# facebookresearch/ReAgent

Hardware: AMD Instinct MI355X
Metric: transitions/sec at batch=65536 state_dim=128; 1/2/4/8 MI355X scaling (higher is better)
Workload: dtype bf16; 1 GPU; Discrete DQN state_dim=128 |A|=16 3x512 MLP (BASELINE.json configs[1]; replay gather + normalize + 3 fwd + TD/Huber + bwd + Adam + soft update); batch=65536/GPU, 3x512 hidden; global_batch=65536, parallelism=dp1, launch=eager stream launches

## Files before the change

### include/reagent_hip.h

```cpp
#ifndef REAGENT_HIP_H_
#define REAGENT_HIP_H_

#include <stddef.h>
#include <stdint.h>

#ifdef __cplusplus
extern "C" {
#endif

typedef void* rg_stream_t;

enum { RG_OK = 0, RG_EINVAL = -1, RG_EALIGN = -2, RG_EUNSUPPORTED = -3, RG_EWORKSPACE = -4 };
enum { RG_PREC_F32 = 0, RG_PREC_BF16 = 1, RG_PREC_BF16X3 = 2  };
enum { RG_DT_F32 = 0, RG_DT_BF16 = 1 };
enum {
  RG_ACT_LINEAR = 0, RG_ACT_RELU = 1, RG_ACT_LEAKY_RELU = 2, RG_ACT_TANH = 3, RG_ACT_SIGMOID = 4,
  RG_ACT_SOFTPLUS = 5
};
enum { RG_LOSS_MSE = 0, RG_LOSS_HUBER = 1 };

const char* rg_strerror(int code);
int rg_abi_version(void);


// ... 24 lines not shown
                           rg_stream_t stream);

size_t rg_batch_norm_workspace_bytes(int batch, int n);
int rg_batch_norm_forward(const float* x, int64_t ldx, const float* gamma, const float* beta, float* running_mean,
                          float* running_var, int training, int stat_updates, double momentum, double eps, int batch, int n, float* y,
                          int64_t ldy, float* save_mean, float* save_rstd, void* workspace, size_t workspace_bytes,
                          rg_stream_t stream);
int rg_batch_norm_backward(const float* g, int64_t ldg, const float* x, int64_t ldx, const float* gamma,
                           const float* mean, const float* rstd, const float* running_var, int training, double eps,
                           int batch, int n, float* dx, int64_t lddx, float* dgamma, float* dbeta, void* workspace,
                           size_t workspace_bytes, rg_stream_t stream);

int rg_dropout(const float* x, int64_t ldx, int batch, int n, double p, int generate, uint64_t seed, uint64_t offset,
               uint8_t* keep, float* y, int64_t ldy, rg_stream_t stream);

int rg_act_backward(const float* dy, int64_t ld_dy, const float* y, int64_t ld_y, int act, float* dz,
                    int64_t ld_dz, int rows, int cols, rg_stream_t stream);


#define RG_MLP_MAX_LAYERS 6
typedef struct {
  int32_t n_layers;
  int32_t dims[RG_MLP_MAX_LAYERS + 1];
  int32_t acts[RG_MLP_MAX_LAYERS];
  const void* wfrag_fwd[RG_MLP_MAX_LAYERS];
  const void* wfrag_bwd[RG_MLP_MAX_LAYERS];
  const float* bias[RG_MLP_MAX_LAYERS];
  void* act_frag[RG_MLP_MAX_LAYERS];
  void* dz_frag[RG_MLP_MAX_LAYERS];
  void* act_sign[RG_MLP_MAX_LAYERS];
  float* db[RG_MLP_MAX_LAYERS];
  const float* w[RG_MLP_MAX_LAYERS];
  float* dw[RG_MLP_MAX_LAYERS];
  int32_t x3;
  int32_t dx_only;
  const void* x2;
  int64_t ldx2;
  int32_t x_split;
  int32_t dx_col0;
  int32_t x2_dtype;
  int32_t wgrad_flags;
  const int32_t* rowmap;
  const int32_t* tile_key;
  const int32_t* row_begin;
  int32_t n_groups;
  int32_t out_scatter;
  int64_t group_stride_fwd, group_stride_bwd;
  int32_t defer_db;
  int32_t sum_n;
  const float* db_partials;
  const float* sum_in;
  float* sum_out;
  double sum_scale;
} rg_mlp_desc;

int rg_mlp_fused_supported(const rg_mlp_desc* d);
size_t rg_frag_elems(int rows, int cols);
size_t rg_sign_bytes(int rows, int cols);
size_t rg_wfrag_elems(int out_features, int in_features);
int rg_stage_weights_frag(const float* w, int out_features, int in_features, void* wfrag_fwd,
                          void* wfrag_bwd, rg_stream_t stream);
int rg_mlp_forward_fused(const rg_mlp_desc* d, const void* x, int x_dtype, int64_t ldx, int batch,
                         float* out32, int64_t ldo, int save, rg_stream_t stream);
size_t rg_mlp_backward_fused_workspace_bytes(const rg_mlp_desc* d, int batch);
int rg_mlp_backward_fused(const rg_mlp_desc* d, const float* dout32, int64_t lddo, int batch,
                          float* dx32, int64_t lddx, void* workspace, size_t workspace_bytes,
                          rg_stream_t stream);
size_t rg_fc_wgrad_frag_workspace_bytes(int out_features, int in_features, int batch);
int rg_fc_wgrad_frag(const void* dz_frag, const void* x_frag, int out_features, int in_features,
                     int batch, float* dw, void* workspace, size_t workspace_bytes,
                     rg_stream_t stream);

int rg_mlp_stage_weights_fused(const rg_mlp_desc* d, int need_bwd, rg_stream_t stream);
size_t rg_mlp_wgrad_fused_workspace_bytes(const rg_mlp_desc* d, int batch);
int rg_mlp_wgrad_fused(const rg_mlp_desc* d, int batch, void* workspace, size_t workspace_bytes,
                       rg_stream_t stream);

typedef struct {
  float* param;
  const float* grad;
  float* exp_avg;
  float* exp_avg_sq;
  float* target;
  int32_t n_layers;
  int32_t dims[RG_MLP_MAX_LAYERS + 1];
  int64_t w_off[RG_MLP_MAX_LAYERS];
  int64_t b_off[RG_MLP_MAX_LAYERS];
  void* wfrag_fwd[RG_MLP_MAX_LAYERS];
  void* wfrag_bwd[RG_MLP_MAX_LAYERS];
  void* target_wfrag_fwd[RG_MLP_MAX_LAYERS];
  int32_t x3;
  int32_t group_rows[RG_MLP_MAX_LAYERS];
  int32_t sched_pre_ticked;
  int32_t post_tick_mod;
  int64_t* post_tick;
} rg_mlp_update_desc;
int rg_mlp_update_fused(const rg_mlp_update_desc* d, double lr, double beta1, double beta2, double eps,
                        double weight_decay, double bias_correction1, double bias_correction2_sqrt,
                        double grad_scale, double tau, rg_stream_t stream);


int rg_replay_nstep(const int64_t* indices, const uint8_t* terminal, const float* reward,
                    const float* decays, int64_t capacity, int update_horizon, int batch,
                    int64_t* steps, int64_t* next_indices, uint8_t* out_terminal,
                    float* out_reward, rg_stream_t stream);

// ... 98 lines not shown
  const int64_t* mdp_id;
  const int64_t* sequence_number;
  const float* decays;
  int64_t capacity;
  int32_t n_features;
  int32_t n_actions;
  int32_t update_horizon;
  int32_t reserved;
} rg_replay_view;
int rg_replay_dqn_batch(const rg_replay_view* view, const int64_t* indices, int batch, const rg_norm_col* cols,
                        const float* quantiles, const rg_dqn_batch_out* out, rg_stream_t stream);
int rg_replay_dqn_batch_pooled(const rg_replay_view* view, const int64_t* index_pool, const int64_t* cursor,
                               double* pre_tick_sched, int batch, const rg_norm_col* cols, const float* quantiles,
                               const rg_dqn_batch_out* out, rg_stream_t stream);

typedef struct {
  const float* observation;
  const float* action;
  const float* reward;
  const uint8_t* terminal;
  const float* log_prob;
  const float* decays;
  const float* ranges;
  int64_t capacity;
  int32_t n_features;
  int32_t action_dim;
  int32_t update_horizon;
  int32_t reserved;
} rg_policy_replay_view;
typedef struct {
  void* state;
  void* next_state;
  float* action;
  float* next_action;
  float* reward;
  float* not_terminal;
  float* action_probability;
  int32_t state_dtype;
  int32_t reserved;
} rg_policy_batch_out;
int rg_replay_policy_batch(const rg_policy_replay_view* view, const int64_t* indices, int batch, const rg_norm_col* cols,
                           const float* quantiles, const rg_policy_batch_out* out, rg_stream_t stream);

int rg_table_check_actions(const rg_dqn_table* table, const int64_t* indices, int batch, int* bad_flag,
                           rg_stream_t stream);


int rg_dqn_head_partials(int batch);
int rg_dqn_head(const float* q, const float* qn_online, const float* qn_target, const float* action,
                const float* next_mask, const float* reward, const float* reward_boosts,
                const float* not_terminal, double gamma, const float* gamma_exponent, int batch,
                int num_actions, int double_q, int loss_type, float* dq, float* loss_partials,
                float* next_q, int64_t* next_idx, float* q_sel, rg_stream_t stream);

int rg_bcq_filter(const float* imitator_logits, int batch, int num_actions, double drop_threshold, float* mask,
                  rg_stream_t stream);

int rg_cpe_head(const float* reward_est, const float* q_cpe, const float* q_cpe_tgt_next,
                const float* next_scores, const float* next_mask, const float* action,
                const float* reward, const float* extra_metrics, const float* not_terminal, double gamma,
                const float* gamma_exponent, double temperature, int batch, int num_actions,
                int num_metrics, int loss_type, float* d_reward_est, float* d_q_cpe,
                float* reward_partials, float* cpe_partials, float* propensities_out,
                rg_stream_t stream);

int rg_c51_head(const float* q, const float* qn_online, const float* qn_target, const float* action,
                const float* next_mask, const float* reward, const float* reward_boosts,
                const float* not_terminal, double gamma, const float* gamma_exponent, const float* support,
                double qmin, double qmax, int batch, int num_actions, int num_atoms, int maxq, float* dq,
                float* loss_partials, float* all_q, rg_stream_t stream);

int rg_dueling_combine(const float* value, int64_t ldv, const float* advantage, int64_t lda, int batch,
                       int num_actions, int num_atoms, float* q, int64_t ldq, rg_stream_t stream);
int rg_dueling_split(const float* dq, int64_t lddq, int batch, int num_actions, int num_atoms, float* dadvantage,
                     int64_t ldda, float* dvalue, int64_t lddv, rg_stream_t stream);

size_t rg_group_rows_workspace_bytes(int batch, int n_groups);
int rg_group_rows(const int32_t* key, int batch, int n_groups, int n_tiles, int dense, int32_t* rowmap, int32_t* tile_key,
                  int32_t* row_begin, void* workspace, size_t workspace_bytes, rg_stream_t stream);
size_t rg_group_wfrag_elems(int group_rows, int in_features, int transposed);
int rg_group_weights_stage(const float* w, int n_groups, int group_rows, int in_features, int x3, void* wfrag_fwd,
                           void* wfrag_bwd, rg_stream_t stream);
int rg_wide_head_mean(const float* w, const float* b, int n_groups, int group_rows, int in_features, float* wbar,
                      float* bbar, rg_stream_t stream);
int rg_wide_head_mean_staged(const float* w, const float* b, int n_groups, int group_rows, int in_features, float* wbar,
                             float* bbar, void* wfrag_fwd, int x3, rg_stream_t stream);
int rg_qr_select_action(const float* q, int64_t ldq, const float* mask, int batch, int num_actions, int maxq,
                        int32_t* key, rg_stream_t stream);
int rg_qr_select_group_rows(const float* q, int64_t ldq, const float* mask, int batch, int num_actions, int maxq,
                            int32_t* key, int n_tiles, int dense, int32_t* rowmap, int32_t* tile_key, int32_t* row_begin,
                            void* workspace, size_t workspace_bytes, rg_stream_t stream);
int rg_qr_compact_head(const float* z, int64_t ldz, const float* zt, int64_t ldzt, const int32_t* rowmap,
                       const int32_t* row_key, int padded_rows, const float* reward, const float* reward_boosts,
                       const float* not_terminal, double gamma, const float* gamma_exponent,
                       const float* quantiles, int batch, int num_atoms, float* dz, int64_t lddz,
                       float* loss_partials, float* tile_losses, rg_stream_t stream);
size_t rg_group_head_wgrad_workspace_bytes(int n_groups, int group_rows, int in_features, int splits);
int rg_group_head_wgrad(const void* dz_frag, const void* h_frag, const int32_t* row_begin, int n_groups,
                        int group_rows, int in_features, int splits, int x3, int rows, float* dw, void* workspace,
                        size_t workspace_bytes, rg_stream_t stream);

int rg_crr_partials(int batch);
int rg_crr_critic_head(const float* q1, const float* q2, const float* q1_next_target, const float* q2_next_target,
                       const float* next_logits, const float* action, const float* reward,
                       const float* reward_boosts, const float* not_terminal, double gamma, int batch,
                       int num_actions, float* target_out, float* dq1, float* dq2, float* partials1,
                       float* partials2, rg_stream_t stream);
int rg_crr_actor_head(const float* q, const float* logits, const float* action, const float* logged_prob,
                      double beta, double max_weight, double entropy_coeff, double clip_limit, int batch,
                      int num_actions, float* dlogits, float* plain_partials, float* entropy_partials,
                      rg_stream_t stream);

int rg_qr_head(const float* q, const float* qn_online, const float* qn_target, const float* action,
               const float* next_mask, const float* reward, const float* reward_boosts,
               const float* not_terminal, double gamma, const float* gamma_exponent,
               const float* quantiles, int batch, int num_actions, int num_atoms, int maxq, float* dq,
               float* loss_partials, float* all_q, rg_stream_t stream);


int rg_gaussian_head_forward(const float* loc_scale, int64_t ldls, const float* noise, int batch,
                             int action_dim, float* action, int64_t lda, float* log_prob,
                             float* squashed_mean, rg_stream_t stream);
int rg_gaussian_log_prob(const float* loc_scale, int64_t ldls, const float* action, int64_t lda,
                         int batch, int action_dim, float* log_prob, rg_stream_t stream);
int rg_gaussian_head_backward(const float* loc_scale, int64_t ldls, const float* noise,
                              const float* g_action, int64_t ldga, const float* g_log_prob, int batch,
                              int action_dim, float* d_loc_scale, int64_t lddls, rg_stream_t stream);
int rg_gaussian_head_backward_kld(const float* loc_scale, int64_t ldls, const float* noise, const float* g_action,
                                  int64_t ldga, const float* g_log_prob, int batch, int action_dim,
                                  float* d_loc_scale, int64_t lddls, const float* kld_coef, int kld_on_mean,
                                  rg_stream_t stream);
int rg_sac_kld(const float* x, int64_t ldx, int squash, int batch, int action_dim, const float* emb_mean,
               const float* emb_var, double weight, float* coef, float* kld_terms, float* kld, float* loss_inout,
               rg_stream_t stream);

int rg_sac_partials(int batch);
int rg_sac_critic_head(const float* q1, const float* q2, const float* q1_target, const float* q2_target,
                       const float* log_prob_next, const float* reward, const float* not_terminal,
                       double gamma, const double* alpha, int batch, float* target, float* dq1,
                       float* dq2, float* loss1_partials, float* loss2_partials, rg_stream_t stream);
int rg_sac_actor_head(const float* log_prob, const float* q1_actor, const float* q2_actor, const double* alpha,
                      double target_entropy, int batch, const float* v_cur, int crr_mode, double crr_p0,
                      double crr_clamp, int backprop_log_prob, float* g_log_prob, float* dq1_actor,
                      float* dq2_actor, float* loss_partials, float* entropy_partials, rg_stream_t stream);
int rg_sac_alpha_grad(const float* entropy_partials, int batch, const double* log_alpha, double* grad,
                      double* alpha_loss, rg_stream_t stream);
int rg_td3_target_action(const float* next_actor, int64_t ld_a, const float* noise, double noise_variance,
                         double noise_clip_lo, double noise_clip_hi, double lo, double hi, float* out,
                         int64_t ld_out, int batch, int action_dim, rg_stream_t stream);

int rg_adam_step_f64(double* param, const double* grad, double* exp_avg, double* exp_avg_sq, int64_t n,
                     double lr, double beta1, double beta2, double eps, double bias_correction1,
                     double bias_correction2_sqrt, double* exp_param_out, rg_stream_t stream);
int rg_add_cols(const float* a, int64_t lda, const float* b, int64_t ldb, int batch, int cols,
                float* out, int64_t ldo, rg_stream_t stream);

int rg_reduce_sum(const float* in, int n, float scale, float* out, rg_stream_t stream);


int rg_adam_step(float* param, const float* grad, float* exp_avg, float* exp_avg_sq, int64_t n,
                 double lr, double beta1, double beta2, double eps, double weight_decay,
                 double bias_correction1, double bias_correction2_sqrt, double grad_scale,
                 rg_stream_t stream);

int rg_adam_step_sched(float* param, const float* grad, float* exp_avg, float* exp_avg_sq, int64_t n,
                       double beta1, double beta2, double eps, double weight_decay, double grad_scale,
                       const double* sched, rg_stream_t stream);
int rg_mlp_update_fused_sched(const rg_mlp_update_desc* d, double beta1, double beta2, double eps,
                              double weight_decay, double grad_scale, double tau, const double* sched,
                              rg_stream_t stream);
int rg_adam_step_f64_sched(double* param, const double* grad, double* exp_avg, double* exp_avg_sq, int64_t n,
                           double beta1, double beta2, double eps, const double* sched,
                           double* exp_param_out, rg_stream_t stream);
int rg_sched_tick(double* sched, rg_stream_t stream);
#define RG_MAX_TICKS 8
int rg_sched_tick_many(double* const* scheds, int n, rg_stream_t stream);

int rg_soft_update(float* target, const float* source, int64_t n, double tau, rg_stream_t stream);

#ifdef __cplusplus
}
#endif
#endif
```

### profiles/microbench/fwd_phases.hip

```cpp
#include <hip/hip_runtime.h>
__device__ unsigned long long* g_stamps;
#define RG_STAMP(slot)                                                                                   \
  do {                                                                                                   \
    if ((threadIdx.x & 63) == 0)                                                                         \
      g_stamps[((long)blockIdx.x * (blockDim.x >> 6) + (threadIdx.x >> 6)) * 20 + (slot)] = __builtin_amdgcn_s_memtime(); \
  } while (0)
#include "../../reagent_amd/csrc/mlp_fused.hip"
namespace rg {
int x3_forward_launch(const rg_mlp_desc*, MlpArgs&, hipStream_t) { return RG_EINVAL; }
int x3_backward_launch(const rg_mlp_desc*, MlpArgs&, hipStream_t) { return RG_EINVAL; }
void grouped_bias_reduce_launch(const float*, const int*, int, int, float*, int, hipStream_t) {}
}
#include <cstdio>
#include <vector>

int main(int argc, char** argv) {
  using namespace rg;
  const int save = argc > 1 ? atoi(argv[1]) : 0;
  const int B = 65536, dims[5] = {128, 512, 512, 512, 16};
  MlpArgs a{};
  a.n_layers = 4; a.batch = B;
  for (int i = 0; i < 5; ++i) a.dims[i] = dims[i];
  for (int l = 0; l < 4; ++l) {
    a.acts[l] = l < 3 ? ACT_RELU : ACT_LINEAR;
    void* w; const size_t n = rg_wfrag_elems(dims[l + 1], dims[l]);
    hipMalloc(&w, n * 2); hipMemset(w, 0x3c, n * 2);
    a.wfrag[l] = (const bf16_t*)w;
    float* b; hipMalloc((void**)&b, dims[l + 1] * 4); hipMemset(b, 0, dims[l + 1] * 4);
    a.bias[l] = b;
    if (save) {
      void* f; hipMalloc(&f, rg_frag_elems(B, dims[l]) * 2); a.act_frag[l] = (bf16_t*)f;
      if (l >= 1) { void* sg; hipMalloc(&sg, rg_sign_bytes(B, dims[l])); a.act_sign[l] = (unsigned*)sg; }
    }
  }
  float *x, *out;
  hipMalloc((void**)&x, (size_t)B * 128 * 4); hipMemset(x, 0x3c, (size_t)B * 128 * 4);
  hipMalloc((void**)&out, (size_t)B * 16 * 4);
  a.x = x; a.ldx = 128; a.x_is_f32 = 1; a.out32 = out; a.ldo = 16; a.pitch = 520; a.save = save;
  const int n_wg = argc > 2 ? atoi(argv[2]) : B / 128, NPH = 20, NWV = FB_NW;
  unsigned long long* stamps;
  hipMalloc((void**)&stamps, (size_t)n_wg * NWV * NPH * 8);
  hipMemcpyToSymbol(HIP_SYMBOL(g_stamps), &stamps, sizeof(stamps));
  a.out_lds = argc > 3 ? atoi(argv[3]) : 0;
  const size_t lds = (size_t)128 * 520 * 2 + (a.out_lds ? 32 * 512 : 0);
  hipFuncSetAttribute((const void*)mlp_fwd_fused_kernel<512 / (32 * FB_NW), FB_NW, 520>, hipFuncAttributeMaxDynamicSharedMemorySize, (int)lds);
  hipEvent_t e0, e1; hipEventCreate(&e0); hipEventCreate(&e1);
  for (int w = 0; w < 3; ++w) mlp_fwd_fused_kernel<512 / (32 * FB_NW), FB_NW, 520><<<n_wg, FB_NW * 64, lds>>>(a);
  hipDeviceSynchronize();
  hipEventRecord(e0);
  for (int r = 0; r < 20; ++r) mlp_fwd_fused_kernel<512 / (32 * FB_NW), FB_NW, 520><<<n_wg, FB_NW * 64, lds>>>(a);
  hipEventRecord(e1); hipEventSynchronize(e1);
  float ms; hipEventElapsedTime(&ms, e0, e1);
  printf("forward NW=%d RING=%d save=%d: %.2f us/launch (stamps on), err=%d\n", FB_NW, MlpCfg<FB_NW>::RING, save, ms * 1e3 / 20, (int)hipGetLastError());
  std::vector<unsigned long long> h((size_t)n_wg * NWV * NPH);
  hipMemcpy(h.data(), stamps, h.size() * 8, hipMemcpyDeviceToHost);
  const char* names[NPH] = {"", "x tile load+barrier", "L0 mainloop(K=128)", "L0 pack", "L0 barrier wait", "L0 LDS store+barrier",
                            "L1 mainloop(K=512)", "L1 pack", "L1 barrier wait", "L1 LDS store+barrier",
                            "L2 mainloop(K=512)", "L2 pack", "L2 barrier wait", "L2 LDS store+barrier", "output layer", ""};
  double tot[NPH] = {0}, span = 0;
  for (int g = 0; g < n_wg; ++g)
    for (int w = 0; w < NWV; ++w) {
      const unsigned long long* s = &h[((size_t)g * NWV + w) * NPH];
      for (int p = 1; p <= 14; ++p) tot[p] += (double)(s[p] - s[p - 1]);
      span += (double)(s[14] - s[0]);
    }
  const double nw = (double)n_wg * NWV;
  printf("workgroups %d, shader clock %.3f GHz (ticks of one round / launch time)\n", n_wg, (span / nw) * ((n_wg + 255) / 256) / (ms * 1e6 / 20));
  printf("avg s_memtime ticks per wave: %.0f\n", span / nw);
  for (int p = 1; p <= 14; ++p) printf("  %-22s %9.0f ticks  %5.1f %%\n", names[p], tot[p] / nw, 100.0 * tot[p] / span);
  {
    double t[4] = {0, 0, 0, 0}, t19 = 0, n19 = 0;
    for (int g = 0; g < n_wg; ++g)
      for (int w = 0; w < NWV; ++w) {
        const unsigned long long* s = &h[((size_t)g * NWV + w) * NPH];
        if (!s[16]) continue;
        if (s[19]) { t19 += (double)(s[19] - s[18]); n19 += 1; }
        t[0] += (double)(s[16] - s[13]); t[1] += (double)(s[17] - s[16]); t[2] += (double)(s[18] - s[17]); t[3] += (double)(s[14] - s[18]);
      }
    printf("  storing waves: LDS sum %.0f ticks (of their sum + stores)\n", t19 / (n19 > 0 ? n19 : 1));
    printf("  output layer split: K loop %.0f | barrier wait %.0f | hand-off + barrier %.0f | sum + stores %.0f ticks\n", t[0] / nw, t[1] / nw, t[2] / nw, t[3] / nw);
  }
  printf("per-wave L1 main loop / barrier wait (ticks), averaged over workgroups:\n");
  for (int w = 0; w < NWV; ++w) {
    double ml = 0, bw = 0, ep = 0;
    for (int g = 0; g < n_wg; ++g) {
      const unsigned long long* s = &h[((size_t)g * NWV + w) * NPH];
      ml += (double)(s[6] - s[5]); bw += (double)(s[7] - s[6]); ep += (double)(s[8] - s[7]);
    }
    printf("  wave %d: mainloop %8.0f  pack %8.0f  wait %8.0f\n", w, ml / n_wg, bw / n_wg, ep / n_wg);
  }
  return 0;
}
```

### reagent_amd/_lib.py

```python
import ctypes
import os
import threading

import torch

_HERE = os.path.dirname(os.path.abspath(__file__))
LIB_PATH = os.environ.get("RG_LIB") or os.path.join(_HERE, "lib", "libreagent_hip.so")

ABI_VERSION = 11
PREC_F32, PREC_BF16, PREC_BF16X3 = 0, 1, 2
DT_F32, DT_BF16 = 0, 1
ACT = {"linear": 0, "relu": 1, "leaky_relu": 2, "tanh": 3, "sigmoid": 4, "softplus": 5}
LOSS = {"mse": 0, "huber": 1}
MAX_GATHER_COLS = 16

c_void_p, c_int, c_i64, c_f, c_d, c_sz = (
    ctypes.c_void_p,
    ctypes.c_int,
    ctypes.c_int64,
    ctypes.c_float,
    ctypes.c_double,
    ctypes.c_size_t,
)


class GatherCol(ctypes.Structure):
    _fields_ = [
        ("src", c_void_p),
        ("dst", c_void_p),
        ("indices", c_void_p),
        ("row_elems", ctypes.c_int32),
        ("elem_bytes", ctypes.c_int32),
        ("norm", c_void_p),
        ("norm_quantiles", c_void_p),
        ("out_dtype", ctypes.c_int32),
        ("reserved", ctypes.c_int32),
    ]


class NormCol(ctypes.Structure):
    _fields_ = [
        ("op", ctypes.c_int32),
        ("in_col", ctypes.c_int32),
        ("p0", c_f),
        ("p1", c_f),
        ("p2", c_f),
        ("p3", c_f),
    ]


MLP_MAX_LAYERS = 6


class MlpDesc(ctypes.Structure):
    _fields_ = [
        ("n_layers", ctypes.c_int32),
        ("dims", ctypes.c_int32 * (MLP_MAX_LAYERS + 1)),
        ("acts", ctypes.c_int32 * MLP_MAX_LAYERS),
        ("wfrag_fwd", c_void_p * MLP_MAX_LAYERS),
        ("wfrag_bwd", c_void_p * MLP_MAX_LAYERS),
        ("bias", c_void_p * MLP_MAX_LAYERS),
        ("act_frag", c_void_p * MLP_MAX_LAYERS),
        ("dz_frag", c_void_p * MLP_MAX_LAYERS),
        ("act_sign", c_void_p * MLP_MAX_LAYERS),
        ("db", c_void_p * MLP_MAX_LAYERS),
        ("w", c_void_p * MLP_MAX_LAYERS),
        ("dw", c_void_p * MLP_MAX_LAYERS),
        ("x3", ctypes.c_int32),
        ("dx_only", ctypes.c_int32),
        ("x2", c_void_p),
        ("ldx2", ctypes.c_int64),
        ("x_split", ctypes.c_int32),
        ("dx_col0", ctypes.c_int32),
        ("x2_dtype", ctypes.c_int32),
        ("wgrad_flags", ctypes.c_int32),
        ("rowmap", c_void_p),
        ("tile_key", c_void_p),
        ("row_begin", c_void_p),
        ("n_groups", ctypes.c_int32),
        ("out_scatter", ctypes.c_int32),
        ("group_stride_fwd", ctypes.c_int64),
        ("group_stride_bwd", ctypes.c_int64),
        ("defer_db", ctypes.c_int32),
        ("sum_n", ctypes.c_int32),
        ("db_partials", c_void_p),
        ("sum_in", c_void_p),
        ("sum_out", c_void_p),
        ("sum_scale", ctypes.c_double),
    ]


class MlpUpdateDesc(ctypes.Structure):
    _fields_ = [
        ("param", c_void_p), ("grad", c_void_p), ("exp_avg", c_void_p), ("exp_avg_sq", c_void_p), ("target", c_void_p),
        ("n_layers", ctypes.c_int32),
        ("dims", ctypes.c_int32 * (MLP_MAX_LAYERS + 1)),
        ("w_off", ctypes.c_int64 * MLP_MAX_LAYERS),
        ("b_off", ctypes.c_int64 * MLP_MAX_LAYERS),
        ("wfrag_fwd", c_void_p * MLP_MAX_LAYERS),
        ("wfrag_bwd", c_void_p * MLP_MAX_LAYERS),
        ("target_wfrag_fwd", c_void_p * MLP_MAX_LAYERS),
        ("x3", ctypes.c_int32),
        ("group_rows", ctypes.c_int32 * MLP_MAX_LAYERS),
        ("sched_pre_ticked", ctypes.c_int32),
        ("post_tick_mod", ctypes.c_int32),
        ("post_tick", c_void_p),
    ]


TABLE_COLUMNS = ("state_features", "state_features_presence", "next_state_features", "next_state_features_presence",
                 "action", "next_action", "reward", "action_probability", "time_diff", "step", "mdp_id",
                 "sequence_number", "possible_actions_mask", "possible_next_actions_mask")


class DqnTable(ctypes.Structure):
    _fields_ = [(n, c_void_p) for n in TABLE_COLUMNS] + [
        ("n_rows", ctypes.c_int64), ("n_features", ctypes.c_int32), ("n_actions", ctypes.c_int32)]


BATCH_OUT_FIELDS = ("state", "next_state", "action", "next_action", "reward", "time_diff", "step", "not_terminal",
                    "possible_actions_mask", "possible_next_actions_mask", "action_probability", "mdp_id",
                    "sequence_number")


class DqnBatchOut(ctypes.Structure):
    _fields_ = [(n, c_void_p) for n in BATCH_OUT_FIELDS] + [
        ("state_dtype", ctypes.c_int32), ("reserved", ctypes.c_int32)]


REPLAY_VIEW_COLUMNS = ("observation", "action", "reward", "terminal", "log_prob", "possible_actions_mask", "mdp_id",
                       "sequence_number", "decays")


class ReplayView(ctypes.Structure):
    _fields_ = [(n, c_void_p) for n in REPLAY_VIEW_COLUMNS] + [
        ("capacity", ctypes.c_int64), ("n_features", ctypes.c_int32), ("n_actions", ctypes.c_int32),
        ("update_horizon", ctypes.c_int32), ("reserved", ctypes.c_int32)]


POLICY_VIEW_COLUMNS = ("observation", "action", "reward", "terminal", "log_prob", "decays", "ranges")

# ... 31 lines not shown
    "rg_sign_bytes": (c_sz, [c_int, c_int]),
    "rg_wfrag_elems": (c_sz, [c_int, c_int]),
    "rg_stage_weights_frag": (c_int, [c_void_p, c_int, c_int, c_void_p, c_void_p, c_void_p]),
    "rg_mlp_forward_fused": (c_int, [ctypes.POINTER(MlpDesc), c_void_p, c_int, c_i64, c_int, c_void_p, c_i64,
                                      c_int, c_void_p]),
    "rg_mlp_backward_fused_workspace_bytes": (c_sz, [ctypes.POINTER(MlpDesc), c_int]),
    "rg_mlp_backward_fused": (c_int, [ctypes.POINTER(MlpDesc), c_void_p, c_i64, c_int, c_void_p, c_i64,
                                       c_void_p, c_sz, c_void_p]),
    "rg_fc_wgrad_frag_workspace_bytes": (c_sz, [c_int, c_int, c_int]),
    "rg_fc_wgrad_frag": (c_int, [c_void_p, c_void_p, c_int, c_int, c_int, c_void_p, c_void_p, c_sz, c_void_p]),
    "rg_mlp_stage_weights_fused": (c_int, [ctypes.POINTER(MlpDesc), c_int, c_void_p]),
    "rg_mlp_wgrad_fused_workspace_bytes": (c_sz, [ctypes.POINTER(MlpDesc), c_int]),
    "rg_mlp_wgrad_fused": (c_int, [ctypes.POINTER(MlpDesc), c_int, c_void_p, c_sz, c_void_p]),
    "rg_replay_nstep": (c_int, [c_void_p, c_void_p, c_void_p, c_void_p, c_i64, c_int, c_int,
                                 c_void_p, c_void_p, c_void_p, c_void_p, c_void_p]),
    "rg_replay_gather": (c_int, [ctypes.POINTER(GatherCol), c_int, c_i64, c_int, c_int, c_void_p]),
    "rg_mlp_update_fused": (c_int, [ctypes.POINTER(MlpUpdateDesc)] + [ctypes.c_double] * 9 + [c_void_p]),
    "rg_sumtree_depth": (c_int, [c_i64]),
    "rg_sumtree_nodes": (c_sz, [c_i64]),
    "rg_sumtree_set": (c_int, [c_void_p, c_int, c_i64, c_void_p, c_void_p, c_int, c_void_p, c_void_p]),
    "rg_sumtree_sample": (c_int, [c_void_p, c_int, c_void_p, c_int, c_void_p, c_void_p]),
    "rg_sumtree_get": (c_int, [c_void_p, c_int, c_i64, c_void_p, c_int, c_void_p, c_void_p, c_void_p]),
    "rg_make_dqn_input": (c_int, [c_void_p, c_void_p, c_void_p, c_void_p, c_int, c_int, c_void_p,
                                   c_void_p, c_void_p, c_void_p, c_void_p]),
    "rg_layer_norm_forward": (c_int, [c_void_p, c_i64, c_void_p, c_void_p, c_d, c_int, c_int, c_int, c_void_p, c_int, c_i64,
                                       c_void_p, c_i64, c_void_p, c_void_p, c_void_p]),
    "rg_layer_norm_backward_workspace_bytes": (c_sz, [c_int, c_int]),
    "rg_layer_norm_backward": (c_int, [c_void_p, c_i64, c_void_p, c_i64, c_void_p, c_void_p, c_void_p, c_int, c_int,
                                        c_void_p, c_int, c_i64, c_void_p, c_i64, c_void_p, c_void_p, c_void_p, c_sz, c_void_p]),
    "rg_batch_norm_workspace_bytes": (c_sz, [c_int, c_int]),
    "rg_batch_norm_forward": (c_int, [c_void_p, c_i64, c_void_p, c_void_p, c_void_p, c_void_p, c_int, c_int, c_d, c_d, c_int, c_int,
                                       c_void_p, c_i64, c_void_p, c_void_p, c_void_p, c_sz, c_void_p]),
    "rg_batch_norm_backward": (c_int, [c_void_p, c_i64, c_void_p, c_i64, c_void_p, c_void_p, c_void_p, c_void_p, c_int, c_d,
                                        c_int, c_int, c_void_p, c_i64, c_void_p, c_void_p, c_void_p, c_sz, c_void_p]),
    "rg_dropout": (c_int, [c_void_p, c_i64, c_int, c_int, c_d, c_int, ctypes.c_uint64, ctypes.c_uint64, c_void_p, c_void_p,
                            c_i64, c_void_p]),
    "rg_ragged_offsets": (c_int, [c_void_p, c_void_p, c_int, c_void_p, c_void_p, c_void_p]),
    "rg_ragged_copy": (c_int, [c_void_p, c_void_p, c_int, c_void_p, c_void_p, c_void_p, c_int, c_void_p, c_void_p, c_void_p]),
    "rg_make_policy_input": (c_int, [c_void_p, c_i64, c_void_p, c_i64, c_void_p, c_void_p, c_void_p, c_int, c_int,
                                      c_void_p, c_void_p, c_void_p, c_void_p, c_void_p]),
    "rg_normalize_dense": (c_int, [c_void_p, c_i64, c_void_p, c_i64, c_void_p, c_int, c_void_p,
                                    c_void_p, c_i64, c_int, c_void_p]),
    "rg_table_dqn_batch": (c_int, [ctypes.POINTER(DqnTable), c_void_p, c_int, c_void_p, c_int, c_void_p,
                                    ctypes.POINTER(DqnBatchOut), c_void_p]),
    "rg_replay_dqn_batch": (c_int, [ctypes.POINTER(ReplayView), c_void_p, c_int, c_void_p, c_void_p,
                                     ctypes.POINTER(DqnBatchOut), c_void_p]),
    "rg_replay_policy_batch": (c_int, [ctypes.POINTER(PolicyReplayView), c_void_p, c_int, c_void_p, c_void_p,
                                        ctypes.POINTER(PolicyBatchOut), c_void_p]),
    "rg_replay_dqn_batch_pooled": (c_int, [ctypes.POINTER(ReplayView), c_void_p, c_void_p, c_void_p, c_int, c_void_p, c_void_p,
                                            ctypes.POINTER(DqnBatchOut), c_void_p]),
    "rg_table_check_actions": (c_int, [ctypes.POINTER(DqnTable), c_void_p, c_int, c_void_p, c_void_p]),
    "rg_bcq_filter": (c_int, [c_void_p, c_int, c_int, c_d, c_void_p, c_void_p]),
    "rg_dqn_head_partials": (c_int, [c_int]),
    "rg_dqn_head": (c_int, [c_void_p] * 8 + [c_d, c_void_p, c_int, c_int, c_int, c_int] + [c_void_p] * 5 + [c_void_p]),
    "rg_cpe_head": (c_int, [c_void_p] * 9 + [ctypes.c_double, c_void_p, ctypes.c_double, c_int, c_int, c_int, c_int,
                            c_void_p, c_void_p, c_void_p, c_void_p, c_void_p, c_void_p]),
    "rg_c51_head": (c_int, [c_void_p] * 8 + [c_d, c_void_p, c_void_p, c_d, c_d, c_int, c_int, c_int, c_int, c_void_p,
                            c_void_p, c_void_p, c_void_p]),
    "rg_crr_partials": (c_int, [c_int]),
    "rg_crr_critic_head": (c_int, [c_void_p] * 9 + [c_d, c_int, c_int] + [c_void_p] * 5 + [c_void_p]),
    "rg_crr_actor_head": (c_int, [c_void_p] * 4 + [c_d, c_d, c_d, c_d, c_int, c_int] + [c_void_p] * 3 + [c_void_p]),
    "rg_qr_head": (c_int, [c_void_p] * 8 + [c_d, c_void_p, c_void_p, c_int, c_int, c_int, c_int, c_void_p,
                            c_void_p, c_void_p, c_void_p]),
    "rg_gaussian_head_forward": (c_int, [c_void_p, c_i64, c_void_p, c_int, c_int, c_void_p, c_i64, c_void_p,
                                          c_void_p, c_void_p]),
    "rg_gaussian_log_prob": (c_int, [c_void_p, c_i64, c_void_p, c_i64, c_int, c_int, c_void_p, c_void_p]),
    "rg_gaussian_head_backward": (c_int, [c_void_p, c_i64, c_void_p, c_void_p, c_i64, c_void_p, c_int, c_int,
                                           c_void_p, c_i64, c_void_p]),
    "rg_gaussian_head_backward_kld": (c_int, [c_void_p, c_i64, c_void_p, c_void_p, c_i64, c_void_p, c_int, c_int,
                                               c_void_p, c_i64, c_void_p, c_int, c_void_p]),
    "rg_sac_kld": (c_int, [c_void_p, c_i64, c_int, c_int, c_int, c_void_p, c_void_p, c_d] + [c_void_p] * 4 + [c_void_p]),
    "rg_sac_partials": (c_int, [c_int]),
    "rg_sac_critic_head": (c_int, [c_void_p] * 7 + [c_d, c_void_p, c_int] + [c_void_p] * 5 + [c_void_p]),
    "rg_sac_actor_head": (c_int, [c_void_p] * 4 + [c_d, c_int, c_void_p, c_int, c_d, c_d, c_int] + [c_void_p] * 5 + [c_void_p]),
    "rg_sac_alpha_grad": (c_int, [c_void_p, c_int, c_void_p, c_void_p, c_void_p, c_void_p]),
    "rg_adam_step_f64": (c_int, [c_void_p, c_void_p, c_void_p, c_void_p, c_i64, c_d, c_d, c_d, c_d, c_d, c_d,
                                  c_void_p, c_void_p]),
    "rg_add_cols": (c_int, [c_void_p, c_i64, c_void_p, c_i64, c_int, c_int, c_void_p, c_i64, c_void_p]),
    "rg_reduce_sum": (c_int, [c_void_p, c_int, c_f, c_void_p, c_void_p]),
    "rg_adam_step": (c_int, [c_void_p, c_void_p, c_void_p, c_void_p, c_i64, c_d, c_d, c_d, c_d, c_d,
                              c_d, c_d, c_d, c_void_p]),
    "rg_soft_update": (c_int, [c_void_p, c_void_p, c_i64, c_d, c_void_p]),
    "rg_dueling_combine": (c_int, [c_void_p, c_i64, c_void_p, c_i64, c_int, c_int, c_int, c_void_p, c_i64, c_void_p]),
    "rg_dueling_split": (c_int, [c_void_p, c_i64, c_int, c_int, c_int, c_void_p, c_i64, c_void_p, c_i64, c_void_p]),
    "rg_group_rows_workspace_bytes": (c_sz, [c_int, c_int]),
    "rg_group_rows": (c_int, [c_void_p, c_int, c_int, c_int, c_int, c_void_p, c_void_p, c_void_p, c_void_p, c_sz, c_void_p]),
    "rg_group_wfrag_elems": (c_sz, [c_int, c_int, c_int]),
    "rg_group_weights_stage": (c_int, [c_void_p, c_int, c_int, c_int, c_int, c_void_p, c_void_p, c_void_p]),
    "rg_wide_head_mean": (c_int, [c_void_p, c_void_p, c_int, c_int, c_int, c_void_p, c_void_p, c_void_p]),
    "rg_wide_head_mean_staged": (c_int, [c_void_p, c_void_p, c_int, c_int, c_int, c_void_p, c_void_p, c_void_p, c_int, c_void_p]),
    "rg_qr_select_action": (c_int, [c_void_p, c_i64, c_void_p, c_int, c_int, c_int, c_void_p, c_void_p]),
    "rg_qr_select_group_rows": (c_int, [c_void_p, c_i64, c_void_p, c_int, c_int, c_int, c_void_p, c_int, c_int, c_void_p, c_void_p, c_void_p, c_void_p, c_sz, c_void_p]),
    "rg_qr_compact_head": (c_int, [c_void_p, c_i64, c_void_p, c_i64, c_void_p, c_void_p, c_int, c_void_p, c_void_p,
                                    c_void_p, c_d, c_void_p, c_void_p, c_int, c_int, c_void_p, c_i64, c_void_p, c_void_p, c_void_p]),
    "rg_group_head_wgrad_workspace_bytes": (c_sz, [c_int, c_int, c_int, c_int]),
    "rg_group_head_wgrad": (c_int, [c_void_p, c_void_p, c_void_p, c_int, c_int, c_int, c_int, c_int, c_int, c_void_p, c_void_p,
                                     c_sz, c_void_p]),
    "rg_adam_step_sched": (c_int, [c_void_p, c_void_p, c_void_p, c_void_p, c_i64, c_d, c_d, c_d, c_d, c_d, c_void_p,
                                    c_void_p]),
    "rg_mlp_update_fused_sched": (c_int, [ctypes.POINTER(MlpUpdateDesc)] + [ctypes.c_double] * 6 + [c_void_p, c_void_p]),
    "rg_adam_step_f64_sched": (c_int, [c_void_p, c_void_p, c_void_p, c_void_p, c_i64, c_d, c_d, c_d, c_void_p,
                                        c_void_p, c_void_p]),
    "rg_sched_tick": (c_int, [c_void_p, c_void_p]),
    "rg_sched_tick_many": (c_int, [ctypes.POINTER(c_void_p), c_int, c_void_p]),
}

_lib = None
_lock = threading.Lock()


EUNSUPPORTED = -3


class ReagentHipError(RuntimeError):
    pass


def load(path: str = LIB_PATH):
    if not os.path.exists(path):
        raise ReagentHipError(
            f"{path} not found: the HIP extension is not built and there is no CPU fallback. "
            "Run `make -C reagent_amd/csrc` (or __graft_entry__.build())."
        )
    lib = ctypes.CDLL(path)
    for name, (res, args) in SIGNATURES.items():
        try:
            fn = getattr(lib, name)
        except AttributeError as e:
            raise ReagentHipError(f"{path} does not export {name}") from e
        fn.restype = res
        fn.argtypes = args
    if lib.rg_abi_version() != ABI_VERSION:
# ... 36 lines not shown
```

### reagent_amd/csrc/heads.hip

```cpp
#include <rg_platform.h>
#include "../../include/reagent_hip.h"
#include "rg_reduce.h"

namespace rg {

constexpr int HEAD_THREADS = 256;

__global__ void dqn_head_kernel(const float* __restrict__ q, const float* __restrict__ qn_online,
                                const float* __restrict__ qn_target, const float* __restrict__ action,
                                const float* __restrict__ next_mask, const float* __restrict__ reward,
                                const float* __restrict__ reward_boosts,
                                const float* __restrict__ not_terminal, float gamma,
                                const float* __restrict__ gamma_exponent, int batch, int A, int double_q,
                                int loss_type, float* __restrict__ dq, float* __restrict__ loss_partials,
                                float* __restrict__ next_q_out, int64_t* __restrict__ next_idx_out,
                                float* __restrict__ q_sel_out) {
  __shared__ float scratch[4];
  const int b = blockIdx.x * HEAD_THREADS + threadIdx.x;
  float loss = 0.f;
  const bool v4 = (A & 3) == 0 && ((((uintptr_t)q | (uintptr_t)qn_target | (uintptr_t)action | (uintptr_t)next_mask |
                                     (uintptr_t)dq | (uintptr_t)(double_q ? qn_online : qn_target)) & 15) == 0);
  if (b < batch) {
    const long o = (long)b * A;
    float best = 0.f, best_t = 0.f;
    int best_i = 0;
    float rb = 0.f, qs = 0.f;
    if (v4) {
      for (int a0 = 0; a0 < A; a0 += 4) {
        const f32x4 m4 = *(const f32x4*)(next_mask + o + a0);
        const f32x4 qt4 = *(const f32x4*)(qn_target + o + a0);
        const f32x4 qo4 = double_q ? *(const f32x4*)(qn_online + o + a0) : qt4;
        const f32x4 ac4 = *(const f32x4*)(action + o + a0);
        const f32x4 q4 = *(const f32x4*)(q + o + a0);
#pragma unroll
        for (int e = 0; e < 4; ++e) {
          const float pen = -1e9f * (1.f - m4[e]);
          const float qo = qo4[e] + pen, qt = qt4[e] + pen;
          const float key = double_q ? qo : qt;
          if (a0 + e == 0 || key > best) {
            best = key;
            best_t = qt;
            best_i = a0 + e;
          }
          if (reward_boosts) rb += ac4[e] * reward_boosts[a0 + e];
          qs += q4[e] * ac4[e];
        }
      }
    } else {
      for (int a = 0; a < A; ++a) {
        const float pen = -1e9f * (1.f - next_mask[o + a]);
        const float qo = (double_q ? qn_online[o + a] : qn_target[o + a]) + pen;
        const float qt = qn_target[o + a] + pen;
        const float key = double_q ? qo : qt;
        if (a == 0 || key > best) {
          best = key;
          best_t = qt;
          best_i = a;
        }
      }
      if (reward_boosts)
        for (int a = 0; a < A; ++a) rb += action[o + a] * reward_boosts[a];
      for (int a = 0; a < A; ++a) qs += q[o + a] * action[o + a];
    }
    const float next_q = best_t;
    const float rew = reward[b] + rb;
    const float disc = gamma_exponent ? powf(gamma, gamma_exponent[b]) : gamma;
    const float target = rew + disc * (next_q * not_terminal[b]);
    const float d = qs - target;
    float g;
    if (loss_type == RG_LOSS_HUBER) {
      const float ad = fabsf(d);
      loss = ad < 1.f ? 0.5f * d * d : ad - 0.5f;
      g = ad < 1.f ? d : (d > 0.f ? 1.f : -1.f);
    } else {
      loss = d * d;
      g = 2.f * d;
    }
    g /= (float)batch;
    if (v4) {
      for (int a0 = 0; a0 < A; a0 += 4) {
        const f32x4 ac4 = *(const f32x4*)(action + o + a0);
        *(f32x4*)(dq + o + a0) = f32x4{g * ac4[0], g * ac4[1], g * ac4[2], g * ac4[3]};
      }
    } else {
      for (int a = 0; a < A; ++a) dq[o + a] = g * action[o + a];
    }
    if (next_q_out) next_q_out[b] = next_q;
    if (next_idx_out) next_idx_out[b] = best_i;
    if (q_sel_out) q_sel_out[b] = qs;
  }
  const float s = block_sum_256(loss, scratch);
  if (threadIdx.x == 0) loss_partials[blockIdx.x] = s;
}

template <int G>
__global__ void __launch_bounds__(256 * G) dqn_head_lanes_kernel(
    const float* __restrict__ q, const float* __restrict__ qn_online, const float* __restrict__ qn_target,
    const float* __restrict__ action, const float* __restrict__ next_mask, const float* __restrict__ reward,
    const float* __restrict__ reward_boosts, const float* __restrict__ not_terminal, float gamma,
    const float* __restrict__ gamma_exponent, int batch, int double_q, int loss_type, float* __restrict__ dq,
    float* __restrict__ loss_partials, float* __restrict__ next_q_out, int64_t* __restrict__ next_idx_out,
    float* __restrict__ q_sel_out) {
  constexpr int A = 4 * G, WAVES = 4 * G;
  __shared__ float scratch[WAVES];
  const int t = threadIdx.x, sub = t % G;
  const int b_raw = blockIdx.x * 256 + t / G;
  const bool live = b_raw < batch;
  const int b = live ? b_raw : batch - 1;
  float loss = 0.f;
  {
    const long o = (long)b * A + sub * 4;
    const f32x4 m4 = *(const f32x4*)(next_mask + o);
    const f32x4 qt4 = *(const f32x4*)(qn_target + o);
    const f32x4 qo4 = double_q ? *(const f32x4*)(qn_online + o) : qt4;
    const f32x4 ac4 = *(const f32x4*)(action + o);
    const f32x4 q4 = *(const f32x4*)(q + o);
    float best = 0.f, best_t = 0.f, rb = 0.f, qs = 0.f;
    int best_i = 0;
#pragma unroll
    for (int e = 0; e < 4; ++e) {
      const float pen = -1e9f * (1.f - m4[e]);
      const float qo = qo4[e] + pen, qt = qt4[e] + pen;
      const float key = double_q ? qo : qt;
      if (e == 0 || key > best) {
        best = key;
        best_t = qt;
        best_i = sub * 4 + e;
      }
      if (reward_boosts) rb += ac4[e] * reward_boosts[sub * 4 + e];
      qs += q4[e] * ac4[e];
    }
#pragma unroll
    for (int off = 1; off < G; off <<= 1) {
      const float ok = shfl_xor(best, off), ot = shfl_xor(best_t, off);
      const int oi = shfl_xor(best_i, off);
      if (ok > best || (ok == best && oi < best_i)) {
        best = ok;
        best_t = ot;
        best_i = oi;
      }
      rb += shfl_xor(rb, off);
      qs += shfl_xor(qs, off);
    }
    const float rew = reward[b] + rb;
    const float disc = gamma_exponent ? powf(gamma, gamma_exponent[b]) : gamma;
    const float target = rew + disc * (best_t * not_terminal[b]);
    const float d = qs - target;
    float g, row_loss;
    if (loss_type == RG_LOSS_HUBER) {
      const float ad = fabsf(d);
      row_loss = ad < 1.f ? 0.5f * d * d : ad - 0.5f;
      g = ad < 1.f ? d : (d > 0.f ? 1.f : -1.f);
    } else {
      row_loss = d * d;
      g = 2.f * d;
    }
    g /= (float)batch;
    if (live) *(f32x4*)(dq + o) = f32x4{g * ac4[0], g * ac4[1], g * ac4[2], g * ac4[3]};
    if (live && sub == 0) {
      loss = row_loss;
      if (next_q_out) next_q_out[b] = best_t;
      if (next_idx_out) next_idx_out[b] = best_i;
      if (q_sel_out) q_sel_out[b] = qs;
    }
  }
#pragma unroll
  for (int off = 32; off >= 1; off >>= 1) loss += shfl_xor(loss, off);
  if ((t & 63) == 0) scratch[t >> 6] = loss;
  __syncthreads();
  if (t == 0) {
    float s = 0.f;
#pragma unroll
    for (int w = 0; w < WAVES; ++w) s += scratch[w];
    loss_partials[blockIdx.x] = s;
  }
}

__global__ void cpe_head_kernel(const float* __restrict__ reward_est, const float* __restrict__ q_cpe,
                                const float* __restrict__ q_cpe_tgt_next, const float* __restrict__ next_scores,
                                const float* __restrict__ next_mask, const float* __restrict__ action,
                                const float* __restrict__ reward, const float* __restrict__ extra_metrics,
                                const float* __restrict__ not_terminal, float gamma,
                                const float* __restrict__ gamma_exponent, float temperature, int batch, int A,
                                int M, int loss_type, float* __restrict__ d_reward_est, float* __restrict__ d_q_cpe,
                                float* __restrict__ reward_partials, float* __restrict__ cpe_partials,
                                float* __restrict__ propensities_out) {
  __shared__ float scratch[4];
  const int b = blockIdx.x * HEAD_THREADS + threadIdx.x;
  float loss_r = 0.f, loss_c = 0.f;
  if (b < batch) {
    const long o = (long)b * A, om = (long)b * M * A;
    int a_log = 0;
    float a_best = action[o];
    for (int a = 1; a < A; ++a)
      if (action[o + a] > a_best) {
        a_best = action[o + a];
        a_log = a;
      }
    float mx = 0.f;
    for (int a = 0; a < A; ++a) {
      const float v = next_scores[o + a] / temperature - ((1.0f - next_mask[o + a]) * 1e20f);
      if (a == 0 || v > mx) mx = v;
    }
    float den = 0.f;
    for (int a = 0; a < A; ++a) {
      const float v = next_scores[o + a] / temperature - ((1.0f - next_mask[o + a]) * 1e20f);
      den += expf(v - mx) * next_mask[o + a];
    }
    if (propensities_out)
      for (int a = 0; a < A; ++a) {
        const float v = next_scores[o + a] / temperature - ((1.0f - next_mask[o + a]) * 1e20f);
        const float p = expf(v - mx) * next_mask[o + a] / den;
        propensities_out[o + a] = p != p ? 0.f : p;
      }
    const float disc = gamma_exponent ? powf(gamma, gamma_exponent[b]) : gamma;
    const float nd = not_terminal[b];
    const float inv = 1.f / ((float)batch * (float)M);
    for (int i = 0; i < M; ++i) {
      const float real = i == 0 ? reward[b] : extra_metrics[(long)b * (M - 1) + (i - 1)];
      for (int a = 0; a < A; ++a) {
// ... 296 lines not shown
  __syncthreads();
  for (int k = tid; k < N; k += HEAD_THREADS) {
    float m = 0.f;
    for (int j = 0; j < N; ++j)
      if (LO[j] == k) m += W0[j];
    for (int j = 0; j < N; ++j)
      if (UP[j] == k) m += W1[j];
    Mm[k] = m;
  }
  __syncthreads();
  float lsum = 0.f, msum = 0.f;
  for (int j = tid; j < N; j += HEAD_THREADS) {
    lsum += Mm[j] * LD[j];
    msum += Mm[j];
  }
  const float tot_l = block_sum_256(lsum, scratch);
  const float tot_m = block_sum_256(msum, scratch);
  const float inv_b = 1.f / (float)batch;
  for (int i = tid; i < A * N; i += HEAD_THREADS) {
    const int a = i / N, k = i % N;
    const float w = act_row[a];
    float g = 0.f;
    if (w != 0.f) g = w * (expf((q[row + i] - c_max[a]) - c_lse[a]) * tot_m - Mm[k]) * inv_b;
    dq[row + i] = g;
  }
  if (tid == 0) loss_partials[b] = -tot_l * inv_b;
}

__global__ void bcq_filter_kernel(const float* __restrict__ logits, int batch, int A, float drop_threshold,
                                  float* __restrict__ mask) {
  const int b = blockIdx.x * HEAD_THREADS + threadIdx.x;
  if (b >= batch) return;
  const long o = (long)b * A;
  float mx = logits[o];
  for (int a = 1; a < A; ++a) mx = fmaxf(mx, logits[o + a]);
  float den = 0.f;
  for (int a = 0; a < A; ++a) den += expf(logits[o + a] - mx);
  float pmax = 0.f;
  for (int a = 0; a < A; ++a) pmax = fmaxf(pmax, expf(logits[o + a] - mx) / den);
  for (int a = 0; a < A; ++a) {
    const float keep = ((expf(logits[o + a] - mx) / den) / pmax >= drop_threshold) ? 1.f : 0.f;
    mask[o + a] *= keep;
  }
}

__global__ void reduce_sum_kernel(const float* __restrict__ in, int n, float scale,
                                  float* __restrict__ out) {
  __shared__ float scratch[4];
  static_assert(HEAD_THREADS == 256, "strided_sum_256");
  const float s = block_sum_256(strided_sum_256(in, n, threadIdx.x), scratch);
  if (threadIdx.x == 0) out[0] = s * scale;
}

}

namespace rg {
__global__ void dueling_combine_kernel(const float* __restrict__ value, long ldv, const float* __restrict__ adv, long lda,
                                       int batch, int A, int N, float* __restrict__ q, long ldq) {
  const int lane = threadIdx.x & 63, b = blockIdx.x * (blockDim.x >> 6) + (threadIdx.x >> 6);
  if (b >= batch) return;
  const int M = A * N;
  float s = 0.f;
  for (int i = lane; i < M; i += 64) s += adv[(long)b * lda + i];
#pragma unroll
  for (int off = 32; off >= 1; off >>= 1) s += shfl_xor(s, off);
  const float mean = s / (float)M;
  for (int i = lane; i < M; i += 64) q[(long)b * ldq + i] = value[(long)b * ldv + i % N] + (adv[(long)b * lda + i] - mean);
}
__global__ void dueling_split_kernel(const float* __restrict__ dq, long lddq, int batch, int A, int N,
                                     float* __restrict__ dadv, long ldda, float* __restrict__ dvalue, long lddv) {
  const int lane = threadIdx.x & 63, b = blockIdx.x * (blockDim.x >> 6) + (threadIdx.x >> 6);
  if (b >= batch) return;
  const int M = A * N;
  float s = 0.f;
  for (int i = lane; i < M; i += 64) s += dq[(long)b * lddq + i];
#pragma unroll
  for (int off = 32; off >= 1; off >>= 1) s += shfl_xor(s, off);
  const float mean = s / (float)M;
  for (int i = lane; i < M; i += 64) dadv[(long)b * ldda + i] = dq[(long)b * lddq + i] - mean;
  for (int n = lane; n < N; n += 64) {
    float t = 0.f;
    for (int a = 0; a < A; ++a) t += dq[(long)b * lddq + (long)a * N + n];
    dvalue[(long)b * lddv + n] = t;
  }
}
}

using namespace rg;

extern "C" {

int rg_dueling_combine(const float* value, int64_t ldv, const float* advantage, int64_t lda, int batch, int num_actions,
                       int num_atoms, float* q, int64_t ldq, rg_stream_t stream) {
  if (!value || !advantage || !q || batch <= 0 || num_actions <= 0 || num_atoms <= 0) return RG_EINVAL;
  RG_LAUNCH(dueling_combine_kernel, dim3((batch + 3) / 4), dim3(256), (hipStream_t)stream, value, (long)ldv, advantage,
            (long)lda, batch, num_actions, num_atoms, q, (long)ldq);
  return (int)hipGetLastError();
}

int rg_dueling_split(const float* dq, int64_t lddq, int batch, int num_actions, int num_atoms, float* dadvantage,
                     int64_t ldda, float* dvalue, int64_t lddv, rg_stream_t stream) {
  if (!dq || !dadvantage || !dvalue || batch <= 0 || num_actions <= 0 || num_atoms <= 0) return RG_EINVAL;
  RG_LAUNCH(dueling_split_kernel, dim3((batch + 3) / 4), dim3(256), (hipStream_t)stream, dq, (long)lddq, batch, num_actions,
            num_atoms, dadvantage, (long)ldda, dvalue, (long)lddv);
  return (int)hipGetLastError();
}
// ... 40 lines not shown
  RG_LAUNCH(cpe_head_kernel, dim3(rg_dqn_head_partials(batch)), dim3(HEAD_THREADS), (hipStream_t)stream, reward_est,
            q_cpe, q_cpe_tgt_next, next_scores, next_mask, action, reward, extra_metrics, not_terminal, (float)gamma,
            gamma_exponent, (float)temperature, batch, num_actions, num_metrics, loss_type, d_reward_est, d_q_cpe,
            reward_partials, cpe_partials, propensities_out);
  return (int)hipGetLastError();
}

int rg_qr_head(const float* q, const float* qn_online, const float* qn_target, const float* action,
               const float* next_mask, const float* reward, const float* reward_boosts,
               const float* not_terminal, double gamma, const float* gamma_exponent,
               const float* quantiles, int batch, int num_actions, int num_atoms, int maxq, float* dq,
               float* loss_partials, float* all_q, rg_stream_t stream) {
  if (!q || !qn_target || !action || !next_mask || !reward || !not_terminal || !quantiles || !dq ||
      !loss_partials || batch <= 0 || num_actions <= 0 || num_atoms <= 0)
    return RG_EINVAL;
  if (num_atoms > QR_MAX_ATOMS || num_actions > QR_MAX_ACTIONS) return RG_EUNSUPPORTED;
  RG_LAUNCH(qr_head_kernel, dim3(batch), dim3(HEAD_THREADS), (hipStream_t)stream, q, qn_online, qn_target,
            action, next_mask, reward, reward_boosts, not_terminal, (float)gamma, gamma_exponent, quantiles,
            batch, num_actions, num_atoms, maxq, dq, loss_partials, all_q);
  return (int)hipGetLastError();
}

int rg_c51_head(const float* q, const float* qn_online, const float* qn_target, const float* action,
                const float* next_mask, const float* reward, const float* reward_boosts, const float* not_terminal,
                double gamma, const float* gamma_exponent, const float* support, double qmin, double qmax,
                int batch, int num_actions, int num_atoms, int maxq, float* dq, float* loss_partials, float* all_q,
                rg_stream_t stream) {
  if (!q || !qn_target || !action || !next_mask || !reward || !not_terminal || !support || !dq || !loss_partials ||
      batch <= 0 || num_actions <= 0 || num_atoms <= 1)
    return RG_EINVAL;
  if (num_atoms > C51_MAX_ATOMS || num_actions > C51_MAX_ACTIONS) return RG_EUNSUPPORTED;
  const float scale = (float)((qmax - qmin) / ((double)num_atoms - 1.0));
  RG_LAUNCH(c51_head_kernel, dim3(batch), dim3(HEAD_THREADS), (hipStream_t)stream, q, qn_online, qn_target, action,
            next_mask, reward, reward_boosts, not_terminal, (float)gamma, gamma_exponent, support, (float)qmin,
            (float)qmax, scale, batch, num_actions, num_atoms, maxq, dq, loss_partials, all_q);
  return (int)hipGetLastError();
}

int rg_bcq_filter(const float* imitator_logits, int batch, int num_actions, double drop_threshold, float* mask,
                  rg_stream_t stream) {
  if (!imitator_logits || !mask || batch < 0 || num_actions <= 0) return RG_EINVAL;
  if (batch == 0) return RG_OK;
  RG_LAUNCH(bcq_filter_kernel, dim3((batch + HEAD_THREADS - 1) / HEAD_THREADS), dim3(HEAD_THREADS),
            (hipStream_t)stream, imitator_logits, batch, num_actions, (float)drop_threshold, mask);
  return (int)hipGetLastError();
}

int rg_reduce_sum(const float* in, int n, float scale, float* out, rg_stream_t stream) {
  if (!in || !out || n < 0) return RG_EINVAL;
  RG_LAUNCH(reduce_sum_kernel, dim3(1), dim3(HEAD_THREADS), (hipStream_t)stream, in, n, scale, out);
  return (int)hipGetLastError();
}

}
```

### reagent_amd/csrc/mlp_fused.hip

```cpp

#include "rg_mlp_frag.h"
#include "rg_reduce.h"
#include <cstdio>

namespace rg {

constexpr int WGRAD_TARGET = 128;
constexpr int GROUPED_RING = 8;
constexpr int REDUCE_FLY = 16;
constexpr int REDUCE_FLY_BF16 = 8;

template <int NW> struct MlpCfg {
  static constexpr int THREADS = NW * 64;
  static constexpr int RING = NW == 4 ? 8 : 2;
};

template <int NW>
__device__ __forceinline__ void grouped_whole_tile_out(bf16_t* act, int pitch, int KC, const bf16_t* wf_out, const float* b_out,
                                                                 int N, int NTo, int out_act, int lo, int hi, int row_base,
                                                                 const int* scatter, int batch, float* out32, long ldo) {
  const int tid = threadIdx.x, lane = tid & 63, wave = wave_uniform(tid >> 6), lr = lane & 31, lg = lane >> 5;
  const int P = NTo * 32 + 4, np = N >> 2;
  f32x16 acc4[4][1];
#pragma unroll
  for (int tm = 0; tm < 4; ++tm)
#pragma unroll
    for (int r = 0; r < 16; ++r) acc4[tm][0][r] = 0.f;
  const int col = wave * 32 + lr;
  float b = 0.f;
  if (wave < NTo) {
    if (b_out && col < N) b = b_out[col];
    wide_mainloop<1, GROUPED_RING>(act, pitch, KC, wf_out + (long)wave * KC * 512, 0, acc4, lane, k_rotation(blockIdx.x, wave, KC));
  }
  RG_STAMP(16);
  __syncthreads();
  RG_STAMP(17);
  float* stage = (float*)act;
  if (wave < NTo) {
#pragma unroll
    for (int tm = 0; tm < 4; ++tm) {
      float v[16];
#pragma unroll
      for (int r = 0; r < 16; ++r) v[r] = acc4[tm][0][r] + b;
      act_apply_n(v, out_act);
#pragma unroll
      for (int r = 0; r < 16; ++r) stage[(tm * 32 + (r & 3) + 8 * (r >> 2) + 4 * lg) * P + col] = v[r];
    }
  }
  __syncthreads();
  RG_STAMP(18);
  for (int rel = lo + wave; rel < hi; rel += NW) {
    int row = row_base + rel;
    if (scatter) row = scatter[row];
    if (row >= 0 && (scatter || row < batch) && lane < np)
      stream_store(*(const f32x4*)(stage + rel * P + lane * 4), (f32x4*)(out32 + (long)row * ldo + lane * 4));
  }
  RG_STAMP(19);
}

template <int TN, int NW, int PITCH, bool GROUPED>
__device__ __forceinline__ void mlp_fwd_fused_body(const MlpArgs& a) {
  constexpr int THREADS = MlpCfg<NW>::THREADS, RING = MlpCfg<NW>::RING;
  RG_DYN_LDS(smem);
  bf16_t* act = (bf16_t*)smem;
  const int tid = threadIdx.x, lane = tid & 63, wave = wave_uniform(tid >> 6);
  const int lr = lane & 31, lg = lane >> 5;
  const int tile = GROUPED ? grouped_tile(blockIdx.x, (a.batch + FB_BM - 1) / FB_BM) : (int)blockIdx.x;
  if (GROUPED && tile * FB_BM >= round_up(a.batch, FB_BM)) return;
  const int row_base = tile * FB_BM;
  constexpr int pitch = PITCH;
  const int k0p = round_up(a.dims[0], 32);
  RG_STAMP(0);
  if (a.rowmap) {
    if (a.x_is_f32)
      load_tile_rows_mapped<float, THREADS>(act, pitch, (const float*)a.x, a.ldx, a.rowmap, row_base, a.dims[0], k0p, tid);
    else
      load_tile_rows_mapped<bf16_t, THREADS>(act, pitch, (const bf16_t*)a.x, a.ldx, a.rowmap, row_base, a.dims[0], k0p, tid);
  } else if (a.x2) {
    const int n2 = a.dims[0] - a.x_split;
    if (a.x_is_f32)
      load_tile_to_lds<float, THREADS>(act, pitch, (const float*)a.x, a.ldx, row_base, a.batch, a.x_split, a.x_split, tid);
    else
      load_tile_to_lds<bf16_t, THREADS>(act, pitch, (const bf16_t*)a.x, a.ldx, row_base, a.batch, a.x_split, a.x_split, tid);
    if (a.x2_is_f32)
      load_tile_to_lds<float, THREADS>(act + a.x_split, pitch, (const float*)a.x2, a.ldx2, row_base, a.batch, n2, k0p - a.x_split, tid);
    else
      load_tile_to_lds<bf16_t, THREADS>(act + a.x_split, pitch, (const bf16_t*)a.x2, a.ldx2, row_base, a.batch, n2, k0p - a.x_split, tid);
  } else if (a.x_is_f32)
    load_tile_to_lds<float, THREADS>(act, pitch, (const float*)a.x, a.ldx, row_base, a.batch, a.dims[0], k0p, tid);
  else
    load_tile_to_lds<bf16_t, THREADS>(act, pitch, (const bf16_t*)a.x, a.ldx, row_base, a.batch, a.dims[0], k0p, tid);
  __syncthreads();
  RG_STAMP(1);
  if (a.save == 1 && a.act_frag[0]) emit_frags_from_lds(act, pitch, k0p / 32, a.act_frag[0], tile * 4, wave, NW, lane);
  const bool out_lds = !GROUPED && a.out_lds;
  char* wo = (char*)(act + FB_BM * pitch);
  if (out_lds) out_lds_prefetch(a.wfrag[a.n_layers - 1], (a.dims[a.n_layers - 1] + 15) / 16, wo, wave, NW, lane);

  for (int l = 0; l < a.n_layers; ++l) {
    const int K = a.dims[l], N = a.dims[l + 1];
    const int KC = (K + 15) / 16;
    if (l < a.n_layers - 1) {
      f32x16 acc[4][TN];
#pragma unroll
      for (int tm = 0; tm < 4; ++tm)
#pragma unroll
        for (int tn = 0; tn < TN; ++tn)
#pragma unroll
          for (int r = 0; r < 16; ++r) acc[tm][tn][r] = 0.f;
      const long nt_stride = (long)KC * 512;
      wide_mainloop<TN, RING>(act, pitch, KC, a.wfrag[l] + (long)(wave * TN) * nt_stride, nt_stride, acc, lane,
                              k_rotation(blockIdx.x, wave, KC), wave / (NW / 2));
      RG_STAMP(2 + 4 * l);
      unsigned PK[4][TN][8];
      unsigned* sign_dst = a.save ? a.act_sign[l + 1] : nullptr;
      RG_DISPATCH_ACT(a.acts[l], (fwd_hidden_pack<TN, A_>(acc, a.bias[l], fwd_save_dst(a, l),
                                                          sign_dst, N / 32, tile * 4, wave, lane, PK)));
      RG_STAMP(3 + 4 * l);
      __syncthreads();
      RG_STAMP(4 + 4 * l);
      store_packed_tiles<TN>(act, pitch, PK, wave, lane);
      if (out_lds) RG_WAIT_VMCNT(0);
      __syncthreads();
      RG_STAMP(5 + 4 * l);
    } else {
      const int NTo = (N + 31) / 32;
      const int out_act = a.acts[l];
      const bool stream_out = N > 64;
      int seg_g = GROUPED ? a.tile_key[tile] : 0;
      RowSegment seg{0, 0, FB_BM};
      const int o_lane = GROUPED ? opaque(lane) : lane, o_tid = GROUPED ? opaque(tid) : tid;
      while (!GROUPED || next_segment(a.row_begin, a.n_groups, row_base, FB_BM, seg_g, seg)) {
        const int lane = o_lane, tid = o_tid, lr = lane & 31, lg = lane >> 5;
        const int grp = seg.grp;
        const bf16_t* wf_out = a.wfrag[l] + (GROUPED ? (long)grp * a.group_stride : 0);
        const float* b_out = a.bias[l] ? a.bias[l] + (GROUPED ? (long)grp * N : 0) : nullptr;
        const int tm0 = GROUPED ? seg.lo >> 5 : 0, tm1 = GROUPED ? (seg.hi + 31) >> 5 : 4;
        const float b_tile0 = (b_out && lr < N) ? b_out[lr] : 0.f;
        auto store_tile = [&](const f32x16& acc, int tm, int nt) {
          const int col = nt * 32 + lr;
          if (col < N) {
            const float b = nt == 0 ? b_tile0 : (b_out ? b_out[col] : 0.f);
            float ov[16];
#pragma unroll
            for (int r = 0; r < 16; ++r) ov[r] = acc[r] + b;
            act_apply_n(ov, out_act);
#pragma unroll
            for (int r = 0; r < 16; ++r) {
              const int rel = tm * 32 + (r & 3) + 8 * (r >> 2) + 4 * lg;
              if (GROUPED && (rel < seg.lo || rel >= seg.hi)) continue;
              int row = row_base + rel;
              if (a.out_scatter) row = a.rowmap[row];
              if (row >= 0 && (a.out_scatter || row < a.batch)) {
                const float o = ov[r];
                if (stream_out) stream_store(o, a.out32 + (long)row * a.ldo + col);
                else a.out32[(long)row * a.ldo + col] = o;
              }
            }
          }
        };
        if (!GROUPED && NTo == 1 && NW == 8 && KC >= 8) {
          const int tm = wave & 3, half = wave >> 2, kc_mid = (KC / 2 + 3) / 4 * 4;
          f32x16 acc = out_lds ? tile_kloop_ldsb(act, pitch, wo, tm, lane, half ? kc_mid : 0, half ? KC : kc_mid)
                               : tile_kloop(act, pitch, KC, wf_out, tm, 0, lane, half ? kc_mid : 0, half ? KC : kc_mid);
          RG_STAMP(16);
          __syncthreads();
          RG_STAMP(17);
          const int o_ln = opaque(lane), o_lr = o_ln & 31, o_lg = o_ln >> 5;
          const bool aligned16 = (reinterpret_cast<uintptr_t>(a.out32) & 15) == 0;
          const bool dense_run = a.ldo == N && row_base + FB_BM <= a.batch;
          const bool rowstore = !a.out_scatter && aligned16 && (dense_run || ((N & 3) == 0 && (a.ldo & 3) == 0));
          if (rowstore) {
            float* outs = (float*)act + half * (FB_BM * 32);
            float* bias_s = (float*)act + 2 * (FB_BM * 32);
            if (o_lr < N) {
#pragma unroll
              for (int r = 0; r < 16; ++r) outs[(tm * 32 + (r & 3) + 8 * (r >> 2) + 4 * o_lg) * N + o_lr] = acc[r];
              if (wave == 0 && o_lg == 0) bias_s[o_lr] = b_tile0;
            }
            __syncthreads();
            RG_STAMP(18);
            RG_STAMP(19);
            const float* lo_ = (const float*)act;
            const float* hi_ = lo_ + FB_BM * 32;
            if (dense_run) {
              float* dst = a.out32 + (long)row_base * N;
              for (int it = wave * 64 + o_ln; it < (FB_BM * N) >> 2; it += THREADS) {
                const f32x4 l4 = *(const f32x4*)(lo_ + it * 4), h4 = *(const f32x4*)(hi_ + it * 4);
                float o[4];
#pragma unroll
                for (int e = 0; e < 4; ++e) o[e] = (l4[e] + h4[e]) + bias_s[(it * 4 + e) % N];
                act_apply_n(o, out_act);
                *(f32x4*)(dst + it * 4) = f32x4{o[0], o[1], o[2], o[3]};
              }
            }
            const int np = N >> 2;
            for (int it = wave * 64 + o_ln; !dense_run && it < FB_BM * np; it += THREADS) {
              const int rel = it / np, c4 = it - rel * np;
              const int row = row_base + rel;
              if (row < a.batch) {
                const f32x4 l4 = *(const f32x4*)(lo_ + rel * N + c4 * 4), h4 = *(const f32x4*)(hi_ + rel * N + c4 * 4);
                const f32x4 b4 = *(const f32x4*)(bias_s + c4 * 4);
                float o[4];
#pragma unroll
                for (int e = 0; e < 4; ++e) o[e] = (l4[e] + h4[e]) + b4[e];
                act_apply_n(o, out_act);
                *(f32x4*)(a.out32 + (long)row * a.ldo + c4 * 4) = f32x4{o[0], o[1], o[2], o[3]};
              }
            }
          } else {
            float* hand = (float*)act + (tm * 64 + lane) * 16;
            if (half) {
#pragma unroll
              for (int r = 0; r < 16; r += 4) *(f32x4*)(hand + r) = f32x4{acc[r], acc[r + 1], acc[r + 2], acc[r + 3]};
            }
            __syncthreads();
            RG_STAMP(18);
            if (!half) {
#pragma unroll
              for (int r = 0; r < 16; r += 4) {
                const f32x4 o = *(const f32x4*)(hand + r);
                acc[r] += o[0]; acc[r + 1] += o[1]; acc[r + 2] += o[2]; acc[r + 3] += o[3];
              }
              RG_STAMP(19);
              store_tile(acc, tm, 0);
            }
          }
        } else if (GROUPED && NTo <= NW && a.stage_out) {
          const int P = NTo * 32 + 4;
          const int np = N >> 2;
          bool last_segment = false;
          if ((size_t)FB_BM * P * sizeof(float) <= (size_t)FB_BM * pitch * sizeof(bf16_t)) {
            int g2 = seg_g;
            RowSegment s2;
            last_segment = !next_segment(a.row_begin, a.n_groups, row_base, FB_BM, g2, s2);
          }
          if (last_segment) {
            grouped_whole_tile_out<NW>(act, pitch, KC, wf_out, b_out, N, NTo, out_act, seg.lo, seg.hi, row_base, a.out_scatter ? a.rowmap : nullptr,
                                       a.batch, a.out32, a.ldo);
            break;
          }
          float* stage = (float*)(act + FB_BM * pitch);
          for (int tm = tm0; tm < tm1; ++tm) {
            if (wave < NTo) {
              const f32x16 acc = tile_kloop(act, pitch, KC, wf_out, tm, wave, lane);
              const int col = wave * 32 + lr;
              const float b = (b_out && col < N) ? b_out[col] : 0.f;
              float v[16];
#pragma unroll
              for (int r = 0; r < 16; ++r) v[r] = acc[r] + b;
              act_apply_n(v, out_act);
#pragma unroll
              for (int r = 0; r < 16; ++r) stage[((r & 3) + 8 * (r >> 2) + 4 * lg) * P + col] = v[r];
            }
            __syncthreads();
            for (int it = tid; it < 32 * np; it += THREADS) {
              const int r = it / np, c4 = it - r * np;
              const int rel = tm * 32 + r;
              if (rel < seg.lo || rel >= seg.hi) continue;
              int row = row_base + rel;
              if (a.out_scatter) row = a.rowmap[row];
              if (row >= 0 && (a.out_scatter || row < a.batch))
                stream_store(*(const f32x4*)(stage + r * P + c4 * 4), (f32x4*)(a.out32 + (long)row * a.ldo + c4 * 4));
            }
            __syncthreads();
          }
        } else {
          for (int t = wave; t < 4 * NTo; t += NW) {
            const int tm = t & 3, nt = t >> 2;
            if (tm < tm0 || tm >= tm1) continue;
            store_tile(tile_kloop(act, pitch, KC, wf_out, tm, nt, lane), tm, nt);
          }
        }
        if (!GROUPED) break;
      }
      RG_STAMP(2 + 4 * l);
    }
  }
}

template <int TN, int NW, int PITCH>
__global__ void RG_LAUNCH_BOUNDS(NW * 64, 1) mlp_fwd_fused_kernel(MlpArgs a) {
  mlp_fwd_fused_body<TN, NW, PITCH, false>(a);
}
template <int TN, int NW, int PITCH>
__global__ void RG_LAUNCH_BOUNDS(NW * 64, 1) mlp_fwd_grouped_kernel(MlpArgs a) {
  mlp_fwd_fused_body<TN, NW, PITCH, true>(a);
}

template <int TN, int NW, int PITCH, bool DX_ONLY, bool GROUPED = false>
__device__ __forceinline__ void mlp_bwd_fused_body(const MlpArgs& a) {
  constexpr int THREADS = MlpCfg<NW>::THREADS, RING = MlpCfg<NW>::RING;
  RG_DYN_LDS(smem);
  bf16_t* act = (bf16_t*)smem;
  const int tid = threadIdx.x, lane = tid & 63, wave = wave_uniform(tid >> 6);
  const int lr = lane & 31, lg = lane >> 5;
  const int tile = GROUPED ? grouped_tile(blockIdx.x, (a.batch + FB_BM - 1) / FB_BM) : (int)blockIdx.x;
  if (tile * FB_BM >= round_up(a.batch, FB_BM)) return;
  const int row_base = tile * FB_BM;
  constexpr int pitch = PITCH;
  const int L = a.n_layers;
  const int nop = round_up(a.dims[L], 32);
  RG_BSTAMP(0);
  auto request_signs = [&](int l, unsigned (&sg)[2 * TN]) {
    if (a.act_sign[l] != nullptr) {
      const u32x2* sp = (const u32x2*)(a.act_sign[l] + sign_offset(tile, wave, lane, TN, a.dims[l]));
#pragma unroll
      for (int i = 0; i < TN; ++i) {
        const u32x2 t = sp[i];
        sg[2 * i] = t[0];
        sg[2 * i + 1] = t[1];
      }
    } else {
#pragma unroll
      for (int i = 0; i < 2 * TN; ++i) sg[i] = 0u;
    }
  };
  unsigned sg_first[2 * TN];
  if (L >= 2) request_signs(L - 1, sg_first);
  const bool first_one_chunk = !GROUPED && L >= 2 && a.dims[L] <= 16;
  u16x8 w_first[TN];
  if (first_one_chunk) {
    const bf16_t* wl = a.wfrag[L - 1] + (long)(wave * TN) * 512 + lane * 8;
#pragma unroll
    for (int tn = 0; tn < TN; ++tn) w_first[tn] = *(const u16x8*)(wl + tn * 512);
  }
  load_tile_to_lds<float, THREADS>(act, pitch, a.dout32, a.lddo, row_base, a.batch, a.dims[L], nop, tid);
  __syncthreads();
  RG_BSTAMP(1);
  if (!GROUPED) {
    if (!DX_ONLY) emit_frags_from_lds(act, pitch, nop / 32, a.dz_frag[L - 1], tile * 4, wave, NW, lane);
    if (a.db_part[L - 1] && tid < a.dims[L]) {
      float s = 0.f;
// ... 642 lines not shown
    for (; r + 248 < S; r += 256) {
      float v[32];
#pragma unroll
      for (int u = 0; u < 32; ++u) v[u] = partials[(long)(r + 8 * u) * N + c];
#pragma unroll
      for (int u = 0; u < 32; u += 8) {
        s0 += v[u]; s1 += v[u + 1]; s2 += v[u + 2]; s3 += v[u + 3]; s4 += v[u + 4]; s5 += v[u + 5]; s6 += v[u + 6]; s7 += v[u + 7];
      }
    }
    for (; r + 56 < S; r += 64) {
      s0 += partials[(long)r * N + c];
      s1 += partials[(long)(r + 8) * N + c];
      s2 += partials[(long)(r + 16) * N + c];
      s3 += partials[(long)(r + 24) * N + c];
      s4 += partials[(long)(r + 32) * N + c];
      s5 += partials[(long)(r + 40) * N + c];
      s6 += partials[(long)(r + 48) * N + c];
      s7 += partials[(long)(r + 56) * N + c];
    }
    for (; r < S; r += 8) s0 += partials[(long)r * N + c];
  }
  red[g][threadIdx.x & 31] = ((s0 + s1) + (s2 + s3)) + ((s4 + s5) + (s6 + s7));
  __syncthreads();
  if (g == 0 && c < N) {
    float t = 0.f;
#pragma unroll
    for (int k = 0; k < 8; ++k) t += red[k][threadIdx.x & 31];
    out[c] = t;
  }
}

struct ReduceColsGroupArgs {
  int n;
  int block_begin[FB_MAXL + 1];
  const float* partials[FB_MAXL];
  float* out[FB_MAXL];
  int N[FB_MAXL];
  int S;
};
__global__ void reduce_cols_group_kernel(ReduceColsGroupArgs G) {
  int l = 0;
#pragma unroll
  for (int i = 1; i < FB_MAXL; ++i)
    if (i < G.n && (int)blockIdx.x >= G.block_begin[i]) l = i;
  reduce_cols_body(G.partials[l], G.S, G.N[l], G.out[l], (int)blockIdx.x - G.block_begin[l]);
}

struct ReduceTailArgs {
  ReduceGroupArgs splits;
  ReduceColsGroupArgs cols;
  int elem_blocks;
  const float* sum_in;
  int sum_n;
  float sum_scale;
  float* sum_out;
};

__global__ void reduce_tail_kernel(ReduceTailArgs T) {
  const int b = blockIdx.x;
  if (b < T.elem_blocks) {
    reduce_group_body(T.splits, (long)b * blockDim.x + threadIdx.x);
    return;
  }
  const int cb = b - T.elem_blocks;
  if (cb < T.cols.block_begin[T.cols.n]) {
    int l = 0;
#pragma unroll
    for (int i = 1; i < FB_MAXL; ++i)
      if (i < T.cols.n && cb >= T.cols.block_begin[i]) l = i;
    reduce_cols_body(T.cols.partials[l], T.cols.S, T.cols.N[l], T.cols.out[l], cb - T.cols.block_begin[l]);
    return;
  }
  __shared__ float scratch[4];
  float acc = strided_sum_256(T.sum_in, T.sum_n, threadIdx.x);
#pragma unroll
  for (int off = 32; off >= 1; off >>= 1) acc += shfl_xor(acc, off);
  if ((threadIdx.x & 63) == 0) scratch[threadIdx.x >> 6] = acc;
  __syncthreads();
  if (threadIdx.x == 0) T.sum_out[0] = ((scratch[0] + scratch[1]) + (scratch[2] + scratch[3])) * T.sum_scale;
}

__global__ void reduce_splits2_kernel(const float* __restrict__ partials, long slab, int splits,
                                      float* __restrict__ out, long n) {
  const long i = (long)blockIdx.x * blockDim.x + threadIdx.x;
  if (i >= n) return;
  float s = 0.f;
  for (int k = 0; k < splits; ++k) s += partials[(long)k * slab + i];
  out[i] = s;
}

__global__ void stage_group_kernel(StageGroupArgs G) {
  const long i = (long)blockIdx.x * blockDim.x + threadIdx.x;
  if (i >= G.begin[G.n]) return;
  const float* w = G.w[0];
  int N = G.N[0], K = G.K[0];
  bf16_t* wf = G.wf[0];
  bf16_t* wb = G.wb[0];
  long base = 0;
#pragma unroll
  for (int k = 1; k < FB_MAXL; ++k)
    if (k < G.n && i >= G.begin[k]) {
      w = G.w[k]; N = G.N[k]; K = G.K[k]; wf = G.wf[k]; wb = G.wb[k]; base = G.begin[k];
    }
  stage_weight_elem(w, N, K, wf, wb, i - base, G.x3);
}

__global__ void stage_weights_frag_kernel(const float* __restrict__ w, int N, int K, bf16_t* __restrict__ wf,
                                          bf16_t* __restrict__ wb) {
  const int NTf = (N + 31) / 32, KCf = (K + 15) / 16;
  const int NTb = (K + 31) / 32, KCb = (N + 15) / 16;
  const long tf = (long)NTf * KCf * 512, tb = (long)NTb * KCb * 512;
  const long total = tf > tb ? tf : tb;
  for (long i = (long)blockIdx.x * blockDim.x + threadIdx.x; i < total; i += (long)gridDim.x * blockDim.x) {
    stage_weight_elem(w, N, K, wf, wb, i);
  }
}

struct UpdateArgs {
  int n;
  long total;
  int N[FB_MAXL], K[FB_MAXL];
  long w_off[FB_MAXL], b_off[FB_MAXL];
  bf16_t* wf[FB_MAXL];
  bf16_t* wb[FB_MAXL];
  bf16_t* twf[FB_MAXL];
  float* p;
  const float* g;
// ... 150 lines not shown
    if (U.t) *(f32x4*)(U.t + i) = Tg;
    const int KCf = (K + 15) / 16;
    int nl = n;
    long gf = 0;
    if (U.Ng[l] > 0) {
      const int g = n / U.Ng[l];
      nl = n - g * U.Ng[l];
      gf = g * U.per_f[l];
    }
    const long jf = gf + ((((long)(nl >> 5) * KCf + (k >> 4)) * 64) + ((nl & 31) + 32 * ((k & 15) >> 3))) * 8 + (k & 7);
    const long tf = (long)(((U.Ng[l] > 0 ? U.Ng[l] : N) + 31) / 32) * KCf * 512;
    if (U.wf[l]) *(uint2*)(U.wf[l] + jf) = uint2{pack_bf16x2(pn[0], pn[1]), pack_bf16x2(pn[2], pn[3])};
    if (U.twf[l]) *(uint2*)(U.twf[l] + jf) = uint2{pack_bf16x2(tn[0], tn[1]), pack_bf16x2(tn[2], tn[3])};
    if (U.x3) {
#pragma unroll
      for (int e = 0; e < 4; ++e) {
        pl[e] = pn[e] - bf16_to_f32(f32_to_bf16(pn[e]));
        tl[e] = tn[e] - bf16_to_f32(f32_to_bf16(tn[e]));
      }
      if (U.wf[l]) *(uint2*)(U.wf[l] + tf + jf) = uint2{pack_bf16x2(pl[0], pl[1]), pack_bf16x2(pl[2], pl[3])};
      if (U.twf[l]) *(uint2*)(U.twf[l] + tf + jf) = uint2{pack_bf16x2(tl[0], tl[1]), pack_bf16x2(tl[2], tl[3])};
    }
  }
  if (!U.wb[l]) return;
#pragma unroll
  for (int e = 0; e < 4; ++e) {
    tile[r * UT_PITCH + c + e] = live ? f32_to_bf16(pn[e]) : (bf16_t)0;
    if (U.x3) tile_lo[r * UT_PITCH + c + e] = live ? f32_to_bf16(pl[e]) : (bf16_t)0;
  }
  __syncthreads();
  const int kk = tid & 31, ng = tid >> 5;
  const int kt = k0 + kk, nt = n0 + ng * 8;
  if (ng < UT_ROWS / 8 && kt < K && nt < N) {
    unsigned short h[8];
#pragma unroll
    for (int e = 0; e < 8; ++e) h[e] = (nt + e < N) ? tile[(ng * 8 + e) * UT_PITCH + kk] : (bf16_t)0;
    const int grp = U.Ng[l] > 0 ? nt / U.Ng[l] : 0;
    const int ntl = nt - grp * (U.Ng[l] > 0 ? U.Ng[l] : 0);
    const int KCb = ((U.Ng[l] > 0 ? U.Ng[l] : N) + 15) / 16;
    const long jb = grp * (U.Ng[l] > 0 ? U.per_b[l] : 0) +
                    ((((long)(kt >> 5) * KCb + (ntl >> 4)) * 64) + ((kt & 31) + 32 * ((ntl & 15) >> 3))) * 8;
    *(u32x4*)(U.wb[l] + jb) = u32x4{(unsigned)h[0] | ((unsigned)h[1] << 16), (unsigned)h[2] | ((unsigned)h[3] << 16),
                                    (unsigned)h[4] | ((unsigned)h[5] << 16), (unsigned)h[6] | ((unsigned)h[7] << 16)};
    if (U.x3) {
#pragma unroll
      for (int e = 0; e < 8; ++e) h[e] = (nt + e < N) ? tile_lo[(ng * 8 + e) * UT_PITCH + kk] : (bf16_t)0;
      const long tb = (long)((K + 31) / 32) * KCb * 512;
      *(u32x4*)(U.wb[l] + tb + jb) = u32x4{(unsigned)h[0] | ((unsigned)h[1] << 16), (unsigned)h[2] | ((unsigned)h[3] << 16),
                                           (unsigned)h[4] | ((unsigned)h[5] << 16), (unsigned)h[6] | ((unsigned)h[7] << 16)};
    }
  }
}

#define RG_LAUNCH_FUSED(KERNEL, hidden, pitch, grid, lds, stream, args)                                      \
  do {                                                                                                       \
    const dim3 block_(FB_NW * 64);                                                                           \
    if ((hidden) == 256 && (pitch) == 264) {                                                                 \
      RG_ALLOW_LDS((KERNEL<256 / (32 * FB_NW), FB_NW, 264>), lds);                                           \
      RG_LAUNCH_DYN((KERNEL<256 / (32 * FB_NW), FB_NW, 264>), grid, block_, lds, (hipStream_t)stream, args); \
    } else if ((hidden) == 256) {                                                                            \
      RG_ALLOW_LDS((KERNEL<256 / (32 * FB_NW), FB_NW, 520>), lds);                                           \
      RG_LAUNCH_DYN((KERNEL<256 / (32 * FB_NW), FB_NW, 520>), grid, block_, lds, (hipStream_t)stream, args); \
    } else {                                                                                                 \
      RG_ALLOW_LDS((KERNEL<512 / (32 * FB_NW), FB_NW, 520>), lds);                                           \
      RG_LAUNCH_DYN((KERNEL<512 / (32 * FB_NW), FB_NW, 520>), grid, block_, lds, (hipStream_t)stream, args); \
    }                                                                                                        \
  } while (0)

}

namespace rg {
static int padded_wgs(const rg_mlp_desc* d, int batch) {
  const int bm = d->x3 ? X3_BM : FB_BM;
  return (batch + 127) / 128 * (128 / bm);
}
}

using namespace rg;

extern "C" {

int rg_mlp_fused_supported(const rg_mlp_desc* d) { return fused_supported(d) > 0; }

size_t rg_frag_elems(int rows, int cols) {
  return (size_t)((rows + 127) / 128 * 128) * (size_t)((cols + 31) / 32 * 32);
}

size_t rg_sign_bytes(int rows, int cols) { return rg_frag_elems(rows, cols) / 8; }

size_t rg_wfrag_elems(int out_features, int in_features) {
  return (size_t)((out_features + 31) / 32) * (size_t)((in_features + 15) / 16) * 512;
}

int rg_stage_weights_frag(const float* w, int out_features, int in_features, void* wfrag_fwd, void* wfrag_bwd,
                          rg_stream_t stream) {
  if (!w || out_features <= 0 || in_features <= 0 || (!wfrag_fwd && !wfrag_bwd)) return RG_EINVAL;
  const size_t tf = rg_wfrag_elems(out_features, in_features), tb = rg_wfrag_elems(in_features, out_features);
  const size_t total = tf > tb ? tf : tb;
  long blocks = (long)((total + 255) / 256);
  if (blocks > 4096) blocks = 4096;
  RG_LAUNCH(stage_weights_frag_kernel, dim3((unsigned)blocks), dim3(256), (hipStream_t)stream, w, out_features,
            in_features, (bf16_t*)wfrag_fwd, (bf16_t*)wfrag_bwd);
  return (int)hipGetLastError();
}

int rg_mlp_forward_fused(const rg_mlp_desc* d, const void* x, int x_dtype, int64_t ldx, int batch, float* out32,
                         int64_t ldo, int save, rg_stream_t stream) {
  const int tn = fused_supported(d);
  if (!tn) return RG_EUNSUPPORTED;
  if (!x || !out32 || batch <= 0) return RG_EINVAL;
  MlpArgs a;
  int rc = fill_args(d, batch, a, 0);
  if (rc) return rc;
  if (save < 0 || save > 2) return RG_EINVAL;
  if (save)
    for (int l = (save == 2 ? 1 : 0); l < d->n_layers; ++l)
      if (!d->act_frag[l]) return RG_EINVAL;
  if (d->rowmap && (d->x2 || (d->x3 && !d->tile_key) || (batch % 128) != 0)) return RG_EUNSUPPORTED;
  if (d->tile_key && (!d->rowmap || !d->row_begin || d->n_groups <= 0)) return RG_EINVAL;
  if (d->x2 && (d->x_split <= 0 || d->x_split >= d->dims[0] || (d->x_split % 32) != 0)) return RG_EINVAL;
  a.x = x; a.ldx = ldx; a.x_is_f32 = (x_dtype == RG_DT_F32); a.out32 = out32; a.ldo = ldo; a.save = save;
  if (d->x3) return x3_forward_launch(d, a, (hipStream_t)stream);
  size_t lds = (size_t)FB_BM * a.pitch * sizeof(bf16_t);
  const int n_tiles = (batch + FB_BM - 1) / FB_BM;
  const dim3 grid(d->tile_key ? (n_tiles + 7) / 8 * 8 : n_tiles);
  a.stage_out = a.out_lds = 0;
  {
    const int L = d->n_layers, KCo = (d->dims[L - 1] + 15) / 16;
    if (!d->tile_key && L >= 2 && d->dims[L] <= 16 && FB_NW == 8 && KCo >= 8 && (KCo & 1) == 0 &&
        lds + (size_t)KCo * 512 <= 160 * 1024) {
      a.out_lds = 1;
      lds += (size_t)KCo * 512;
    }
  }
  if (d->tile_key) {
    const int No = d->dims[d->n_layers], NTo = (No + 31) / 32;
    const size_t stage = (size_t)32 * (NTo * 32 + 4) * sizeof(float);
    if (No > 64 && (No & 3) == 0 && (ldo & 3) == 0 && (((uintptr_t)out32) & 15) == 0 && lds + stage <= 160 * 1024) {
      a.stage_out = 1;
      lds += stage;
    }
  }
  if (d->tile_key) RG_LAUNCH_FUSED(mlp_fwd_grouped_kernel, d->dims[1], a.pitch, grid, lds, stream, a);
  else RG_LAUNCH_FUSED(mlp_fwd_fused_kernel, d->dims[1], a.pitch, grid, lds, stream, a);
  return (int)hipGetLastError();
}

size_t rg_mlp_backward_fused_workspace_bytes(const rg_mlp_desc* d, int batch) {
  if (!d || batch <= 0) return 0;
  size_t cols = 0;
  for (int l = 0; l < d->n_layers; ++l) cols += (size_t)d->dims[l + 1];
  const size_t extra = d->n_groups > 0 ? (size_t)d->n_groups * d->dims[d->n_layers] : 0;
  return ((size_t)padded_wgs(d, batch) * cols + extra) * sizeof(float);
}

int rg_mlp_backward_fused(const rg_mlp_desc* d, const float* dout32, int64_t lddo, int batch, float* dx32,
                          int64_t lddx, void* workspace, size_t workspace_bytes, rg_stream_t stream) {
  if (!fused_supported(d) && !fused_trunk(d)) return RG_EUNSUPPORTED;
  if (!dout32 || batch <= 0) return RG_EINVAL;
  MlpArgs a;
  int rc = fill_args(d, batch, a, 1);
  if (rc) return rc;
  bool want_db = false;
  for (int l = 0; l < d->n_layers; ++l) {
    if (!d->dx_only && !d->dz_frag[l]) return RG_EINVAL;
    if (l >= 1 && !d->act_frag[l]) return RG_EINVAL;
    if (d->db[l]) want_db = true;
  }
  if (dx32 && !d->wfrag_bwd[0]) return RG_EINVAL;
  if (d->dx_only && (!dx32 || want_db || d->tile_key)) return RG_EINVAL;
  if (d->tile_key && (!d->row_begin || d->n_groups <= 0 || d->dims[d->n_layers] > 256)) return RG_EINVAL;
  if (d->dx_col0 < 0 || d->dx_col0 >= d->dims[0] || (d->dx_col0 % 32) != 0) return RG_EINVAL;
  const int n_wg = padded_wgs(d, batch);
  if (want_db) {
    if (!workspace || workspace_bytes < rg_mlp_backward_fused_workspace_bytes(d, batch)) return RG_EWORKSPACE;
    float* p = (float*)workspace;
    for (int l = 0; l < d->n_layers; ++l) {
      a.db_part[l] = d->db[l] ? p : nullptr;
      p += (size_t)n_wg * d->dims[l + 1];
    }
  }
  a.dout32 = dout32; a.lddo = lddo; a.dx32 = dx32; a.lddx = lddx;
  if (d->x3) {
    rc = x3_backward_launch(d, a, (hipStream_t)stream);
  } else {
    size_t lds = (size_t)FB_BM * a.pitch * sizeof(bf16_t);
    const dim3 grid(d->tile_key ? (n_wg + 7) / 8 * 8 : n_wg);
    if (d->tile_key && a.pitch < 2 * 256 + 8) lds *= 2;
    if (d->dx_only) RG_LAUNCH_FUSED(mlp_bwd_dx_kernel, d->dims[1], a.pitch, grid, lds, stream, a);
    else if (d->tile_key) RG_LAUNCH_FUSED(mlp_bwd_grouped_kernel, d->dims[1], a.pitch, grid, lds, stream, a);
    else RG_LAUNCH_FUSED(mlp_bwd_fused_kernel, d->dims[1], a.pitch, grid, lds, stream, a);
    rc = (int)hipGetLastError();
  }
  if (rc) return rc;
  if (d->defer_db) {
    if (!want_db) return RG_EINVAL;
    const int l = d->n_layers - 1;
// ... 290 lines not shown
      continue;
    }
    const Entry& e = ent[j];
    const int l = e.layer;
    const WgradFragPlan& p = plan[l];
    WgradFragArgs& g = G.layer[j];
    g.a_frag = (const bf16_t*)d->dz_frag[l]; g.b_frag = (const bf16_t*)d->act_frag[l];
    g.NTa = p.NTa; g.NTb = p.NTb; g.MB = e.mb_end; g.mb_base = e.mb_base; g.mb_per_split = e.per; g.splits = e.splits;
    g.partial = part_of[l] + (size_t)e.split_base * slab_of[l]; g.slab = slab_of[l]; g.N = d->dims[l + 1]; g.K = d->dims[l];
    g.x3 = d->x3 ? (x3_dz_planes() == 1 ? 2 : 1) : 0;
    g.shape = p.shape;
    g.a_lo = d->x3 ? (long)frag_elems(batch, d->dims[l + 1]) : 0;
    g.b_lo = d->x3 ? (long)frag_elems(batch, d->dims[l]) : 0;
    g.part_mode = part_mode;
    wg += p.tiles * ((e.splits + 7) / 8 * 8);
  }
  G.wg_begin[WG_MAXV] = wg;
  R.elem_begin[FB_MAXL] = el;
  for (int l = d->n_layers; l <= FB_MAXL; ++l) R.elem_begin[l] = el;
  const size_t lds = (size_t)WG_SHAPED_LDS;
  RG_ALLOW_LDS(wgrad_group_kernel, lds);
  RG_LAUNCH_DYN(wgrad_group_kernel, dim3(wg), dim3(WG_THREADS), lds, (hipStream_t)stream, G);
  int rc = (int)hipGetLastError();
  if (rc) return rc;
  const int elem_blocks = (int)((el + 255) / 256);
  if (!d->db_partials && !d->sum_in) {
    RG_LAUNCH(reduce_group_kernel, dim3((unsigned)elem_blocks), dim3(256), (hipStream_t)stream, R);
    return (int)hipGetLastError();
  }
  ReduceTailArgs T;
  T.splits = R;
  T.elem_blocks = elem_blocks;
  ReduceColsGroupArgs& C = T.cols;
  C.n = 0;
  C.S = padded_wgs(d, batch);
  int blocks = 0;
  if (d->db_partials) {
    const float* p = d->db_partials;
    for (int l = 0; l < d->n_layers; ++l) {
      if (d->db[l]) {
        const int i = C.n++;
        C.block_begin[i] = blocks;
        C.partials[i] = p;
        C.out[i] = d->db[l];
        C.N[i] = d->dims[l + 1];
        blocks += (d->dims[l + 1] + 31) / 32;
      }
      p += (size_t)C.S * d->dims[l + 1];
    }
  }
  for (int i = C.n; i <= FB_MAXL; ++i) C.block_begin[i] = blocks;
  for (int i = C.n; i < FB_MAXL; ++i) { C.partials[i] = nullptr; C.out[i] = nullptr; C.N[i] = 0; }
  if (d->sum_in && (!d->sum_out || d->sum_n <= 0)) return RG_EINVAL;
  T.sum_in = d->sum_in; T.sum_n = d->sum_n; T.sum_scale = (float)d->sum_scale; T.sum_out = d->sum_out;
  RG_LAUNCH(reduce_tail_kernel, dim3((unsigned)(elem_blocks + blocks + (d->sum_in ? 1 : 0))), dim3(256), (hipStream_t)stream, T);
  return (int)hipGetLastError();
}

static int mlp_update_launch(const rg_mlp_update_desc* d, double lr, double beta1, double beta2, double eps,
                             double weight_decay, double bias_correction1, double bias_correction2_sqrt,
                             double grad_scale, double tau, const double* sched, rg_stream_t stream) {
  if (!d || d->n_layers < 1 || d->n_layers > FB_MAXL || !d->param || !d->grad || !d->exp_avg || !d->exp_avg_sq ||
      bias_correction1 == 0.0 || (d->target && (tau < 0.0 || tau > 1.0)))
    return RG_EINVAL;
  UpdateArgs U;
  U.n = d->n_layers;
  long total = 0;
  for (int l = 0; l < FB_MAXL; ++l) {
    if (l < d->n_layers) {
      const int K = d->dims[l], N = d->dims[l + 1];
      U.N[l] = N; U.K[l] = K;
      U.w_off[l] = d->w_off[l]; U.b_off[l] = d->b_off[l];
      U.wf[l] = (bf16_t*)d->wfrag_fwd[l]; U.wb[l] = (bf16_t*)d->wfrag_bwd[l]; U.twf[l] = (bf16_t*)d->target_wfrag_fwd[l];
      const int Ng = d->group_rows[l];
      if (Ng < 0 || (Ng > 0 && N % Ng != 0)) return RG_EINVAL;
      U.Ng[l] = Ng;
      U.per_f[l] = Ng > 0 ? (long)wfrag_elems(Ng, K) * (d->x3 ? 2 : 1) : 0;
      U.per_b[l] = Ng > 0 ? (long)wfrag_elems(K, Ng) * (d->x3 ? 2 : 1) : 0;
      const long we = d->w_off[l] + (long)N * K, be = d->b_off[l] + N;
      total = we > total ? we : total;
      total = be > total ? be : total;
    } else {
      U.N[l] = U.K[l] = 0; U.w_off[l] = U.b_off[l] = 0; U.wf[l] = U.wb[l] = U.twf[l] = nullptr;
      U.Ng[l] = 0; U.per_f[l] = U.per_b[l] = 0;
    }
  }
  U.total = total;
  U.p = d->param; U.g = d->grad; U.m = d->exp_avg; U.v = d->exp_avg_sq; U.t = d->target;
  const double step_size = lr / bias_correction1;
  U.c = AdamCoef{(float)(1.0 - beta1), (float)beta2, (float)(1.0 - beta2), (float)eps, (float)weight_decay,
                 (float)(-step_size), (float)bias_correction2_sqrt, (float)grad_scale};
  U.tau = (float)tau; U.one_minus_tau = (float)(1.0 - tau);
  U.sched = sched;
  U.pre_ticked = (sched && d->sched_pre_ticked) ? 1 : 0;
  U.post_tick = (long long*)d->post_tick;
  U.post_tick_mod = d->post_tick_mod > 0 ? d->post_tick_mod : 1;
  if (d->sched_pre_ticked && !sched) return RG_EINVAL;
  U.x3 = d->x3 ? 1 : 0;
  UpdateTileArgs T;
  T.u = U;
  int wgs = 0, any_tiled = 0;
  long rest = 0;
  for (int l = 0; l < FB_MAXL; ++l) {
    T.tile_begin[l] = wgs;
    T.tiled[l] = 0;
    if (l < d->n_layers) {
      const int K = U.K[l], N = U.N[l];
// ... 45 lines not shown
```

### reagent_amd/csrc/optim.hip

```cpp
#include "rg_optim.h"
#include "../../include/reagent_hip.h"

namespace rg {

__global__ void adam_kernel(float* __restrict__ p, const float* __restrict__ g, float* __restrict__ m,
                            float* __restrict__ v, long n, AdamCoef c0, const double* __restrict__ sched) {
  const AdamCoef c = sched_coef(c0, sched);
  for (long i = (long)blockIdx.x * blockDim.x + threadIdx.x; i < n; i += (long)gridDim.x * blockDim.x) {
    float mi = m[i], vi = v[i];
    p[i] = adam_element(c, p[i], g[i], mi, vi);
    m[i] = mi;
    v[i] = vi;
  }
}

__global__ void sched_tick_kernel(double* sched) {
  if (blockIdx.x == 0 && threadIdx.x == 0) sched[0] = sched[0] + 1.0;
}

struct TickMany {
  double* s[RG_MAX_TICKS];
};
__global__ void sched_tick_many_kernel(TickMany t, int n) {
  const int i = threadIdx.x;
// ... 26 lines not shown
  if (n == 0) return RG_OK;
  const double step_size = lr / bias_correction1;
  const AdamCoef c = {(float)(1.0 - beta1), (float)beta2, (float)(1.0 - beta2), (float)eps, (float)weight_decay,
                      (float)(-step_size), (float)bias_correction2_sqrt, (float)grad_scale};
  RG_LAUNCH(adam_kernel, dim3(grid_for(n)), dim3(256), (hipStream_t)stream, param, grad, exp_avg, exp_avg_sq, (long)n,
            c, sched);
  return (int)hipGetLastError();
}

int rg_adam_step(float* param, const float* grad, float* exp_avg, float* exp_avg_sq, int64_t n,
                 double lr, double beta1, double beta2, double eps, double weight_decay,
                 double bias_correction1, double bias_correction2_sqrt, double grad_scale,
                 rg_stream_t stream) {
  return adam_launch(param, grad, exp_avg, exp_avg_sq, n, lr, beta1, beta2, eps, weight_decay, bias_correction1,
                     bias_correction2_sqrt, grad_scale, nullptr, stream);
}

int rg_adam_step_sched(float* param, const float* grad, float* exp_avg, float* exp_avg_sq, int64_t n, double beta1,
                       double beta2, double eps, double weight_decay, double grad_scale, const double* sched,
                       rg_stream_t stream) {
  if (!sched) return RG_EINVAL;
  return adam_launch(param, grad, exp_avg, exp_avg_sq, n, 0.0, beta1, beta2, eps, weight_decay, 1.0, 1.0, grad_scale,
                     sched, stream);
}

int rg_sched_tick(double* sched, rg_stream_t stream) {
  if (!sched) return RG_EINVAL;
  RG_LAUNCH(sched_tick_kernel, dim3(1), dim3(64), (hipStream_t)stream, sched);
  return (int)hipGetLastError();
}

int rg_sched_tick_many(double* const* scheds, int n, rg_stream_t stream) {
  if (!scheds || n < 0 || n > RG_MAX_TICKS) return RG_EINVAL;
  if (n == 0) return RG_OK;
  TickMany t;
  for (int i = 0; i < RG_MAX_TICKS; ++i) {
    t.s[i] = scheds[i < n ? i : 0];
    if (i < n && !scheds[i]) return RG_EINVAL;
    for (int j = 0; j < i && i < n; ++j)
      if (scheds[j] == scheds[i]) return RG_EINVAL;
  }
  RG_LAUNCH(sched_tick_many_kernel, dim3(1), dim3(64), (hipStream_t)stream, t, n);
  return (int)hipGetLastError();
}

int rg_soft_update(float* target, const float* source, int64_t n, double tau, rg_stream_t stream) {
  if (!target || !source || n < 0 || tau < 0.0 || tau > 1.0) return RG_EINVAL;
  if (n == 0) return RG_OK;
  RG_LAUNCH(soft_update_kernel, dim3(grid_for(n)), dim3(256), (hipStream_t)stream, target, source,
            (long)n, (float)tau, (float)(1.0 - tau));
  return (int)hipGetLastError();
}

int rg_abi_version(void) { return 11; }

const char* rg_strerror(int code) {
  switch (code) {
    case RG_OK: return "ok";
    case RG_EINVAL: return "invalid argument";
    case RG_EALIGN: return "misaligned pointer or leading dimension";
    case RG_EUNSUPPORTED: return "unsupported dtype/precision";
    case RG_EWORKSPACE: return "workspace too small";
    default: return code > 0 ? "HIP runtime error (code is hipError_t)" : "unknown error";
  }
}

}
```

### reagent_amd/csrc/rg_mlp_frag.h

```cpp
#pragma once
#include "rg_gemm.h"
#include "rg_optim.h"
#include <type_traits>
#include "../../include/reagent_hip.h"

#ifndef RG_STAMP
#define RG_STAMP(slot)
#endif
#ifndef RG_BSTAMP
#define RG_BSTAMP(slot)
#endif
#ifndef RG_PHASE_INIT
#define RG_PHASE_INIT()
#define RG_PHASE(i)
#define RG_PHASE_FLUSH()
#endif

namespace rg {

constexpr int FB_BM = 128;
constexpr int WG_THREADS = 512;
constexpr int FB_NW = 8;
constexpr int FB_MAXL = RG_MLP_MAX_LAYERS;

#ifndef RG_X3_DZ_PLANES
#define RG_X3_DZ_PLANES 2
#endif
inline int x3_dz_planes() {
  static const int v = [] {
    const char* e = getenv("RG_X3_DZ_PLANES");
    const int n = e ? atoi(e) : RG_X3_DZ_PLANES;
    return n == 1 ? 1 : 2;
  }();
  return v;
}

struct MlpArgs {
  int n_layers, batch;
  int dims[FB_MAXL + 1];
  int acts[FB_MAXL];
  const bf16_t* wfrag[FB_MAXL];
  const float* bias[FB_MAXL];
  bf16_t* act_frag[FB_MAXL + 1];
  bf16_t* dz_frag[FB_MAXL];
  unsigned* act_sign[FB_MAXL];
  float* db_part[FB_MAXL];
  const void* x;
  long ldx;
  const void* x2;
  long ldx2;
  int x_split;
  int dx_col0;
  const int* rowmap;
  const int* tile_key;
  const int* row_begin;
  int n_groups;
  long group_stride;
  int out_scatter;
  int stage_out;
  int out_lds;
  int x_is_f32, x2_is_f32;
  float* out32;
  long ldo;
  const float* dout32;
  long lddo;
  float* dx32;
  long lddx;
  int pitch;
  int save;
  long wfrag_lo[FB_MAXL];
  long act_lo[FB_MAXL + 1];
  long dz_lo[FB_MAXL];
};

__device__ __forceinline__ int round_up(int x, int m) { return (x + m - 1) / m * m; }

template <int ACT> __device__ __forceinline__ float act_t(float z) { return act_apply(z, ACT); }

template <int ACT> __device__ __forceinline__ float act_grad_t(float h) { return act_grad_from_output(h, ACT); }
#define RG_DISPATCH_ACT(act, ...)                                                   \
  switch (act) {                                                                    \
    case ACT_RELU: { constexpr int A_ = ACT_RELU; __VA_ARGS__; } break;             \
    case ACT_LEAKY_RELU: { constexpr int A_ = ACT_LEAKY_RELU; __VA_ARGS__; } break; \
    case ACT_TANH: { constexpr int A_ = ACT_TANH; __VA_ARGS__; } break;             \
    case ACT_SIGMOID: { constexpr int A_ = ACT_SIGMOID; __VA_ARGS__; } break;       \
    case ACT_SOFTPLUS: { constexpr int A_ = ACT_SOFTPLUS; __VA_ARGS__; } break;     \
    default: { constexpr int A_ = ACT_LINEAR; __VA_ARGS__; } break;                 \
  }

__device__ __forceinline__ long frag_offset(int mb, int nt, int NT, int h, int lane) {
  return ((((long)mb * NT + nt) * 2 + h) * 64 + lane) * 8;
}
__device__ __forceinline__ int frag_row(int h, int e, int lg) {
  const int r = 8 * h + e;
  return (r & 3) + 8 * (r >> 2) + 4 * lg;
}

template <typename T, int THREADS>
__device__ __forceinline__ void load_tile_to_lds(bf16_t* act, int pitch, const T* src, long ld, int row_base,
                                                 int nrows, int ncols, int ncols_pad, int tid) {
  const int cpr = ncols_pad / 8;
  const int total = FB_BM * cpr;
  const bool vec = ((ld % 8) == 0) && ((((uintptr_t)src) & 15) == 0);
  if (vec && (ncols & 7) == 0 && ncols > 0) {
    constexpr int U = 4;
    const int kmax = ncols - 8;
    for (int c0 = tid; c0 < total; c0 += THREADS * U) {
      f32x4 raw[U][sizeof(T) == 4 ? 2 : 1];
#pragma unroll
      for (int u = 0; u < U; ++u) {
        const int cu = c0 + u * THREADS, c = cu < total ? cu : total - 1;
        const int gr = row_base + c / cpr, grow = gr < nrows ? gr : nrows - 1;
        const int kk = (c % cpr) * 8;
        const T* p = src + (long)grow * ld + (kk < kmax ? kk : kmax);
        raw[u][0] = *(const f32x4*)p;
        if (sizeof(T) == 4) raw[u][sizeof(T) == 4 ? 1 : 0] = *(const f32x4*)(p + 4);
      }
#pragma unroll
      for (int u = 0; u < U; ++u) {
        const int c = c0 + u * THREADS;
        if (c >= total) break;
        const int r = c / cpr, k0 = (c % cpr) * 8;
        u16x8 v;
        if (sizeof(T) == 4) {
#pragma unroll
          for (int e = 0; e < 4; ++e) {
            v[e] = f32_to_bf16(raw[u][0][e]);
// ... 530 lines not shown
```

### reagent_amd/csrc/rg_reduce.h

```cpp
#pragma once
#include <rg_platform.h>

namespace rg {

__device__ __forceinline__ float block_sum_256(float v, float* scratch ) {
#pragma unroll
  for (int off = 32; off >= 1; off >>= 1) v += shfl_xor(v, off);
  const int wave = threadIdx.x >> 6;
  if ((threadIdx.x & 63) == 0) scratch[wave] = v;
  __syncthreads();
  const float s = (scratch[0] + scratch[1]) + (scratch[2] + scratch[3]);
  __syncthreads();
  return s;
}

__device__ __forceinline__ float strided_sum_256(const float* __restrict__ in, int n, int tid) {
  float a[16];
#pragma unroll
  for (int j = 0; j < 16; ++j) a[j] = 0.f;
  int i = tid;
  for (; i + 15 * 256 < n; i += 16 * 256) {
#pragma unroll
    for (int j = 0; j < 16; ++j) a[j] += in[i + j * 256];
  }
  for (; i < n; i += 256) a[0] += in[i];
  return (((a[0] + a[1]) + (a[2] + a[3])) + ((a[4] + a[5]) + (a[6] + a[7]))) +
         (((a[8] + a[9]) + (a[10] + a[11])) + ((a[12] + a[13]) + (a[14] + a[15])));
}

}
```

### reagent_amd/engine.py

```python
import contextlib
from typing import List, Optional, Sequence

import torch

from . import _lib as L
from . import ops


def _round_up(x: int, m: int) -> int:
    return (x + m - 1) // m * m


def _mat(rows: int, cols: int, dtype, device) -> torch.Tensor:
    ld = _round_up(max(cols, 1), 8)
    return torch.empty(rows, ld, dtype=dtype, device=device)[:, :cols]


class ParamSlab:

    ALIGN = 4

    def __init__(self, params: Sequence[torch.nn.Parameter]):
        self.params = list(params)
        assert len(self.params) > 0
# ... 303 lines not shown
        P = self.planes
        for i, w in enumerate(self.weights):
            out_f, in_f = w.shape
            if self._wf[i] is None or self._wf[i].device != dev:
                self._wf[i] = torch.empty(P * lib.rg_wfrag_elems(out_f, in_f), dtype=torch.bfloat16, device=dev)
            if need_bwd and (self._wb[i] is None or self._wb[i].device != dev):
                self._wb[i] = torch.empty(P * lib.rg_wfrag_elems(in_f, out_f), dtype=torch.bfloat16, device=dev)
            wd = w.detach()
            assert wd.is_contiguous()
            L.require_cuda(wd)
            d.w[i] = wd.data_ptr()
            d.wfrag_fwd[i] = self._wf[i].data_ptr()
            d.wfrag_bwd[i] = self._wb[i].data_ptr() if self._wb[i] is not None else None
        ops._run("rg_mlp_stage_weights_fused", dict(L=self.L),
                 lambda: lib.rg_mlp_stage_weights_fused(d, int(need_bwd), L.stream_ptr()))
        self._staged_versions = versions
        self._wsrc_ptrs = [w.data_ptr() for w in self.weights]

    def _ensure_ws(self, batch: int, device, training: bool):
        key = (batch, device, training)
        if self._ws.get("key") == key:
            return
        if not training and self._ws.get("key", (0, device))[1] == device:
            self._ws.setdefault("key", key)
            return
        lib = L.lib()
        ws = {"key": key}
        if training:
            bf = dict(dtype=torch.bfloat16, device=device)
            P = self.planes
            ws["act_frag"] = [torch.empty(P * lib.rg_frag_elems(batch, self.dims[l]), **bf) for l in range(self.L)]
            ws["dz_frag"] = [torch.empty(P * lib.rg_frag_elems(batch, self.dims[l + 1]), **bf) for l in range(self.L)]
            ws["act_sign"] = [torch.empty(lib.rg_sign_bytes(batch, self.dims[l]), dtype=torch.uint8, device=device)
                              if l >= 1 else None for l in range(self.L)]
            dd = L.MlpDesc()
            dd.n_layers = self.L
            dd.x3 = int(self.x3)
            for i, v in enumerate(self.dims):
                dd.dims[i] = v
            nbytes = lib.rg_mlp_wgrad_fused_workspace_bytes(dd, batch)
            ws["wgrad"] = torch.empty(_round_up(nbytes, 16) // 4, dtype=torch.float32, device=device)
            self._ws = ws
            nb = lib.rg_mlp_backward_fused_workspace_bytes(self._fill_desc(), batch)
            ws["bwd"] = torch.empty(_round_up(nb, 16) // 4, dtype=torch.float32, device=device)
        self._ws = ws
        self._batch = batch

    def _fill_desc(self):
        d = self._desc
        d.n_layers = self.L
        d.x3 = int(self.x3)
        d.dx_col0 = 0
        d.dx_only = 0
        d.defer_db, d.sum_n = 0, 0
        d.db_partials, d.sum_in, d.sum_out = None, None, None
        for i, v in enumerate(self.dims):
            d.dims[i] = v
        ws = self._ws
        for l in range(self.L):
            d.acts[l] = self.acts[l]
            d.wfrag_fwd[l] = self._wf[l].data_ptr() if self._wf[l] is not None else None
            d.wfrag_bwd[l] = self._wb[l].data_ptr() if self._wb[l] is not None else None
            d.bias[l] = self.biases[l].data_ptr()
            d.act_frag[l] = ws["act_frag"][l].data_ptr() if "act_frag" in ws else None
            d.dz_frag[l] = ws["dz_frag"][l].data_ptr() if "dz_frag" in ws else None
            d.act_sign[l] = ws["act_sign"][l].data_ptr() if "act_sign" in ws and ws["act_sign"][l] is not None else None
        return d

    def stage_input(self, x32: torch.Tensor, need_transposed: bool):
        return x32, None

    def forward(self, xc: torch.Tensor, out32: torch.Tensor, save: bool = False, x2: Optional[torch.Tensor] = None,
                rowmap: Optional[torch.Tensor] = None):
        L.require_cuda(xc)
        B = xc.shape[0] if rowmap is None else rowmap.shape[0]
        save = int(save)
        self._ensure_ws(B, xc.device, training=bool(save))
        d = self._fill_desc()
        assert xc.stride(1) == 1 and out32.stride(1) == 1
        if x2 is not None:
            L.require_cuda(x2)
            assert x2.stride(1) == 1 and xc.shape[1] % 32 == 0
            assert xc.shape[1] + x2.shape[1] == self.dims[0] and x2.shape[0] == B
            d.x2, d.ldx2, d.x_split, d.x2_dtype = x2.data_ptr(), x2.stride(0), xc.shape[1], ops.dt_code(x2.dtype)
        else:
            assert xc.shape[1] == self.dims[0]
            d.x2, d.ldx2, d.x_split = None, 0, 0
        if rowmap is not None:
            assert rowmap.dtype == torch.int32 and rowmap.is_contiguous() and B % 128 == 0 and out32.shape[0] == B
            L.require_cuda(rowmap)
        d.rowmap = rowmap.data_ptr() if rowmap is not None else None
        ops._run("rg_mlp_forward_fused", dict(B=B, save=int(save), dims=tuple(self.dims)),
                 lambda: L.lib().rg_mlp_forward_fused(d, xc.data_ptr(), ops.dt_code(xc.dtype), xc.stride(0), B,
                                                      out32.data_ptr(), out32.stride(0), save,
                                                      L.stream_ptr()))
        self._saved = save
        return out32

    def backward(self, dout32: torch.Tensor, xt, dw: List[torch.Tensor], db: List[torch.Tensor],
                 dx32: Optional[torch.Tensor] = None, skip_wgrad: bool = False,
                 out32: Optional[torch.Tensor] = None, dx_col0: int = 0, tail_sum=None):
        dout32 = _through_output_activation(self.acts[-1], dout32, out32)
        B = dout32.shape[0]
        assert self._ws.get("key") == (B, dout32.device, True), "backward needs a saving forward first"
        d = self._fill_desc()
        d.x2, d.ldx2, d.x_split = None, 0, 0
        d.dx_col0 = dx_col0
        d.dx_only = int(skip_wgrad and dx32 is not None and (db is None or all(b is None for b in db)))
        assert self._saved == 1 or d.dx_only, "a forward saved with SAVE_FOR_DX serves a dx-only backward (skip_wgrad) alone"
        if dx32 is not None:
            assert dx_col0 % 32 == 0 and dx32.shape[1] == self.dims[0] - dx_col0
        lib = L.lib()
        ws = self._ws
        want_db = False
        for l in range(self.L):
            d.db[l] = db[l].data_ptr() if (db is not None and not skip_wgrad and db[l] is not None) else None
            want_db = want_db or bool(d.db[l])
        defer = bool(want_db and not skip_wgrad and self.fold_tails)
        d.defer_db = int(defer)
        d.db_partials, d.sum_in, d.sum_out, d.sum_n, d.sum_scale = None, None, None, 0, 0.0
        ops._run("rg_mlp_backward_fused", dict(B=B, dims=tuple(self.dims)),
                 lambda: lib.rg_mlp_backward_fused(d, dout32.data_ptr(), dout32.stride(0), B,
                                                   dx32.data_ptr() if dx32 is not None else None,
                                                   dx32.stride(0) if dx32 is not None else 0,
                                                   ws["bwd"].data_ptr(), ws["bwd"].numel() * 4, L.stream_ptr()))
        d.dx_only = 0
        d.defer_db = 0
        if not skip_wgrad:
            for l in range(self.L):
                d.dw[l] = dw[l].data_ptr()
            if defer:
                d.db_partials = ws["bwd"].data_ptr()
            if tail_sum is not None:
                part, scale, out = tail_sum
                L.require_cuda(part)
                L.require_cuda(out)
                assert part.dtype == torch.float32 and part.is_contiguous() and out.dtype == torch.float32
                d.sum_in, d.sum_n, d.sum_scale, d.sum_out = part.data_ptr(), part.numel(), float(scale), out.data_ptr()
            wsb = ws["wgrad"].numel() * 4
            ops._run("rg_mlp_wgrad_fused", dict(B=B, dims=tuple(self.dims)),
                     lambda: lib.rg_mlp_wgrad_fused(d, B, ws["wgrad"].data_ptr(), wsb, L.stream_ptr()))
            d.db_partials, d.sum_in, d.sum_out, d.sum_n = None, None, None, 0
        else:
            assert tail_sum is None, "tail_sum rides in the weight gradient's launch"


class GroupedHead:

    def __init__(self, weight: torch.Tensor, bias: torch.Tensor, n_groups: int, group_rows: int, need_bwd: bool, x3: bool = False):
        self.weight, self.bias, self.G, self.Ng = weight, bias, n_groups, group_rows
        H = weight.shape[1]
        dev = weight.device
        self.H = H
        self.x3, self.planes = bool(x3), 2 if x3 else 1
        self.per_f = self.planes * ops.group_wfrag_elems(group_rows, H, False)
        self.per_b = self.planes * ops.group_wfrag_elems(group_rows, H, True)
        self.wf = torch.empty(n_groups * self.per_f, dtype=torch.bfloat16, device=dev)
        self.wb = torch.empty(n_groups * self.per_b, dtype=torch.bfloat16, device=dev) if need_bwd else None
        self._rows = -1

    def stage(self):
        ops.group_weights_stage(self.weight.detach(), self.G, self.Ng, self.wf, self.wb, x3=self.x3)

    def workspace(self, rows: int, st: "FusedMLP"):
        if self._rows != rows:
            dev = self.weight.device
            lib = L.lib()
            self.dz_frag = torch.zeros(self.planes * lib.rg_frag_elems(ops.grouped_dz_rows(rows, self.G), self.Ng), dtype=torch.bfloat16,
                                       device=dev)
            d = self.desc(st, None, None, None)
            self.bwd_ws = torch.empty(lib.rg_mlp_backward_fused_workspace_bytes(d, rows) // 4 + 4, dtype=torch.float32, device=dev)
            self._rows = rows

    def desc(self, st: "FusedMLP", space, scatter, save_dz) -> "L.MlpDesc":
        src = st._fill_desc()
        d = L.MlpDesc()
        ctypes_copy(d, src)
        n = st.L
        d.dims[n] = self.Ng
        d.wfrag_fwd[n - 1] = self.wf.data_ptr()
        d.wfrag_bwd[n - 1] = self.wb.data_ptr() if self.wb is not None else None
        d.bias[n - 1] = self.bias.data_ptr()
        d.group_stride_fwd, d.group_stride_bwd, d.n_groups = self.per_f, self.per_b, self.G
        if space is not None:
            d.rowmap, d.tile_key, d.row_begin = space.rowmap.data_ptr(), space.tile_key.data_ptr(), space.row_begin.data_ptr()
            d.out_scatter = int(bool(scatter))
        if save_dz:
            d.dz_frag[n - 1] = self.dz_frag.data_ptr()
        return d


def ctypes_copy(dst, src):
    import ctypes

    ctypes.memmove(ctypes.byref(dst), ctypes.byref(src), ctypes.sizeof(type(src)))
# ... 195 lines not shown
```

### reagent_amd/ops.py

```python
import contextlib
import ctypes
import os
from typing import List, Optional, Tuple

import torch

from . import _lib as L

BF16 = torch.bfloat16
F32 = torch.float32


def compute_dtype(precision: int) -> torch.dtype:
    return F32 if precision == L.PREC_F32 else BF16


def dt_code(dtype: torch.dtype) -> int:
    if dtype == F32:
        return L.DT_F32
    if dtype == BF16:
        return L.DT_BF16
    raise L.ReagentHipError(f"unsupported dtype {dtype}")


# ... 366 lines not shown
    es = out["state"].element_size()
    nbytes = (2 * F_ * 4 + 2 * F_ * es + 5 * H_ + 2 * 8 + 4 + 8 + (2 * A_ * 4 if view.possible_actions_mask else 0)
              + 4 * A_ * 4 + 3 * 4)
    _run("rg_replay_dqn_batch", dict(B=B, bytes_per_row=nbytes), call)
    return rc[0] == 0


def replay_policy_batch(view: "L.PolicyReplayView", indices, cols_dev, quantiles, out: dict) -> bool:
    _chk_dev(indices, cols_dev, quantiles, *out.values())
    assert indices.dtype == torch.int64 and indices.is_contiguous()
    o = L.PolicyBatchOut()
    for name in L.POLICY_OUT_FIELDS:
        t = out.get(name)
        assert t is None or t.is_contiguous()
        setattr(o, name, t.data_ptr() if t is not None else None)
    o.state_dtype = dt_code(out["state"].dtype)
    B = indices.numel()
    rc = [0]

    def call():
        rc[0] = L.lib().rg_replay_policy_batch(ctypes.byref(view), L.ptr(indices), B, L.ptr(cols_dev), L.ptr(quantiles),
                                               ctypes.byref(o), L.stream_ptr())
        return 0 if rc[0] == L.EUNSUPPORTED else rc[0]

    F_, A_, H_ = view.n_features, view.action_dim, view.update_horizon
    es = out["state"].element_size()
    nbytes = 2 * F_ * 4 + 2 * F_ * es + 4 * A_ * 4 + 5 * H_ + 8 + 4 + 3 * 4
    _run("rg_replay_policy_batch", dict(B=B, bytes_per_row=nbytes), call)
    return rc[0] == 0


def table_check_actions(table, indices) -> int:
    _chk_dev(indices)
    flag = torch.zeros(1, dtype=torch.int32, device=indices.device)
    _run("rg_table_check_actions", dict(B=indices.numel()),
         lambda: L.lib().rg_table_check_actions(ctypes.byref(table.desc()), L.ptr(indices), indices.numel(),
                                                L.ptr(flag), L.stream_ptr()))
    return int(flag.item())


def bcq_filter(imitator_logits, drop_threshold: float, mask):
    _chk_dev(imitator_logits, mask)
    B, A = mask.shape
    assert imitator_logits.shape == (B, A) and imitator_logits.dtype == F32 and mask.dtype == F32
    assert imitator_logits.is_contiguous() and mask.is_contiguous()
    _run("rg_bcq_filter", dict(B=B, A=A),
         lambda: L.lib().rg_bcq_filter(L.ptr(imitator_logits), B, A, float(drop_threshold), L.ptr(mask), L.stream_ptr()))


def dqn_head_partials(batch: int) -> int:
    return int(L.lib().rg_dqn_head_partials(batch))


def dqn_head(q, qn_online, qn_target, action, next_mask, reward, reward_boosts, not_terminal, gamma,
             gamma_exponent, double_q, loss_type, dq, loss_partials, next_q=None, next_idx=None,
             q_sel=None):
    _chk_dev(q, qn_online, qn_target, action, next_mask, reward, reward_boosts, not_terminal,
             gamma_exponent, dq, loss_partials, next_q, next_idx, q_sel)
    batch, A = q.shape
    for t in (q, qn_online, qn_target, action, next_mask, dq):
        assert t.is_contiguous() and t.dtype == F32 and t.shape == (batch, A)
    for t in (reward, not_terminal, gamma_exponent):
        assert t is None or (t.is_contiguous() and t.dtype == F32 and t.numel() == batch)
    _run("rg_dqn_head", dict(B=batch, A=A),
         lambda: L.lib().rg_dqn_head(L.ptr(q), L.ptr(qn_online), L.ptr(qn_target), L.ptr(action),
                                     L.ptr(next_mask), L.ptr(reward), L.ptr(reward_boosts),
                                     L.ptr(not_terminal), float(gamma), L.ptr(gamma_exponent), batch, A,
                                     int(double_q), loss_type, L.ptr(dq), L.ptr(loss_partials), L.ptr(next_q),
                                     L.ptr(next_idx), L.ptr(q_sel), L.stream_ptr()))


def cpe_head(reward_est, q_cpe, q_cpe_tgt_next, next_scores, next_mask, action, reward, extra_metrics,
             not_terminal, gamma, gamma_exponent, temperature, num_metrics, loss_type, d_reward_est, d_q_cpe,
             reward_partials, cpe_partials, propensities_out=None):
    _chk_dev(reward_est, q_cpe, q_cpe_tgt_next, next_scores, next_mask, action, reward, extra_metrics,
             not_terminal, gamma_exponent, d_reward_est, d_q_cpe, reward_partials, cpe_partials, propensities_out)
    batch, A = action.shape
    M = num_metrics
    for t in (reward_est, q_cpe, q_cpe_tgt_next, d_reward_est, d_q_cpe):
        assert t.is_contiguous() and t.dtype == F32 and t.shape == (batch, M * A)
    for t in (next_scores, next_mask, action):
        assert t.is_contiguous() and t.dtype == F32 and t.shape == (batch, A)
    assert extra_metrics is None or (extra_metrics.is_contiguous() and extra_metrics.shape == (batch, M - 1))
    _run("rg_cpe_head", dict(B=batch, A=A, M=M),
         lambda: L.lib().rg_cpe_head(L.ptr(reward_est), L.ptr(q_cpe), L.ptr(q_cpe_tgt_next), L.ptr(next_scores),
                                     L.ptr(next_mask), L.ptr(action), L.ptr(reward), L.ptr(extra_metrics),
                                     L.ptr(not_terminal), float(gamma), L.ptr(gamma_exponent), float(temperature),
                                     batch, A, M, loss_type, L.ptr(d_reward_est), L.ptr(d_q_cpe),
                                     L.ptr(reward_partials), L.ptr(cpe_partials), L.ptr(propensities_out),
                                     L.stream_ptr()))


def c51_head(q, qn_online, qn_target, action, next_mask, reward, reward_boosts, not_terminal, gamma,
             gamma_exponent, support, qmin, qmax, num_atoms, maxq, dq, loss_partials, all_q=None):
    _chk_dev(q, qn_online, qn_target, action, next_mask, reward, reward_boosts, not_terminal, gamma_exponent,
             support, dq, loss_partials, all_q)
    batch, A = action.shape
    for t in (q, qn_target, dq):
        assert t.is_contiguous() and t.dtype == F32 and t.shape == (batch, A * num_atoms)
    _run("rg_c51_head", dict(B=batch, A=A, N=num_atoms),
         lambda: L.lib().rg_c51_head(L.ptr(q), L.ptr(qn_online), L.ptr(qn_target), L.ptr(action), L.ptr(next_mask),
                                     L.ptr(reward), L.ptr(reward_boosts), L.ptr(not_terminal), float(gamma),
                                     L.ptr(gamma_exponent), L.ptr(support), float(qmin), float(qmax), batch, A,
                                     num_atoms, int(maxq), L.ptr(dq), L.ptr(loss_partials), L.ptr(all_q),
                                     L.stream_ptr()))


def crr_partials(batch: int) -> int:
    return int(L.lib().rg_crr_partials(batch))


def crr_critic_head(q1, q2, q1_next_t, q2_next_t, next_logits, action, reward, reward_boosts, not_terminal, gamma,
                    target, dq1, dq2, partials1, partials2):
    _chk_dev(q1, q2, q1_next_t, q2_next_t, next_logits, action, reward, reward_boosts, not_terminal, target, dq1, dq2,
             partials1, partials2)
    batch, A = action.shape
    for t in (q1, q2, q1_next_t, q2_next_t, next_logits, action, dq1, dq2):
        assert t is None or (t.is_contiguous() and t.dtype == F32 and t.shape == (batch, A))
    _run("rg_crr_critic_head", dict(B=batch, A=A),
         lambda: L.lib().rg_crr_critic_head(L.ptr(q1), L.ptr(q2), L.ptr(q1_next_t), L.ptr(q2_next_t),
                                            L.ptr(next_logits), L.ptr(action), L.ptr(reward), L.ptr(reward_boosts),
                                            L.ptr(not_terminal), float(gamma), batch, A, L.ptr(target), L.ptr(dq1),
                                            L.ptr(dq2), L.ptr(partials1), L.ptr(partials2), L.stream_ptr()))


def crr_actor_head(q, logits, action, logged_prob, beta, max_weight, entropy_coeff, clip_limit, dlogits,
                   plain_partials, entropy_partials):
    _chk_dev(q, logits, action, logged_prob, dlogits, plain_partials, entropy_partials)
    batch, A = action.shape
    for t in (q, logits, action, dlogits):
        assert t.is_contiguous() and t.dtype == F32 and t.shape == (batch, A)
    _run("rg_crr_actor_head", dict(B=batch, A=A),
         lambda: L.lib().rg_crr_actor_head(L.ptr(q), L.ptr(logits), L.ptr(action), L.ptr(logged_prob), float(beta),
                                           float(max_weight), float(entropy_coeff), float(clip_limit), batch, A,
                                           L.ptr(dlogits), L.ptr(plain_partials), L.ptr(entropy_partials),
                                           L.stream_ptr()))


def qr_head(q, qn_online, qn_target, action, next_mask, reward, reward_boosts, not_terminal, gamma,
            gamma_exponent, quantiles, num_atoms, maxq, dq, loss_partials, all_q=None):
    _chk_dev(q, qn_online, qn_target, action, next_mask, reward, reward_boosts, not_terminal, gamma_exponent,
             quantiles, dq, loss_partials, all_q)
    batch, A = action.shape
    for t in (q, qn_online, qn_target, dq):
        assert t is None or (t.is_contiguous() and t.dtype == F32 and t.shape == (batch, A * num_atoms))
    _run("rg_qr_head", dict(B=batch, A=A, N=num_atoms),
         lambda: L.lib().rg_qr_head(L.ptr(q), L.ptr(qn_online), L.ptr(qn_target), L.ptr(action), L.ptr(next_mask),
                                    L.ptr(reward), L.ptr(reward_boosts), L.ptr(not_terminal), float(gamma),
                                    L.ptr(gamma_exponent), L.ptr(quantiles), batch, A, num_atoms, int(maxq),
                                    L.ptr(dq), L.ptr(loss_partials), L.ptr(all_q), L.stream_ptr()))


def reduce_sum(inp, n: int, scale: float, out):
    _chk_dev(inp, out)
    _run("rg_reduce_sum", dict(n=n), lambda: L.lib().rg_reduce_sum(L.ptr(inp), n, scale, L.ptr(out), L.stream_ptr()))


def adam_step(param, grad, exp_avg, exp_avg_sq, n, lr, beta1, beta2, eps, weight_decay, bc1, bc2_sqrt,
              grad_scale=1.0, offset=0):
    _chk_dev(param, grad, exp_avg, exp_avg_sq)
    o = offset * 4
    _run("rg_adam_step", dict(n=n),
         lambda: L.lib().rg_adam_step(param.data_ptr() + o, grad.data_ptr() + o, exp_avg.data_ptr() + o,
                                      exp_avg_sq.data_ptr() + o, n, lr, beta1, beta2, eps, weight_decay, bc1,
                                      bc2_sqrt, grad_scale, L.stream_ptr()))


def adam_step_sched(param, grad, exp_avg, exp_avg_sq, n, beta1, beta2, eps, weight_decay, sched, grad_scale=1.0,
                    offset=0):
    _chk_dev(param, grad, exp_avg, exp_avg_sq, sched)
    tick_fence(sched)
    o = offset * 4
    _run("rg_adam_step", dict(n=n),
         lambda: L.lib().rg_adam_step_sched(param.data_ptr() + o, grad.data_ptr() + o, exp_avg.data_ptr() + o,
                                            exp_avg_sq.data_ptr() + o, n, beta1, beta2, eps, weight_decay,
                                            grad_scale, sched.data_ptr(), L.stream_ptr()))


MAX_TICKS = 8
_tick_scopes = []
_DEFER_TICKS = os.environ.get("RG_DEFER_TICKS", "1") != "0"


def _flush_ticks(pending):
    if not pending:
        return
    if len(pending) == 1:
        s = pending[0]
        _run("rg_sched_tick", {}, lambda: L.lib().rg_sched_tick(s.data_ptr(), L.stream_ptr()))
    else:
        arr = (ctypes.c_void_p * len(pending))(*[s.data_ptr() for s in pending])
        _run("rg_sched_tick", dict(n=len(pending)), lambda: L.lib().rg_sched_tick_many(arr, len(pending), L.stream_ptr()))
    del pending[:]


class deferred_ticks:
    def __enter__(self):
        _tick_scopes.append([])
        return self

    def __exit__(self, *exc):
        _flush_ticks(_tick_scopes.pop())
        return False


# ... 220 lines not shown
```

### reagent_amd/training/dqn_trainer.py

```python
import logging
from dataclasses import dataclass, field
from typing import List, Optional, Tuple

import torch

from .. import _lib as L
from .. import ops
from ..core import types as rlt
from ..core.parameters import EvaluationParameters, RLParameters
from ..engine import ensure_slab, grad_views
from ..optimizer import Optimizer__Union, SoftUpdate
from .dqn_trainer_base import DQNTrainerBaseLightning

logger = logging.getLogger(__name__)


@dataclass(frozen=True)
class BCQConfig:
    drop_threshold: float = 0.1


class _HipLoss(torch.autograd.Function):

    @staticmethod
# ... 266 lines not shown
            self._alloc_head(batch, device)
            self._ws_batch = batch
        self._dw, self._db = grad_views(self.q_network.fc, self._slab, self._hip_params)

    @staticmethod
    def _f32c(t: torch.Tensor) -> torch.Tensor:
        t = t if t.dtype == torch.float32 else t.float()
        return t if t.is_contiguous() else t.contiguous()

    def _bcq_mask(self, next_mask, next_state):
        st = self.bcq_imitator.stack()
        st.stage_weights(need_transposed=False)
        xi, _ = st.stage_input(next_state, need_transposed=False)
        logits = torch.empty(next_state.shape[0], self.num_actions, dtype=torch.float32, device=next_state.device)
        st.forward(xi, logits, save=False)
        mask = next_mask.clone()
        ops.bcq_filter(logits, self.bcq_drop_threshold, mask)
        return mask

    def _needs_online_next(self) -> bool:
        return True

    _post_step_forward = True

    def _q_has_batch_norm(self) -> bool:
        if getattr(self, "_q_bn", None) is None:
            self._q_bn = self._post_step_forward and any(isinstance(m, torch.nn.BatchNorm1d) for m in self.q_network.modules())
        return self._q_bn

    def _post_step_stats_forward(self, training_batch):
        if not self._q_has_batch_norm() or not self.q_network.training:
            return
        qs = self._qs
        qs.stage_weights(need_transposed=True)
        xn, _ = qs.stage_input(self._net_in(training_batch.next_state.float_features), need_transposed=False)
        qs.forward(xn, self._qn_online, save=False)

    @staticmethod
    def _net_in(t: torch.Tensor) -> torch.Tensor:
        if t.dtype not in (torch.float32, torch.bfloat16):
            t = t.float()
        return t if t.stride(-1) == 1 and t.is_contiguous() else t.contiguous()

    def _hip_forward(self, b) -> torch.Tensor:
        state, next_state = self._net_in(b.state.float_features), self._net_in(b.next_state.float_features)
        L.require_cuda(state, "training_batch.state")
        B, dev = state.shape[0], state.device
        self._engine(B, dev)
        qs, ts = self._qs, self._ts
        qs.stage_weights(need_transposed=True)
        ts.stage_weights(need_transposed=False)
        xs, self._xs_t = qs.stage_input(state, need_transposed=True)
        xn, _ = qs.stage_input(next_state, need_transposed=False)
        if self._needs_online_next():
            qs.forward(xn, self._qn_online, save=False)
        ts.forward(xn, self._qn_target, save=False)
        qs.forward(xs, self._q, save=True)
        gamma_exp = None
        if self.use_seq_num_diff_as_time_diff:
            assert self.multi_steps is None
            gamma_exp = self._f32c(b.time_diff).reshape(-1)
        if self.multi_steps is not None:
            assert b.step is not None
            gamma_exp = self._f32c(b.step).reshape(-1)
        boosts = self.reward_boosts.reshape(-1).to(dev) if self._has_reward_boost else None
        if self.maxq_learning:
            next_mask = self._f32c(b.possible_next_actions_mask)
            if getattr(self, "bcq", False):
                next_mask = self._bcq_mask(next_mask, next_state)
        else:
            next_mask = self._f32c(b.next_action)
        self._run_head(b, B, self._f32c(b.action), next_mask, boosts, gamma_exp)
        return self._loss

    def _hip_backward(self, grad_out=None, async_reduce: bool = False):
        if grad_out is not None:
            self._dq.mul_(grad_out)
        held = held_gradients(self._slab, self._hip_params)
        self._qs.backward(self._dq, self._xs_t, self._dw, self._db, **self._take_loss_tail())
        if self._dp_group is not None:
            if async_reduce and ops.profiling():
                with ops.profile_span("all_reduce", dict(bytes=self._slab.grad.numel() * 4, world=self._dp_world)):
                    dp_reduce(self, self._slab)
            elif async_reduce:
                self._pending_reduce = torch.distributed.all_reduce(self._slab.grad, group=self._dp_group,
                                                                   async_op=True)
            else:
                dp_reduce(self, self._slab)
        publish_gradients(self._slab, self._hip_params, held)

    _loss_tail_wanted = False
    _loss_tail = None

    def _take_loss_tail(self) -> dict:
        tail, self._loss_tail = self._loss_tail, None
        return {"tail_sum": tail} if tail is not None else {}

    def enable_data_parallel(self, process_group=None):
        import torch.distributed as dist

        self._dp_group = process_group if process_group is not None else dist.group.WORLD
        self._dp_world = dist.get_world_size(self._dp_group)
        return self

    def _hip_loss(self, batch):
        self.apply_pending_update()
        loss_buf = self._hip_forward(batch)
        return _HipLoss.apply(self, loss_buf, *self._hip_params)

    def native_optimizers(self):
        if getattr(self, "_native_opts", None) is None:
            made = self.configure_optimizers()
            self._native_opts = [o["optimizer"] for o in made]
            self._native_scheds = [o.get("lr_scheduler") for o in made]
        return self._native_opts

    def native_schedulers(self):
        self.native_optimizers()
        return [s for s in self._native_scheds if s is not None]

    @torch.no_grad()
    def train_step_native(self, training_batch, defer_update: bool = False) -> torch.Tensor:
        self.apply_pending_update()
        self._loss_tail_wanted = True
        try:
            loss = self._hip_forward(training_batch)
# ... 203 lines not shown

    def validation_step(self, batch, batch_idx):
        raise NotImplementedError("CPE / EvaluationDataPage is outside the hot path (SURVEY.md §3.4)")


class DQNTrainer(QStepCore):
    def __init__(
        self,
        q_network,
        q_network_target,
        reward_network,
        q_network_cpe=None,
        q_network_cpe_target=None,
        metrics_to_score=None,
        evaluation: Optional[EvaluationParameters] = None,
        imitator=None,
        actions: Optional[List[str]] = None,
        rl: Optional[RLParameters] = None,
        double_q_learning: bool = True,
        bcq: Optional[BCQConfig] = None,
        minibatch_size: int = 1024,
        minibatches_per_step: int = 1,
        optimizer: Optional[Optimizer__Union] = None,
    ) -> None:
        evaluation = evaluation if evaluation is not None else EvaluationParameters()
        rl = rl if rl is not None else RLParameters()
        actions = actions if actions is not None else []
        optimizer = optimizer if optimizer is not None else Optimizer__Union.default()
        super().__init__(rl, metrics_to_score=metrics_to_score, actions=actions,
                         evaluation_parameters=evaluation)
        assert self._actions is not None, "Discrete-action DQN needs action names"
        self.double_q_learning = double_q_learning
        self.minibatch_size = minibatch_size
        self.minibatches_per_step = minibatches_per_step or 1

        self.q_network = q_network
        self.q_network_target = q_network_target
        self.q_network_optimizer = optimizer
        self._initialize_cpe(reward_network, q_network_cpe, q_network_cpe_target, optimizer=optimizer)
        self._cpe = _CpeEngine(self) if self.calc_cpe_in_training else None

        self.bcq = bcq is not None
        if self.bcq:
            self.bcq_drop_threshold = bcq.drop_threshold
            if imitator is None or not hasattr(imitator, "stack"):
                raise NotImplementedError(
                    "bcq needs `imitator` as a reagent_amd FullyConnectedNetwork (state features -> action logits); "
                    "scikit-learn imitators (a CPU call per batch) are not served")
            self.bcq_imitator = imitator

    def _alloc_head(self, batch, device):
        f32 = dict(dtype=torch.float32, device=device)
        self._loss_partials = torch.empty(ops.dqn_head_partials(batch), **f32)
        self._next_q = torch.empty(batch, **f32)
        self._next_idx = torch.empty(batch, dtype=torch.int64, device=device)
        self._q_sel = torch.empty(batch, **f32)

    def _run_head(self, b, B, action, next_mask, boosts, gamma_exp):
        ops.dqn_head(self._q, self._qn_online, self._qn_target, action, next_mask,
                     self._f32c(b.reward).reshape(-1), boosts, self._f32c(b.not_terminal).reshape(-1),
                     self.gamma, gamma_exp, self.double_q_learning, self._loss_type, self._dq,
                     self._loss_partials, self._next_q, self._next_idx, self._q_sel)
        from ..engine import FusedMLP

        if self._loss_tail_wanted and isinstance(self._qs, FusedMLP):
            self._loss_tail = (self._loss_partials, 1.0 / B, self._loss)
        else:
            ops.reduce_sum(self._loss_partials, self._loss_partials.numel(), 1.0 / B, self._loss)
        self.all_action_scores = self._q

    @torch.no_grad()
    def get_detached_model_outputs(self, state) -> Tuple[torch.Tensor, Optional[torch.Tensor]]:
        return self.q_network(state), self.q_network_target(state)

    def compute_discount_tensor(self, batch, boosted_rewards: torch.Tensor):
        discount_tensor = torch.full_like(boosted_rewards, self.gamma)
        if self.use_seq_num_diff_as_time_diff:
            assert self.multi_steps is None
            discount_tensor = torch.pow(self.gamma, batch.time_diff.float())
        if self.multi_steps is not None:
            assert batch.step is not None
            discount_tensor = torch.pow(self.gamma, batch.step.float())
        return discount_tensor

    def compute_td_loss(self, batch, boosted_rewards=None, discount_tensor=None):
        return self._hip_loss(batch)

    def train_step_gen(self, training_batch: rlt.DiscreteDqnInput, batch_idx: int):
        self._check_input(training_batch)
        td_loss = self.compute_td_loss(training_batch)
        yield td_loss
        td_loss = td_loss.detach()
        yield from self._cpe_segment(training_batch)
        self._log_dqn(td_loss, training_batch)
        yield self.soft_update_result()

    def _log_dqn(self, td_loss, training_batch):
        from .reagent_lightning_module import _NoOpReporter

        if isinstance(self._reporter, _NoOpReporter) and not self.logger:
            return
        rewards = self.boost_rewards(training_batch.reward, training_batch.action)
        logged_action_idxs = torch.argmax(training_batch.action, dim=1, keepdim=True)
        mask = training_batch.possible_actions_mask if self.maxq_learning else training_batch.action
        model_action_idxs = self.get_max_q_values(self.all_action_scores, mask.float())[1]
        self.reporter.log(
            td_loss=td_loss,
            logged_actions=logged_action_idxs,
            logged_propensities=training_batch.extras.action_probability,
            logged_rewards=rewards,
            logged_values=None,
            model_values=self.all_action_scores,
            model_values_on_logged_actions=None,
            model_action_idxs=model_action_idxs,
        )
        if self.logger:
            ap = training_batch.extras.action_probability
            greedy = torch.nn.functional.one_hot(model_action_idxs.reshape(-1), num_classes=self.num_actions).float().mean(dim=0)
            self.logger.log_metrics(
                {
                    "td_loss": td_loss,
# ... 13 lines not shown
```

Baseline: 146.8 million transitions/s.

## Fuse online next-state and state forwards with DQN head into one pair kernel

Adds a paired forward kernel that runs the online network over next_state and state inside one launch and computes the TD/Huber head in the output layer of the second pass. This replaces two separate online forward launches plus the head kernel and its reads of q and qn_online. Loss wave sums are laid out in runs and reduced inside the weight-gradient tail. The kernel restricts itself to ReLU hidden layers with 16 actions, and it makes one workgroup do two passes in sequence.

```diff
diff --git a/include/reagent_hip.h b/include/reagent_hip.h
--- a/include/reagent_hip.h
+++ b/include/reagent_hip.h
@@ -100,6 +100,7 @@
   const float* sum_in;
   float* sum_out;
   double sum_scale;
+  int32_t sum_run;
 } rg_mlp_desc;
 
 int rg_mlp_fused_supported(const rg_mlp_desc* d);
@@ -304,6 +305,14 @@
                 const float* not_terminal, double gamma, const float* gamma_exponent, int batch,
                 int num_actions, int double_q, int loss_type, float* dq, float* loss_partials,
                 float* next_q, int64_t* next_idx, float* q_sel, rg_stream_t stream);
+
+int rg_dqn_pair_wave_sums(int batch);
+int rg_dqn_online_pair_forward(const rg_mlp_desc* d, const void* state, int state_dtype, int64_t ld_state,
+                               const void* next_state, int next_state_dtype, int64_t ld_next_state, int batch, float* q,
+                               float* qn_online, const float* qn_target, const float* action, const float* next_mask,
+                               const float* reward, const float* reward_boosts, const float* not_terminal, double gamma,
+                               const float* gamma_exponent, int double_q, int loss_type, float* dq, float* loss_wave_sums,
+                               float* next_q, int64_t* next_idx, float* q_sel, rg_stream_t stream);
 
 int rg_bcq_filter(const float* imitator_logits, int batch, int num_actions, double drop_threshold, float* mask,
                   rg_stream_t stream);
@@ -408,6 +417,7 @@
                 float* out, int64_t ldo, rg_stream_t stream);
 
 int rg_reduce_sum(const float* in, int n, float scale, float* out, rg_stream_t stream);
+int rg_reduce_sum_runs(const float* in, int n, int run, float scale, float* out, rg_stream_t stream);
 
 
 int rg_adam_step(float* param, const float* grad, float* exp_avg, float* exp_avg_sq, int64_t n,
diff --git a/profiles/microbench/fwd_phases.hip b/profiles/microbench/fwd_phases.hip
--- a/profiles/microbench/fwd_phases.hip
+++ b/profiles/microbench/fwd_phases.hip
@@ -13,6 +13,14 @@
 }
 #include <cstdio>
 #include <vector>
+
+namespace rg {
+template <int TN, int NW, int PITCH>
+__global__ void RG_LAUNCH_BOUNDS(NW * 64, 1) fwd_some_save_kernel(MlpArgs saving, MlpArgs plain, int every) {
+  if ((int)blockIdx.x & every) mlp_fwd_fused_body<TN, NW, PITCH, false>(saving);
+  else mlp_fwd_fused_body<TN, NW, PITCH, false>(plain);
+}
+}
 
 int main(int argc, char** argv) {
   using namespace rg;
@@ -43,12 +51,20 @@
   hipMemcpyToSymbol(HIP_SYMBOL(g_stamps), &stamps, sizeof(stamps));
   a.out_lds = argc > 3 ? atoi(argv[3]) : 0;
   const size_t lds = (size_t)128 * 520 * 2 + (a.out_lds ? 32 * 512 : 0);
+  const int every = argc > 4 ? atoi(argv[4]) : 0;
+  MlpArgs plain = a;
+  plain.save = 0;
   hipFuncSetAttribute((const void*)mlp_fwd_fused_kernel<512 / (32 * FB_NW), FB_NW, 520>, hipFuncAttributeMaxDynamicSharedMemorySize, (int)lds);
+  hipFuncSetAttribute((const void*)fwd_some_save_kernel<512 / (32 * FB_NW), FB_NW, 520>, hipFuncAttributeMaxDynamicSharedMemorySize, (int)lds);
+  auto launch = [&] {
+    if (every) fwd_some_save_kernel<512 / (32 * FB_NW), FB_NW, 520><<<n_wg, FB_NW * 64, lds>>>(a, plain, every);
+    else mlp_fwd_fused_kernel<512 / (32 * FB_NW), FB_NW, 520><<<n_wg, FB_NW * 64, lds>>>(a);
+  };
   hipEvent_t e0, e1; hipEventCreate(&e0); hipEventCreate(&e1);
-  for (int w = 0; w < 3; ++w) mlp_fwd_fused_kernel<512 / (32 * FB_NW), FB_NW, 520><<<n_wg, FB_NW * 64, lds>>>(a);
+  for (int w = 0; w < 3; ++w) launch();
   hipDeviceSynchronize();
   hipEventRecord(e0);
-  for (int r = 0; r < 20; ++r) mlp_fwd_fused_kernel<512 / (32 * FB_NW), FB_NW, 520><<<n_wg, FB_NW * 64, lds>>>(a);
+  for (int r = 0; r < 20; ++r) launch();
   hipEventRecord(e1); hipEventSynchronize(e1);
   float ms; hipEventElapsedTime(&ms, e0, e1);
   printf("forward NW=%d RING=%d save=%d: %.2f us/launch (stamps on), err=%d\n", FB_NW, MlpCfg<FB_NW>::RING, save, ms * 1e3 / 20, (int)hipGetLastError());
@@ -58,13 +74,18 @@
                             "L1 mainloop(K=512)", "L1 pack", "L1 barrier wait", "L1 LDS store+barrier",
                             "L2 mainloop(K=512)", "L2 pack", "L2 barrier wait", "L2 LDS store+barrier", "output layer", ""};
   double tot[NPH] = {0}, span = 0;
-  for (int g = 0; g < n_wg; ++g)
+  int n_counted = 0;
+  for (int g = 0; g < n_wg; ++g) {
+    if (every && !(g & every)) continue;
+    ++n_counted;
     for (int w = 0; w < NWV; ++w) {
       const unsigned long long* s = &h[((size_t)g * NWV + w) * NPH];
       for (int p = 1; p <= 14; ++p) tot[p] += (double)(s[p] - s[p - 1]);
       span += (double)(s[14] - s[0]);
     }
-  const double nw = (double)n_wg * NWV;
+  }
+  const double nw = (double)n_counted * NWV;
+  if (every) printf("only workgroups with (index & %d) save: the tables below cover those %d\n", every, n_counted);
   printf("workgroups %d, shader clock %.3f GHz (ticks of one round / launch time)\n", n_wg, (span / nw) * ((n_wg + 255) / 256) / (ms * 1e6 / 20));
   printf("avg s_memtime ticks per wave: %.0f\n", span / nw);
   for (int p = 1; p <= 14; ++p) printf("  %-22s %9.0f ticks  %5.1f %%\n", names[p], tot[p] / nw, 100.0 * tot[p] / span);
@@ -73,7 +94,7 @@
     for (int g = 0; g < n_wg; ++g)
       for (int w = 0; w < NWV; ++w) {
         const unsigned long long* s = &h[((size_t)g * NWV + w) * NPH];
-        if (!s[16]) continue;
+        if (!s[16] || (every && !(g & every))) continue;
         if (s[19]) { t19 += (double)(s[19] - s[18]); n19 += 1; }
         t[0] += (double)(s[16] - s[13]); t[1] += (double)(s[17] - s[16]); t[2] += (double)(s[18] - s[17]); t[3] += (double)(s[14] - s[18]);
       }
diff --git a/reagent_amd/_lib.py b/reagent_amd/_lib.py
--- a/reagent_amd/_lib.py
+++ b/reagent_amd/_lib.py
@@ -7,7 +7,7 @@
 _HERE = os.path.dirname(os.path.abspath(__file__))
 LIB_PATH = os.environ.get("RG_LIB") or os.path.join(_HERE, "lib", "libreagent_hip.so")
 
-ABI_VERSION = 11
+ABI_VERSION = 12
 PREC_F32, PREC_BF16, PREC_BF16X3 = 0, 1, 2
 DT_F32, DT_BF16 = 0, 1
 ACT = {"linear": 0, "relu": 1, "leaky_relu": 2, "tanh": 3, "sigmoid": 4, "softplus": 5}
@@ -87,6 +87,7 @@
         ("sum_in", c_void_p),
         ("sum_out", c_void_p),
         ("sum_scale", ctypes.c_double),
+        ("sum_run", ctypes.c_int32),
     ]
 
 
@@ -224,6 +225,9 @@
     "rg_table_check_actions": (c_int, [ctypes.POINTER(DqnTable), c_void_p, c_int, c_void_p, c_void_p]),
     "rg_bcq_filter": (c_int, [c_void_p, c_int, c_int, c_d, c_void_p, c_void_p]),
     "rg_dqn_head_partials": (c_int, [c_int]),
+    "rg_dqn_pair_wave_sums": (c_int, [c_int]),
+    "rg_dqn_online_pair_forward": (c_int, [ctypes.POINTER(MlpDesc), c_void_p, c_int, c_i64, c_void_p, c_int, c_i64, c_int]
+                                   + [c_void_p] * 8 + [c_d, c_void_p, c_int, c_int] + [c_void_p] * 5 + [c_void_p]),
     "rg_dqn_head": (c_int, [c_void_p] * 8 + [c_d, c_void_p, c_int, c_int, c_int, c_int] + [c_void_p] * 5 + [c_void_p]),
     "rg_cpe_head": (c_int, [c_void_p] * 9 + [ctypes.c_double, c_void_p, ctypes.c_double, c_int, c_int, c_int, c_int,
                             c_void_p, c_void_p, c_void_p, c_void_p, c_void_p, c_void_p]),
@@ -250,6 +254,7 @@
                                   c_void_p, c_void_p]),
     "rg_add_cols": (c_int, [c_void_p, c_i64, c_void_p, c_i64, c_int, c_int, c_void_p, c_i64, c_void_p]),
     "rg_reduce_sum": (c_int, [c_void_p, c_int, c_f, c_void_p, c_void_p]),
+    "rg_reduce_sum_runs": (c_int, [c_void_p, c_int, c_int, c_f, c_void_p, c_void_p]),
     "rg_adam_step": (c_int, [c_void_p, c_void_p, c_void_p, c_void_p, c_i64, c_d, c_d, c_d, c_d, c_d,
                               c_d, c_d, c_d, c_void_p]),
     "rg_soft_update": (c_int, [c_void_p, c_void_p, c_i64, c_d, c_void_p]),
diff --git a/reagent_amd/csrc/heads.hip b/reagent_amd/csrc/heads.hip
--- a/reagent_amd/csrc/heads.hip
+++ b/reagent_amd/csrc/heads.hip
@@ -1,6 +1,7 @@
 #include <rg_platform.h>
 #include "../../include/reagent_hip.h"
 #include "rg_reduce.h"
+#include "rg_dqn_head_row.h"
 
 namespace rg {
 
@@ -107,65 +108,16 @@
   const int b_raw = blockIdx.x * 256 + t / G;
   const bool live = b_raw < batch;
   const int b = live ? b_raw : batch - 1;
-  float loss = 0.f;
-  {
-    const long o = (long)b * A + sub * 4;
-    const f32x4 m4 = *(const f32x4*)(next_mask + o);
-    const f32x4 qt4 = *(const f32x4*)(qn_target + o);
-    const f32x4 qo4 = double_q ? *(const f32x4*)(qn_online + o) : qt4;
-    const f32x4 ac4 = *(const f32x4*)(action + o);
-    const f32x4 q4 = *(const f32x4*)(q + o);
-    float best = 0.f, best_t = 0.f, rb = 0.f, qs = 0.f;
-    int best_i = 0;
-#pragma unroll
-    for (int e = 0; e < 4; ++e) {
-      const float pen = -1e9f * (1.f - m4[e]);
-      const float qo = qo4[e] + pen, qt = qt4[e] + pen;
-      const float key = double_q ? qo : qt;
-      if (e == 0 || key > best) {
-        best = key;
-        best_t = qt;
-        best_i = sub * 4 + e;
-      }
-      if (reward_boosts) rb += ac4[e] * reward_boosts[sub * 4 + e];
-      qs += q4[e] * ac4[e];
-    }
-#pragma unroll
-    for (int off = 1; off < G; off <<= 1) {
-      const float ok = shfl_xor(best, off), ot = shfl_xor(best_t, off);
-      const int oi = shfl_xor(best_i, off);
-      if (ok > best || (ok == best && oi < best_i)) {
-        best = ok;
-        best_t = ot;
-        best_i = oi;
-      }
-      rb += shfl_xor(rb, off);
-      qs += shfl_xor(qs, off);
-    }
-    const float rew = reward[b] + rb;
-    const float disc = gamma_exponent ? powf(gamma, gamma_exponent[b]) : gamma;
-    const float target = rew + disc * (best_t * not_terminal[b]);
-    const float d = qs - target;
-    float g, row_loss;
-    if (loss_type == RG_LOSS_HUBER) {
-      const float ad = fabsf(d);
-      row_loss = ad < 1.f ? 0.5f * d * d : ad - 0.5f;
-      g = ad < 1.f ? d : (d > 0.f ? 1.f : -1.f);
-    } else {
-      row_loss = d * d;
-      g = 2.f * d;
-    }
-    g /= (float)batch;
-    if (live) *(f32x4*)(dq + o) = f32x4{g * ac4[0], g * ac4[1], g * ac4[2], g * ac4[3]};
-    if (live && sub == 0) {
-      loss = row_loss;
-      if (next_q_out) next_q_out[b] = best_t;
-      if (next_idx_out) next_idx_out[b] = best_i;
-      if (q_sel_out) q_sel_out[b] = qs;
-    }
-  }
-#pragma unroll
-  for (int off = 32; off >= 1; off >>= 1) loss += shfl_xor(loss, off);
+  const long o = (long)b * A + sub * 4;
+  const f32x4 m4 = *(const f32x4*)(next_mask + o);
+  const f32x4 qt4 = *(const f32x4*)(qn_target + o);
+  const f32x4 qo4 = double_q ? *(const f32x4*)(qn_online + o) : qt4;
+  const f32x4 ac4 = *(const f32x4*)(action + o);
+  const f32x4 q4 = *(const f32x4*)(q + o);
+  float loss = dqn_head_lanes_row<G>(m4, qt4, qo4, ac4, q4, sub, b, live, reward[b], reward_boosts, not_terminal[b], gamma,
+                                     gamma_exponent != nullptr, gamma_exponent ? gamma_exponent[b] : 0.f, batch, double_q,
+                                     loss_type, dq, next_q_out, next_idx_out, q_sel_out);
+  loss = dqn_head_wave_sum(loss);
   if ((t & 63) == 0) scratch[t >> 6] = loss;
   __syncthreads();
   if (t == 0) {
@@ -568,6 +520,13 @@
   if (threadIdx.x == 0) out[0] = s * scale;
 }
 
+__global__ void reduce_sum_runs_kernel(const float* __restrict__ in, int n, int run, float scale,
+                                       float* __restrict__ out) {
+  __shared__ float scratch[4];
+  const float s = block_sum_256(strided_sum_256_runs(in, n, run, threadIdx.x), scratch);
+  if (threadIdx.x == 0) out[0] = s * scale;
+}
+
 }
 
 namespace rg {
@@ -714,4 +673,10 @@
   return (int)hipGetLastError();
 }
 
-}
+int rg_reduce_sum_runs(const float* in, int n, int run, float scale, float* out, rg_stream_t stream) {
+  if (!in || !out || n < 0 || run < 1) return RG_EINVAL;
+  RG_LAUNCH(reduce_sum_runs_kernel, dim3(1), dim3(HEAD_THREADS), (hipStream_t)stream, in, n, run, scale, out);
+  return (int)hipGetLastError();
+}
+
+}
diff --git a/reagent_amd/csrc/mlp_fused.hip b/reagent_amd/csrc/mlp_fused.hip
--- a/reagent_amd/csrc/mlp_fused.hip
+++ b/reagent_amd/csrc/mlp_fused.hip
@@ -1,6 +1,7 @@
 
 #include "rg_mlp_frag.h"
 #include "rg_reduce.h"
+#include "rg_dqn_head_row.h"
 #include <cstdio>
 
 namespace rg {
@@ -58,12 +59,14 @@
   RG_STAMP(19);
 }
 
-template <int TN, int NW, int PITCH, bool GROUPED>
-__device__ __forceinline__ void mlp_fwd_fused_body(const MlpArgs& a) {
+template <int TN, int NW, int PITCH, bool GROUPED, bool PAIR = false>
+__device__ __forceinline__ void mlp_fwd_fused_body(const MlpArgs& a, const PairArgs* pp = nullptr, int pass = 0, bool on_state = false) {
   constexpr int THREADS = MlpCfg<NW>::THREADS, RING = MlpCfg<NW>::RING;
+  static_assert(!PAIR || (!GROUPED && NW == 8), "the pair is the plain 8-wave kernel");
+  const int save = PAIR ? (on_state ? 1 : 0) : a.save;
   RG_DYN_LDS(smem);
   bf16_t* act = (bf16_t*)smem;
-  const int tid = threadIdx.x, lane = tid & 63, wave = wave_uniform(tid >> 6);
+  const int tid = PAIR ? opaque((int)threadIdx.x) : (int)threadIdx.x, lane = tid & 63, wave = wave_uniform(tid >> 6);
   const int lr = lane & 31, lg = lane >> 5;
   const int tile = GROUPED ? grouped_tile(blockIdx.x, (a.batch + FB_BM - 1) / FB_BM) : (int)blockIdx.x;
   if (GROUPED && tile * FB_BM >= round_up(a.batch, FB_BM)) return;
@@ -71,7 +74,15 @@
   constexpr int pitch = PITCH;
   const int k0p = round_up(a.dims[0], 32);
   RG_STAMP(0);
-  if (a.rowmap) {
+  if constexpr (PAIR) {
+    const PairIO& io = pp->io[on_state ? 1 : 0];
+    const void* x = io.x;
+    const long ldx = io.ldx;
+    if (io.x_is_f32)
+      load_tile_to_lds<float, THREADS>(act, pitch, (const float*)x, ldx, row_base, a.batch, a.dims[0], k0p, tid);
+    else
+      load_tile_to_lds<bf16_t, THREADS>(act, pitch, (const bf16_t*)x, ldx, row_base, a.batch, a.dims[0], k0p, tid);
+  } else if (a.rowmap) {
     if (a.x_is_f32)
       load_tile_rows_mapped<float, THREADS>(act, pitch, (const float*)a.x, a.ldx, a.rowmap, row_base, a.dims[0], k0p, tid);
     else
@@ -92,10 +103,10 @@
     load_tile_to_lds<bf16_t, THREADS>(act, pitch, (const bf16_t*)a.x, a.ldx, row_base, a.batch, a.dims[0], k0p, tid);
   __syncthreads();
   RG_STAMP(1);
-  if (a.save == 1 && a.act_frag[0]) emit_frags_from_lds(act, pitch, k0p / 32, a.act_frag[0], tile * 4, wave, NW, lane);
-  const bool out_lds = !GROUPED && a.out_lds;
+  if (save == 1 && a.act_frag[0]) emit_frags_from_lds(act, pitch, k0p / 32, a.act_frag[0], tile * 4, wave, NW, lane);
+  const bool out_lds = PAIR || (!GROUPED && a.out_lds);
   char* wo = (char*)(act + FB_BM * pitch);
-  if (out_lds) out_lds_prefetch(a.wfrag[a.n_layers - 1], (a.dims[a.n_layers - 1] + 15) / 16, wo, wave, NW, lane);
+  if (out_lds && pass == 0) out_lds_prefetch(a.wfrag[a.n_layers - 1], (a.dims[a.n_layers - 1] + 15) / 16, wo, wave, NW, lane);
 
   for (int l = 0; l < a.n_layers; ++l) {
     const int K = a.dims[l], N = a.dims[l + 1];
@@ -113,9 +124,13 @@
                               k_rotation(blockIdx.x, wave, KC), wave / (NW / 2));
       RG_STAMP(2 + 4 * l);
       unsigned PK[4][TN][8];
-      unsigned* sign_dst = a.save ? a.act_sign[l + 1] : nullptr;
-      RG_DISPATCH_ACT(a.acts[l], (fwd_hidden_pack<TN, A_>(acc, a.bias[l], fwd_save_dst(a, l),
-                                                          sign_dst, N / 32, tile * 4, wave, lane, PK)));
+      unsigned* sign_dst = save ? a.act_sign[l + 1] : nullptr;
+      if constexpr (PAIR) {
+        fwd_hidden_pack<TN, ACT_RELU>(acc, a.bias[l], save ? a.act_frag[l + 1] : nullptr, sign_dst, N / 32, tile * 4, wave, lane, PK);
+      } else {
+        RG_DISPATCH_ACT(a.acts[l], (fwd_hidden_pack<TN, A_>(acc, a.bias[l], fwd_save_dst(a, l),
+                                                            sign_dst, N / 32, tile * 4, wave, lane, PK)));
+      }
       RG_STAMP(3 + 4 * l);
       __syncthreads();
       RG_STAMP(4 + 4 * l);
@@ -159,7 +174,25 @@
             }
           }
         };
-        if (!GROUPED && NTo == 1 && NW == 8 && KC >= 8) {
+        f32x4 h_m4, h_qt4, h_ac4;
+        float h_rew = 0.f, h_nt = 0.f, h_ge = 0.f;
+        int h_b = 0;
+        bool h_live = false;
+        if constexpr (PAIR) {
+          if (pass == 1) {
+            const int it = wave * 64 + opaque(lane), row = row_base + (it >> 2);
+            h_live = row < a.batch;
+            h_b = h_live ? row : a.batch - 1;
+            const long o = (long)h_b * 16 + (it & 3) * 4;
+            h_m4 = *(const f32x4*)(pp->next_mask + o);
+            h_qt4 = *(const f32x4*)(pp->qn_target + o);
+            h_ac4 = *(const f32x4*)(pp->action + o);
+            h_rew = pp->reward[h_b];
+            h_nt = pp->not_terminal[h_b];
+            if (pp->gamma_exponent) h_ge = pp->gamma_exponent[h_b];
+          }
+        }
+        if (PAIR || (!GROUPED && NTo == 1 && NW == 8 && KC >= 8)) {
           const int tm = wave & 3, half = wave >> 2, kc_mid = (KC / 2 + 3) / 4 * 4;
           f32x16 acc = out_lds ? tile_kloop_ldsb(act, pitch, wo, tm, lane, half ? kc_mid : 0, half ? KC : kc_mid)
                                : tile_kloop(act, pitch, KC, wf_out, tm, 0, lane, half ? kc_mid : 0, half ? KC : kc_mid);
@@ -169,7 +202,7 @@
           const int o_ln = opaque(lane), o_lr = o_ln & 31, o_lg = o_ln >> 5;
           const bool aligned16 = (reinterpret_cast<uintptr_t>(a.out32) & 15) == 0;
           const bool dense_run = a.ldo == N && row_base + FB_BM <= a.batch;
-          const bool rowstore = !a.out_scatter && aligned16 && (dense_run || ((N & 3) == 0 && (a.ldo & 3) == 0));
+          const bool rowstore = PAIR || (!a.out_scatter && aligned16 && (dense_run || ((N & 3) == 0 && (a.ldo & 3) == 0)));
           if (rowstore) {
             float* outs = (float*)act + half * (FB_BM * 32);
             float* bias_s = (float*)act + 2 * (FB_BM * 32);
@@ -183,7 +216,30 @@
             RG_STAMP(19);
             const float* lo_ = (const float*)act;
             const float* hi_ = lo_ + FB_BM * 32;
-            if (dense_run) {
+            if constexpr (PAIR) {
+              const int it = wave * 64 + o_ln, rel = it >> 2, c4 = it & 3, row = row_base + rel;
+              const f32x4 l4 = *(const f32x4*)(lo_ + it * 4), h4 = *(const f32x4*)(hi_ + it * 4);
+              const f32x4 b4 = *(const f32x4*)(bias_s + c4 * 4);
+              float o[4];
+#pragma unroll
+              for (int e = 0; e < 4; ++e) o[e] = (l4[e] + h4[e]) + b4[e];
+              act_apply_n(o, out_act);
+              const f32x4 mine = f32x4{o[0], o[1], o[2], o[3]};
+              if (row < a.batch) *(f32x4*)(pp->io[on_state ? 1 : 0].out + (long)row * 16 + c4 * 4) = mine;
+              f32x4* park = (f32x4*)(wo + (size_t)KC * 512);
+              if (pass == 0) {
+                park[it] = mine;
+              } else {
+                const f32x4 other = park[it];
+                const f32x4 q4 = on_state ? mine : other, qon4 = on_state ? other : mine;
+                const float loss = dqn_head_lanes_row<4>(h_m4, h_qt4, pp->double_q ? qon4 : h_qt4, h_ac4, q4, c4, h_b, h_live, h_rew,
+                                                         pp->reward_boosts, h_nt, pp->gamma, pp->gamma_exponent != nullptr, h_ge,
+                                                         a.batch, pp->double_q, pp->loss_type, pp->dq, pp->next_q, pp->next_idx,
+                                                         pp->q_sel);
+                const float ws = dqn_head_wave_sum(loss);
+                if (o_ln == 0) pp->wave_sums[tile * NW + wave] = ws;
+              }
+            } else if (dense_run) {
               float* dst = a.out32 + (long)row_base * N;
               for (int it = wave * 64 + o_ln; it < (FB_BM * N) >> 2; it += THREADS) {
                 const f32x4 l4 = *(const f32x4*)(lo_ + it * 4), h4 = *(const f32x4*)(hi_ + it * 4);
@@ -195,7 +251,7 @@
               }
             }
             const int np = N >> 2;
-            for (int it = wave * 64 + o_ln; !dense_run && it < FB_BM * np; it += THREADS) {
+            for (int it = wave * 64 + o_ln; !PAIR && !dense_run && it < FB_BM * np; it += THREADS) {
               const int rel = it / np, c4 = it - rel * np;
               const int row = row_base + rel;
               if (row < a.batch) {
@@ -279,6 +335,17 @@
   }
 }
 
+#ifndef RG_PAIR_ORDER_SHIFT
+#define RG_PAIR_ORDER_SHIFT 0
+#endif
+template <int TN, int NW, int PITCH>
+__global__ void RG_LAUNCH_BOUNDS(NW * 64, 1) mlp_fwd_pair_kernel(MlpArgs a, PairArgs p) {
+  const bool state_first = (((int)blockIdx.x >> RG_PAIR_ORDER_SHIFT) & 1) != 0;
+  mlp_fwd_fused_body<TN, NW, PITCH, false, true>(a, &p, 0, state_first);
+  __syncthreads();
+  mlp_fwd_fused_body<TN, NW, PITCH, false, true>(a, &p, 1, !state_first);
+}
+
 template <int TN, int NW, int PITCH>
 __global__ void RG_LAUNCH_BOUNDS(NW * 64, 1) mlp_fwd_fused_kernel(MlpArgs a) {
   mlp_fwd_fused_body<TN, NW, PITCH, false>(a);
@@ -1027,6 +1094,7 @@
   int elem_blocks;
   const float* sum_in;
   int sum_n;
+  int sum_run;
   float sum_scale;
   float* sum_out;
 };
@@ -1047,7 +1115,8 @@
     return;
   }
   __shared__ float scratch[4];
-  float acc = strided_sum_256(T.sum_in, T.sum_n, threadIdx.x);
+  float acc = T.sum_run > 1 ? strided_sum_256_runs(T.sum_in, T.sum_n, T.sum_run, threadIdx.x)
+                            : strided_sum_256(T.sum_in, T.sum_n, threadIdx.x);
 #pragma unroll
   for (int off = 32; off >= 1; off >>= 1) acc += shfl_xor(acc, off);
   if ((threadIdx.x & 63) == 0) scratch[threadIdx.x >> 6] = acc;
@@ -1304,20 +1373,21 @@
   }
 }
 
-#define RG_LAUNCH_FUSED(KERNEL, hidden, pitch, grid, lds, stream, args)                                      \
+#define RG_LAUNCH_FUSED_ARGS(KERNEL, hidden, pitch, grid, lds, stream, ...)                                     \
   do {                                                                                                       \
     const dim3 block_(FB_NW * 64);                                                                           \
     if ((hidden) == 256 && (pitch) == 264) {                                                                 \
       RG_ALLOW_LDS((KERNEL<256 / (32 * FB_NW), FB_NW, 264>), lds);                                           \
-      RG_LAUNCH_DYN((KERNEL<256 / (32 * FB_NW), FB_NW, 264>), grid, block_, lds, (hipStream_t)stream, args); \
+      RG_LAUNCH_DYN((KERNEL<256 / (32 * FB_NW), FB_NW, 264>), grid, block_, lds, (hipStream_t)stream, __VA_ARGS__); \
     } else if ((hidden) == 256) {                                                                            \
       RG_ALLOW_LDS((KERNEL<256 / (32 * FB_NW), FB_NW, 520>), lds);                                           \
-      RG_LAUNCH_DYN((KERNEL<256 / (32 * FB_NW), FB_NW, 520>), grid, block_, lds, (hipStream_t)stream, args); \
+      RG_LAUNCH_DYN((KERNEL<256 / (32 * FB_NW), FB_NW, 520>), grid, block_, lds, (hipStream_t)stream, __VA_ARGS__); \
     } else {                                                                                                 \
       RG_ALLOW_LDS((KERNEL<512 / (32 * FB_NW), FB_NW, 520>), lds);                                           \
-      RG_LAUNCH_DYN((KERNEL<512 / (32 * FB_NW), FB_NW, 520>), grid, block_, lds, (hipStream_t)stream, args); \
+      RG_LAUNCH_DYN((KERNEL<512 / (32 * FB_NW), FB_NW, 520>), grid, block_, lds, (hipStream_t)stream, __VA_ARGS__); \
     }                                                                                                        \
   } while (0)
+#define RG_LAUNCH_FUSED(KERNEL, hidden, pitch, grid, lds, stream, args) RG_LAUNCH_FUSED_ARGS(KERNEL, hidden, pitch, grid, lds, stream, args)
 
 }
 
@@ -1395,6 +1465,47 @@
   }
   if (d->tile_key) RG_LAUNCH_FUSED(mlp_fwd_grouped_kernel, d->dims[1], a.pitch, grid, lds, stream, a);
   else RG_LAUNCH_FUSED(mlp_fwd_fused_kernel, d->dims[1], a.pitch, grid, lds, stream, a);
+  return (int)hipGetLastError();
+}
+
+int rg_dqn_pair_wave_sums(int batch) { return (batch + FB_BM - 1) / FB_BM * FB_NW; }
+
+int rg_dqn_online_pair_forward(const rg_mlp_desc* d, const void* state, int state_dtype, int64_t ld_state,
+                               const void* next_state, int next_state_dtype, int64_t ld_next_state, int batch, float* q,
+                               float* qn_online, const float* qn_target, const float* action, const float* next_mask,
+                               const float* reward, const float* reward_boosts, const float* not_terminal, double gamma,
+                               const float* gamma_exponent, int double_q, int loss_type, float* dq, float* loss_wave_sums,
+                               float* next_q, int64_t* next_idx, float* q_sel, rg_stream_t stream) {
+  if (!fused_supported(d)) return RG_EUNSUPPORTED;
+  if (!state || !next_state || !q || !qn_online || !qn_target || !action || !next_mask || !reward || !not_terminal || !dq ||
+      !loss_wave_sums || batch <= 0)
+    return RG_EINVAL;
+  if (loss_type != RG_LOSS_MSE && loss_type != RG_LOSS_HUBER) return RG_EINVAL;
+  const int L = d->n_layers, KCo = (d->dims[L - 1] + 15) / 16;
+  if (d->x3 || d->x2 || d->rowmap || d->tile_key || L < 2 || d->dims[L] != 16 || KCo < 8 || (KCo & 1)) return RG_EUNSUPPORTED;
+  for (int l = 0; l + 1 < L; ++l)
+    if (d->acts[l] != RG_ACT_RELU) return RG_EUNSUPPORTED;
+  if (((uintptr_t)q | (uintptr_t)qn_online | (uintptr_t)qn_target | (uintptr_t)action | (uintptr_t)next_mask | (uintptr_t)dq) & 15)
+    return RG_EUNSUPPORTED;
+  MlpArgs a;
+  int rc = fill_args(d, batch, a, 0);
+  if (rc) return rc;
+  for (int l = 0; l < L; ++l)
+    if (!d->act_frag[l]) return RG_EINVAL;
+  const size_t park = (size_t)FB_BM * 16 * sizeof(float);
+  const size_t lds = (size_t)FB_BM * a.pitch * sizeof(bf16_t) + (size_t)KCo * 512 + park;
+  if (lds > 160 * 1024) return RG_EUNSUPPORTED;
+  a.x = nullptr; a.ldx = 0; a.x_is_f32 = 0; a.out32 = nullptr; a.ldo = 16; a.save = 0;
+  a.stage_out = 0; a.out_lds = 1;
+  PairArgs p;
+  p.io[0] = PairIO{next_state, (long)ld_next_state, qn_online, next_state_dtype == RG_DT_F32, 0};
+  p.io[1] = PairIO{state, (long)ld_state, q, state_dtype == RG_DT_F32, 0};
+  p.qn_target = qn_target; p.action = action; p.next_mask = next_mask; p.reward = reward;
+  p.reward_boosts = reward_boosts; p.not_terminal = not_terminal; p.gamma_exponent = gamma_exponent; p.gamma = (float)gamma;
+  p.double_q = double_q; p.loss_type = loss_type; p.dq = dq; p.wave_sums = loss_wave_sums; p.next_q = next_q;
+  p.next_idx = next_idx; p.q_sel = q_sel;
+  const dim3 grid((batch + FB_BM - 1) / FB_BM);
+  RG_LAUNCH_FUSED_ARGS(mlp_fwd_pair_kernel, d->dims[1], a.pitch, grid, lds, stream, a, p);
   return (int)hipGetLastError();
 }
 
@@ -1791,7 +1902,7 @@
   for (int i = C.n; i <= FB_MAXL; ++i) C.block_begin[i] = blocks;
   for (int i = C.n; i < FB_MAXL; ++i) { C.partials[i] = nullptr; C.out[i] = nullptr; C.N[i] = 0; }
   if (d->sum_in && (!d->sum_out || d->sum_n <= 0)) return RG_EINVAL;
-  T.sum_in = d->sum_in; T.sum_n = d->sum_n; T.sum_scale = (float)d->sum_scale; T.sum_out = d->sum_out;
+  T.sum_in = d->sum_in; T.sum_n = d->sum_n; T.sum_run = d->sum_run; T.sum_scale = (float)d->sum_scale; T.sum_out = d->sum_out;
   RG_LAUNCH(reduce_tail_kernel, dim3((unsigned)(elem_blocks + blocks + (d->sum_in ? 1 : 0))), dim3(256), (hipStream_t)stream, T);
   return (int)hipGetLastError();
 }
diff --git a/reagent_amd/csrc/optim.hip b/reagent_amd/csrc/optim.hip
--- a/reagent_amd/csrc/optim.hip
+++ b/reagent_amd/csrc/optim.hip
@@ -102,7 +102,7 @@
   return (int)hipGetLastError();
 }
 
-int rg_abi_version(void) { return 11; }
+int rg_abi_version(void) { return 12; }
 
 const char* rg_strerror(int code) {
   switch (code) {
diff --git a/reagent_amd/csrc/rg_dqn_head_row.h b/reagent_amd/csrc/rg_dqn_head_row.h
--- /dev/null
+++ b/reagent_amd/csrc/rg_dqn_head_row.h
@@ -0,0 +1,75 @@
+#pragma once
+#include <rg_platform.h>
+#include "../../include/reagent_hip.h"
+
+namespace rg {
+
+template <int G>
+__device__ __forceinline__ float dqn_head_lanes_row(const f32x4 m4, const f32x4 qt4, const f32x4 qo4, const f32x4 ac4,
+                                                    const f32x4 q4, int sub, int b, bool live, float reward_b,
+                                                    const float* __restrict__ reward_boosts, float not_terminal_b,
+                                                    float gamma, bool has_gamma_exp, float gamma_exp_b, int batch,
+                                                    int double_q, int loss_type, float* __restrict__ dq,
+                                                    float* __restrict__ next_q_out, int64_t* __restrict__ next_idx_out,
+                                                    float* __restrict__ q_sel_out) {
+  constexpr int A = 4 * G;
+  const long o = (long)b * A + sub * 4;
+  float best = 0.f, best_t = 0.f, rb = 0.f, qs = 0.f;
+  int best_i = 0;
+#pragma unroll
+  for (int e = 0; e < 4; ++e) {
+    const float pen = -1e9f * (1.f - m4[e]);
+    const float qo = qo4[e] + pen, qt = qt4[e] + pen;
+    const float key = double_q ? qo : qt;
+    if (e == 0 || key > best) {
+      best = key;
+      best_t = qt;
+      best_i = sub * 4 + e;
+    }
+    if (reward_boosts) rb += ac4[e] * reward_boosts[sub * 4 + e];
+    qs += q4[e] * ac4[e];
+  }
+#pragma unroll
+  for (int off = 1; off < G; off <<= 1) {
+    const float ok = shfl_xor(best, off), ot = shfl_xor(best_t, off);
+    const int oi = shfl_xor(best_i, off);
+    if (ok > best || (ok == best && oi < best_i)) {
+      best = ok;
+      best_t = ot;
+      best_i = oi;
+    }
+    rb += shfl_xor(rb, off);
+    qs += shfl_xor(qs, off);
+  }
+  const float rew = reward_b + rb;
+  const float disc = has_gamma_exp ? powf(gamma, gamma_exp_b) : gamma;
+  const float target = rew + disc * (best_t * not_terminal_b);
+  const float d = qs - target;
+  float g, row_loss;
+  if (loss_type == RG_LOSS_HUBER) {
+    const float ad = fabsf(d);
+    row_loss = ad < 1.f ? 0.5f * d * d : ad - 0.5f;
+    g = ad < 1.f ? d : (d > 0.f ? 1.f : -1.f);
+  } else {
+    row_loss = d * d;
+    g = 2.f * d;
+  }
+  g /= (float)batch;
+  if (live) *(f32x4*)(dq + o) = f32x4{g * ac4[0], g * ac4[1], g * ac4[2], g * ac4[3]};
+  float loss = 0.f;
+  if (live && sub == 0) {
+    loss = row_loss;
+    if (next_q_out) next_q_out[b] = best_t;
+    if (next_idx_out) next_idx_out[b] = best_i;
+    if (q_sel_out) q_sel_out[b] = qs;
+  }
+  return loss;
+}
+
+__device__ __forceinline__ float dqn_head_wave_sum(float loss) {
+#pragma unroll
+  for (int off = 32; off >= 1; off >>= 1) loss += shfl_xor(loss, off);
+  return loss;
+}
+
+}
diff --git a/reagent_amd/csrc/rg_mlp_frag.h b/reagent_amd/csrc/rg_mlp_frag.h
--- a/reagent_amd/csrc/rg_mlp_frag.h
+++ b/reagent_amd/csrc/rg_mlp_frag.h
@@ -73,6 +73,24 @@
   long dz_lo[FB_MAXL];
 };
 
+struct PairIO {
+  const void* x;
+  long ldx;
+  float* out;
+  int x_is_f32, pad_;
+};
+struct PairArgs {
+  PairIO io[2];
+  const float *qn_target, *action, *next_mask, *reward, *reward_boosts, *not_terminal, *gamma_exponent;
+  float gamma;
+  int double_q, loss_type;
+  float* dq;
+  float* wave_sums;
+  float* next_q;
+  int64_t* next_idx;
+  float* q_sel;
+};
+
 __device__ __forceinline__ int round_up(int x, int m) { return (x + m - 1) / m * m; }
 
 template <int ACT> __device__ __forceinline__ float act_t(float z) { return act_apply(z, ACT); }
diff --git a/reagent_amd/csrc/rg_reduce.h b/reagent_amd/csrc/rg_reduce.h
--- a/reagent_amd/csrc/rg_reduce.h
+++ b/reagent_amd/csrc/rg_reduce.h
@@ -28,4 +28,27 @@
          (((a[8] + a[9]) + (a[10] + a[11])) + ((a[12] + a[13]) + (a[14] + a[15])));
 }
 
+__device__ __forceinline__ float run_sum(const float* __restrict__ in, int n_in, int run, int i) {
+  float s = 0.f;
+  for (int w = 0; w < run; ++w) {
+    const long j = (long)i * run + w;
+    s += j < n_in ? in[j] : 0.f;
+  }
+  return s;
 }
+__device__ __forceinline__ float strided_sum_256_runs(const float* __restrict__ in, int n_in, int run, int tid) {
+  const int n = (n_in + run - 1) / run;
+  float a[16];
+#pragma unroll
+  for (int j = 0; j < 16; ++j) a[j] = 0.f;
+  int i = tid;
+  for (; i + 15 * 256 < n; i += 16 * 256) {
+#pragma unroll
+    for (int j = 0; j < 16; ++j) a[j] += run_sum(in, n_in, run, i + j * 256);
+  }
+  for (; i < n; i += 256) a[0] += run_sum(in, n_in, run, i);
+  return (((a[0] + a[1]) + (a[2] + a[3])) + ((a[4] + a[5]) + (a[6] + a[7]))) +
+         (((a[8] + a[9]) + (a[10] + a[11])) + ((a[12] + a[13]) + (a[14] + a[15])));
+}
+
+}
diff --git a/reagent_amd/engine.py b/reagent_amd/engine.py
--- a/reagent_amd/engine.py
+++ b/reagent_amd/engine.py
@@ -379,7 +379,7 @@
         d.x3 = int(self.x3)
         d.dx_col0 = 0
         d.dx_only = 0
-        d.defer_db, d.sum_n = 0, 0
+        d.defer_db, d.sum_n, d.sum_run = 0, 0, 0
         d.db_partials, d.sum_in, d.sum_out = None, None, None
         for i, v in enumerate(self.dims):
             d.dims[i] = v
@@ -423,6 +423,37 @@
                                                       L.stream_ptr()))
         self._saved = save
         return out32
+
+    def dqn_pair_supported(self, num_actions: int) -> bool:
+        k = self.dims[-2]
+        return (not self.x3 and num_actions == 16 and self.dims[-1] == 16 and k >= 128 and ((k + 15) // 16) % 2 == 0
+                and all(a == L.ACT["relu"] for a in self.acts[:-1]))
+
+    def dqn_pair_forward(self, state: torch.Tensor, next_state: torch.Tensor, q, qn_online, qn_target, action, next_mask, reward,
+                         reward_boosts, not_terminal, gamma, gamma_exponent, double_q, loss_type, dq, wave_sums,
+                         next_q=None, next_idx=None, q_sel=None):
+        B, A = q.shape
+        ops._chk_dev(state, next_state, q, qn_online, qn_target, action, next_mask, reward, reward_boosts, not_terminal,
+                     gamma_exponent, dq, wave_sums, next_q, next_idx, q_sel)
+        assert state.shape == (B, self.dims[0]) and next_state.shape == (B, self.dims[0])
+        assert state.stride(1) == 1 and next_state.stride(1) == 1
+        for t in (q, qn_online, qn_target, action, next_mask, dq):
+            assert t.is_contiguous() and t.dtype == torch.float32 and t.shape == (B, A)
+        for t in (reward, not_terminal, gamma_exponent):
+            assert t is None or (t.is_contiguous() and t.dtype == torch.float32 and t.numel() == B)
+        assert reward_boosts is None or (reward_boosts.dtype == torch.float32 and reward_boosts.numel() == A)
+        assert wave_sums.dtype == torch.float32 and wave_sums.numel() == ops.dqn_pair_wave_sums(B)
+        self._ensure_ws(B, state.device, training=True)
+        d = self._fill_desc()
+        d.x2, d.ldx2, d.x_split, d.rowmap = None, 0, 0, None
+        ops._run("rg_mlp_forward_fused", dict(B=2 * B, save=1, dims=tuple(self.dims), pair=1),
+                 lambda: L.lib().rg_dqn_online_pair_forward(
+                     d, state.data_ptr(), ops.dt_code(state.dtype), state.stride(0), next_state.data_ptr(),
+                     ops.dt_code(next_state.dtype), next_state.stride(0), B, L.ptr(q), L.ptr(qn_online), L.ptr(qn_target),
+                     L.ptr(action), L.ptr(next_mask), L.ptr(reward), L.ptr(reward_boosts), L.ptr(not_terminal), float(gamma),
+                     L.ptr(gamma_exponent), int(double_q), loss_type, L.ptr(dq), L.ptr(wave_sums), L.ptr(next_q),
+                     L.ptr(next_idx), L.ptr(q_sel), L.stream_ptr()))
+        self._saved = 1
 
     def backward(self, dout32: torch.Tensor, xt, dw: List[torch.Tensor], db: List[torch.Tensor],
                  dx32: Optional[torch.Tensor] = None, skip_wgrad: bool = False,
@@ -459,15 +490,16 @@
             if defer:
                 d.db_partials = ws["bwd"].data_ptr()
             if tail_sum is not None:
-                part, scale, out = tail_sum
+                part, scale, out = tail_sum[:3]
                 L.require_cuda(part)
                 L.require_cuda(out)
                 assert part.dtype == torch.float32 and part.is_contiguous() and out.dtype == torch.float32
                 d.sum_in, d.sum_n, d.sum_scale, d.sum_out = part.data_ptr(), part.numel(), float(scale), out.data_ptr()
+                d.sum_run = int(tail_sum[3]) if len(tail_sum) > 3 else 0
             wsb = ws["wgrad"].numel() * 4
             ops._run("rg_mlp_wgrad_fused", dict(B=B, dims=tuple(self.dims)),
                      lambda: lib.rg_mlp_wgrad_fused(d, B, ws["wgrad"].data_ptr(), wsb, L.stream_ptr()))
-            d.db_partials, d.sum_in, d.sum_out, d.sum_n = None, None, None, 0
+            d.db_partials, d.sum_in, d.sum_out, d.sum_n, d.sum_run = None, None, None, 0, 0
         else:
             assert tail_sum is None, "tail_sum rides in the weight gradient's launch"
 
diff --git a/reagent_amd/ops.py b/reagent_amd/ops.py
--- a/reagent_amd/ops.py
+++ b/reagent_amd/ops.py
@@ -442,6 +442,13 @@
     return int(L.lib().rg_dqn_head_partials(batch))
 
 
+def dqn_pair_wave_sums(batch: int) -> int:
+    return int(L.lib().rg_dqn_pair_wave_sums(batch))
+
+
+DQN_PAIR_RUN = 16
+
+
 def dqn_head(q, qn_online, qn_target, action, next_mask, reward, reward_boosts, not_terminal, gamma,
              gamma_exponent, double_q, loss_type, dq, loss_partials, next_q=None, next_idx=None,
              q_sel=None):
@@ -541,6 +548,12 @@
                                     L.ptr(dq), L.ptr(loss_partials), L.ptr(all_q), L.stream_ptr()))
 
 
+def reduce_sum_runs(inp, n: int, run: int, scale: float, out):
+    _chk_dev(inp, out)
+    _run("rg_reduce_sum_runs", dict(n=n, run=run),
+         lambda: L.lib().rg_reduce_sum_runs(L.ptr(inp), n, run, scale, L.ptr(out), L.stream_ptr()))
+
+
 def reduce_sum(inp, n: int, scale: float, out):
     _chk_dev(inp, out)
     _run("rg_reduce_sum", dict(n=n), lambda: L.lib().rg_reduce_sum(L.ptr(inp), n, scale, L.ptr(out), L.stream_ptr()))
diff --git a/reagent_amd/training/dqn_trainer.py b/reagent_amd/training/dqn_trainer.py
--- a/reagent_amd/training/dqn_trainer.py
+++ b/reagent_amd/training/dqn_trainer.py
@@ -342,10 +342,12 @@
         ts.stage_weights(need_transposed=False)
         xs, self._xs_t = qs.stage_input(state, need_transposed=True)
         xn, _ = qs.stage_input(next_state, need_transposed=False)
-        if self._needs_online_next():
+        paired = self._pair_wanted(qs, ts)
+        if not paired and self._needs_online_next():
             qs.forward(xn, self._qn_online, save=False)
         ts.forward(xn, self._qn_target, save=False)
-        qs.forward(xs, self._q, save=True)
+        if not paired:
+            qs.forward(xs, self._q, save=True)
         gamma_exp = None
         if self.use_seq_num_diff_as_time_diff:
             assert self.multi_steps is None
@@ -360,8 +362,14 @@
                 next_mask = self._bcq_mask(next_mask, next_state)
         else:
             next_mask = self._f32c(b.next_action)
-        self._run_head(b, B, self._f32c(b.action), next_mask, boosts, gamma_exp)
+        if paired:
+            self._run_pair(b, B, xs, xn, self._f32c(b.action), next_mask, boosts, gamma_exp)
+        else:
+            self._run_head(b, B, self._f32c(b.action), next_mask, boosts, gamma_exp)
         return self._loss
+
+    def _pair_wanted(self, qs, ts) -> bool:
+        return False
 
     def _hip_backward(self, grad_out=None, async_reduce: bool = False):
         if grad_out is not None:
@@ -671,6 +679,7 @@
     def _alloc_head(self, batch, device):
         f32 = dict(dtype=torch.float32, device=device)
         self._loss_partials = torch.empty(ops.dqn_head_partials(batch), **f32)
+        self._wave_sums = torch.empty(ops.dqn_pair_wave_sums(batch), **f32)
         self._next_q = torch.empty(batch, **f32)
         self._next_idx = torch.empty(batch, dtype=torch.int64, device=device)
         self._q_sel = torch.empty(batch, **f32)
@@ -686,6 +695,21 @@
             self._loss_tail = (self._loss_partials, 1.0 / B, self._loss)
         else:
             ops.reduce_sum(self._loss_partials, self._loss_partials.numel(), 1.0 / B, self._loss)
+        self.all_action_scores = self._q
+
+    def _pair_wanted(self, qs, ts) -> bool:
+        from ..engine import FusedMLP
+
+        return (self._loss_tail_wanted and type(self)._run_head is DQNTrainer._run_head and isinstance(qs, FusedMLP) and isinstance(ts, FusedMLP)
+                and not ts.x3 and qs.dqn_pair_supported(self.num_actions) and not self.bcq
+                and getattr(self, "_cpe", None) is None and not self._q_has_batch_norm())
+
+    def _run_pair(self, b, B, xs, xn, action, next_mask, boosts, gamma_exp):
+        self._qs.dqn_pair_forward(xs, xn, self._q, self._qn_online, self._qn_target, action, next_mask,
+                                  self._f32c(b.reward).reshape(-1), boosts, self._f32c(b.not_terminal).reshape(-1),
+                                  self.gamma, gamma_exp, self.double_q_learning, self._loss_type, self._dq,
+                                  self._wave_sums, self._next_q, self._next_idx, self._q_sel)
+        self._loss_tail = (self._wave_sums, 1.0 / B, self._loss, ops.DQN_PAIR_RUN)
         self.all_action_scores = self._q
 
     @torch.no_grad()
```

New measurement: 151.3 million transitions/s, median of 6. 1.03x the previous value.
